# ducha-aiki/affnet

Measured on AMD Instinct MI355X. Metric: keypoints/sec (detect+AffNet+OriNet+HardNet) per image, 2000 kp @1024x768, higher is better.
Workload: dtype f32

## Files before the change

affnet_amd/SparseImgRepresenter.py:

```python
import ctypes as C

import torch
import torch.nn as nn

from . import _lib, engine
from ._lib import lib, check, ptr
from .architectures import _HipPatchNet
from .HandCraftedModules import AffineShapeEstimator, OrientationDetector, _HipHandCrafted
from .HardNet import HardTFeatNet
from .pytorch_sift import SIFTNet

_FOLLOW = (SIFTNet, HardTFeatNet)


class ScaleSpaceAffinePatchExtractor(nn.Module):
    def __init__(self, border=16, num_features=500, patch_size=32, mrSize=3.0, nlevels=3, num_Baum_iters=0,
                 init_sigma=1.6, th=None, RespNet=None, OriNet=None, AffNet=None, arith="fp32"):
        super(ScaleSpaceAffinePatchExtractor, self).__init__()
        self.arith = arith
        _lib.arith_code(arith)
        self.mrSize, self.PS, self.b = mrSize, patch_size, border
        self.num, self.nlevels = num_features, nlevels
        self.num_Baum_iters, self.init_sigma = num_Baum_iters, init_sigma
        self.th = th
        if th is not None:
            self.num = -1
        else:
            self.th = 0
        self.RespNet = RespNet
        if not 1 <= nlevels <= 6:
            raise NotImplementedError("nlevels must be 1..6 (levels per octave = nlevels + 2 <= 8)")
        self.OriNet = OriNet if OriNet is not None else OrientationDetector(patch_size=19)
        self.AffNet = AffNet if AffNet is not None else AffineShapeEstimator(patch_size=19)
        self.scale_pyr = self.sigmas = self.pix_dists = None
        self._ctx = None
        self._ctx_key = None
        self._fctx = self._fctx_key = self._pyr_ctx = None
        self.last_ids = None
        self.max_keep = 16384
        self.raw_div = 4
        self.lazy_shape_rows = -1
        self.shape_form = 1

        self.desc_form = 1

    def _context(self, x, allow_batch=False):
        engine.require_cuda(x, "image")
        if x.dim() != 4 or x.size(1) != 1 or x.size(0) < 1 or (x.size(0) != 1 and not allow_batch):
            raise ValueError("expected a (1,1,H,W) image; forward() is batch-size-1 like the reference "
                             "(HandCraftedModules.py:283-284) - use enqueue()/run_batch() for (B,1,H,W) batches")
        pre = int(1.5 * self.num) if self.num_Baum_iters > 0 else self.num
        key = (x.size(0), x.size(2), x.size(3), x.device, pre, self.num, float(self.th), self.mrSize, self.b, self.init_sigma,
               self.nlevels, self.max_keep, self.num_Baum_iters, self.raw_div, self.lazy_shape_rows)
        if self._ctx is not None and self._ctx_key == key and self._ctx.arith != _lib.arith_code(self.arith):
            self._ctx.set_arith(self.arith)
        if self._ctx is None or self._ctx_key != key:
            self._ctx = engine.Context(x.size(2), x.size(3), x.device, self.nlevels, self.init_sigma, self.b, self.mrSize,
                                       float(self.th), self.num, pre, self.max_keep, batch=x.size(0), baum_iters=self.num_Baum_iters, raw_div=self.raw_div,
                                       lazy_shape_rows=self.lazy_shape_rows, arith=self.arith)
            self._ctx_key = key
        if self._ctx.shape_form != int(self.shape_form):
            self._ctx.set_shape_form(self.shape_form)
        if self._ctx.desc_form != int(self.desc_form):
            self._ctx.set_desc_form(self.desc_form)
        return self._ctx

    def _publish_pyramid(self, ctx):
        self._pyr_ctx = ctx
        self.scale_pyr = ctx.pyramid_views()
        self.sigmas = [list(s) for s in ctx.plan.sigmas]
        self.pix_dists = [list(p) for p in ctx.plan.pix_dists]

    def _response_pyramid(self, ctx, img):
        dev = img.device
        st = engine.stream_of(dev)
        check(lib.affnet_pyramid_build(ctx.handle, ptr(img), st), ctx.handle, "affnet_pyramid_build")
        stride = lib.affnet_pyramid_image_stride(ctx.handle)
        base = lib.affnet_pyramid_level_offset(ctx.handle, 0, 0)
        resp = torch.zeros(ctx.batch * stride, dtype=torch.float32, device=dev)
        with torch.no_grad():
            for b in range(ctx.batch):
                pyr = ctx.pyramid_views(b)
                for o, (h, w) in enumerate(ctx.plan.sizes):
                    for l in range(ctx.plan.levels_per_octave):
                        off = b * stride + lib.affnet_pyramid_level_offset(ctx.handle, o, l) - base
                        r = self.RespNet(pyr[o][l], ctx.plan.sigmas[o][l])
                        resp[off:off + h * w].copy_(r.reshape(-1).to(dev, torch.float32))
        return resp

    @staticmethod
    def _native(slot):
        return slot is None or isinstance(slot, (_HipPatchNet, _HipHandCrafted))

    def enqueue(self, x, do_ori=False, desc=None, det_stream=None, input_ready=None):
        ctx = self._context(x, allow_batch=True)
        dev = x.device
        if not (self._native(self.AffNet) and self._native(self.OriNet)):
            raise NotImplementedError("the fused path needs the native AffNetFast / OriNetFast slots (foreign slots: forward())")
        img = x.contiguous().float()
        B, F = x.size(0), ctx.cap_final
        lafs = torch.empty(B, F, 2, 3, dtype=torch.float32, device=dev)
        resp = torch.empty(B, F, dtype=torch.float32, device=dev)
        ids = torch.empty(B, F, 3, dtype=torch.int32, device=dev)
        count = torch.zeros(B, dtype=torch.int32, device=dev)
        dsc = torch.empty(B, F, 128, dtype=torch.float32, device=dev) if desc is not None else None
        nets = self._nets(dev, do_ori, desc)
        follow = isinstance(desc, _FOLLOW)
        if isinstance(desc, HardTFeatNet):
            desc.check_usable()
        fused_dsc = None if follow else dsc
        if self.RespNet is not None:
            rmaps = self._response_pyramid(ctx, img)
            check(lib.affnet_detect_image_responses(ctx.handle, ptr(rmaps), engine.stream_of(dev)), ctx.handle, "affnet_detect_image_responses")
            rc = lib.affnet_describe_detected(ctx.handle, C.byref(nets), int(bool(do_ori)), ptr(lafs), ptr(resp), ptr(ids), ptr(fused_dsc),
                                              ptr(count), engine.stream_of(dev))
            check(rc, ctx.handle, "affnet_describe_detected")
        elif det_stream is None:
            rc = lib.affnet_extract_features(ctx.handle, C.byref(nets), ptr(img), int(bool(do_ori)), ptr(lafs), ptr(resp), ptr(ids),
                                             ptr(fused_dsc), ptr(count), engine.stream_of(dev))
            check(rc, ctx.handle, "affnet_extract_features")
        else:
            cur = torch.cuda.current_stream(dev)
            if input_ready is None:
                det_stream.wait_stream(cur)
            elif input_ready is not False:
                det_stream.wait_event(input_ready)
            if getattr(self, "_busy", None) is not None:
                det_stream.wait_event(self._busy)
            rc = lib.affnet_detect_image(ctx.handle, ptr(img), C.c_void_p(det_stream.cuda_stream))
            check(rc, ctx.handle, "affnet_detect_image")
            ev = torch.cuda.Event()
            ev.record(det_stream)
            cur.wait_event(ev)
            rc = lib.affnet_describe_detected(ctx.handle, C.byref(nets), int(bool(do_ori)), ptr(lafs), ptr(resp), ptr(ids), ptr(fused_dsc),
                                              ptr(count), engine.stream_of(dev))
            check(rc, ctx.handle, "affnet_describe_detected")
            self._busy = torch.cuda.Event()
            self._busy.record(cur)
        if follow:
            self._desc_follow(ctx, desc, lafs, count, dsc)
            if det_stream is not None:
                self._busy = torch.cuda.Event()
                self._busy.record(torch.cuda.current_stream(dev))
        if B == 1:
            lafs, resp, ids, dsc = lafs[0], resp[0], ids[0], (None if dsc is None else dsc[0])
        return {"LAFs": lafs, "responses": resp, "ids": ids, "descriptors": dsc, "count": count, "overflow": ctx.counter_view(0), "_img": img}

    def _desc_follow(self, ctx, desc, lafs, count, dsc):
        dev, (B, F) = lafs.device, lafs.shape[:2]
        st = engine.stream_of(dev)
        lvl = torch.empty(B, F, 3, dtype=torch.int32, device=dev)
        norm = torch.empty(B, F, 2, 3, dtype=torch.float32, device=dev)
        check(lib.affnet_level_select(ctx.handle, ptr(lafs), ptr(count), F, desc.PS, ptr(lvl), ptr(norm), st), ctx.handle, "affnet_level_select")
        if isinstance(desc, HardTFeatNet):
            floats = lib.affnet_tfeat_scratch_floats(B * F)
            cached = getattr(self, "_tfeat_scratch", None)
            if cached is None or cached.device != dev or cached.numel() < floats:
                cached = self._tfeat_scratch = torch.empty(floats, dtype=torch.float32, device=dev)
            check(lib.affnet_tfeat_forward_pyr(ctx.handle, ptr(desc.packed_weights(dev)), ptr(norm), ptr(lvl), ptr(count), F, ptr(dsc), ptr(cached), st),
                  ctx.handle, "affnet_tfeat_forward_pyr")
            return
        check(lib.affnet_sift_forward_pyr(ctx.handle, ptr(norm), ptr(lvl), ptr(count), F, ptr(desc.window(dev)), float(desc.clipval), ptr(dsc), st),
              ctx.handle, "affnet_sift_forward_pyr")

    def _nets(self, dev, do_ori, desc):
        nets = _lib.Nets()
        if self.num_Baum_iters > 0:
            if isinstance(self.AffNet, _HipHandCrafted):
                nets.h_baumberg_window = C.cast(self.AffNet.window(), C.c_void_p)
            else:
                nets.d_affnet = self.AffNet.packed_weights(dev).data_ptr()
        if do_ori:
            if isinstance(self.OriNet, _HipHandCrafted):
                nets.h_orientation_window = C.cast(self.OriNet.window(), C.c_void_p)
            else:
                nets.d_orinet = self.OriNet.packed_weights(dev).data_ptr()
        nets.d_hardnet = desc.packed_weights(dev).data_ptr() if desc is not None and not isinstance(desc, _FOLLOW) else None
        return nets

    def capture(self, x, do_ori=False, desc=None):
        if isinstance(desc, _FOLLOW):
            raise NotImplementedError("graph capture covers the fused C call (HardNet descriptors or none); the SIFT and HardTFeat descriptors "
                                      "follow it as further launches - use enqueue() / run()")
        return CapturedPath(self, x, do_ori, desc)

    def run_batch(self, x, do_ori=False, desc=None):
        r = self.enqueue(x, do_ori=do_ori, desc=desc)
        ctx = self._ctx
        ctx.read_counts(allow_empty=True)
        cnt = r["count"].cpu().tolist()
        if x.size(0) == 1:
            r = {k: (v.unsqueeze(0) if isinstance(v, torch.Tensor) and k not in ("count", "overflow", "_img") else v) for k, v in r.items()}
        out = []
        for b, n in enumerate(cnt):
            dsc = r["descriptors"]
            out.append({"LAFs": r["LAFs"][b, :n], "responses": r["responses"][b, :n], "ids": r["ids"][b, :n],
                        "descriptors": None if dsc is None else dsc[b, :n]})
        return out

    def run(self, x, do_ori=False, desc=None):
        if x.dim() == 4 and x.size(0) != 1:
            raise ValueError("run() is for a single (1,1,H,W) image; use run_batch() for (B,1,H,W) batches")
        r = self.enqueue(x, do_ori=do_ori, desc=desc)
        ctx = self._ctx
        self._publish_pyramid(ctx)
        n = int(ctx.read_counts()[1])
        self.last_ids = r["ids"][:n]
        dsc = r["descriptors"]
        return {"LAFs": r["LAFs"][:n], "responses": r["responses"][:n], "ids": r["ids"][:n],
                "descriptors": None if dsc is None else dsc[:n]}

    def _frames_context(self, x, n_max):
        engine.require_cuda(x, "image")
        if x.dim() != 4 or x.size(1) != 1 or x.size(0) < 1:
            raise ValueError("expected a (B,1,H,W) image batch")
        budget = self.num if (0 < self.num < n_max and self.num_Baum_iters > 0) else n_max
        key = (x.size(0), x.size(2), x.size(3), x.device, n_max, budget, self.mrSize, self.b, self.init_sigma, self.nlevels, self.num_Baum_iters,
               self.raw_div, self.lazy_shape_rows)
        if self._fctx is not None and self._fctx_key == key and self._fctx.arith != _lib.arith_code(self.arith):
            self._fctx.set_arith(self.arith)
        if self._fctx is None or self._fctx_key != key:
            self._fctx = engine.Context(x.size(2), x.size(3), x.device, self.nlevels, self.init_sigma, self.b, self.mrSize, float(self.th), budget, n_max,
                                        self.max_keep, batch=x.size(0), baum_iters=self.num_Baum_iters, raw_div=self.raw_div,
                                        lazy_shape_rows=self.lazy_shape_rows, arith=self.arith)
            self._fctx_key = key
        if self._fctx.shape_form != int(self.shape_form):
            self._fctx.set_shape_form(self.shape_form)
        if self._fctx.desc_form != int(self.desc_form):
            self._fctx.set_desc_form(self.desc_form)
        return self._fctx

    def enqueue_frames(self, x, LAFs, responses=None, counts=None, do_ori=True, desc=None):
        if not (self._native(self.AffNet) and self._native(self.OriNet)):
            raise NotImplementedError("the fused path needs the native AffNetFast / OriNetFast slots (foreign slots: getAffineShape / getOrientation)")
        engine.require_cuda(x, "image")
        engine.require_cuda(LAFs, "LAFs")
        dev, B = x.device, x.size(0)
        fr = LAFs.contiguous().float()
        if fr.dim() == 3:
            fr = fr.unsqueeze(0)
        if fr.dim() != 4 or fr.size(0) != B or tuple(fr.shape[2:]) != (2, 3):
            raise ValueError("LAFs must be (n,2,3) for one image or (B,n_max,2,3) for a (B,1,H,W) batch, got %s" % (tuple(LAFs.shape),))
        n_max = fr.size(1)
        if n_max == 0:
            fr, responses, counts, n_max = torch.zeros(B, 1, 2, 3, dtype=torch.float32, device=dev), None, [0] * B, 1
        rin = None
        if responses is not None:
            engine.require_cuda(responses, "responses")
            rin = responses.contiguous().float().view(B, n_max)
        cin = None
        if counts is not None:
            cin = counts if isinstance(counts, torch.Tensor) else torch.tensor(list(counts), dtype=torch.int32)
            cin = cin.to(dev, torch.int32).contiguous().view(B)
        ctx = self._frames_context(x, n_max)
        img = x.contiguous().float()
        F = ctx.cap_final
        lafs = torch.empty(B, F, 2, 3, dtype=torch.float32, device=dev)
        resp = torch.empty(B, F, dtype=torch.float32, device=dev)
        ids = torch.empty(B, F, 3, dtype=torch.int32, device=dev)
        count = torch.zeros(B, dtype=torch.int32, device=dev)
        dsc = torch.empty(B, F, 128, dtype=torch.float32, device=dev) if desc is not None else None
        nets = self._nets(dev, do_ori, desc)
        follow = isinstance(desc, _FOLLOW)
        if isinstance(desc, HardTFeatNet):
            desc.check_usable()
        rc = lib.affnet_describe_frames(ctx.handle, C.byref(nets), ptr(img), ptr(fr), ptr(rin), ptr(cin), n_max, int(bool(do_ori)), ptr(lafs), ptr(resp),
                                        ptr(ids), None if follow else ptr(dsc), ptr(count), engine.stream_of(dev))
        check(rc, ctx.handle, "affnet_describe_frames")
        if follow:
            self._desc_follow(ctx, desc, lafs, count, dsc)
        self._publish_pyramid(ctx)
        if B == 1:
            lafs, resp, ids, dsc = lafs[0], resp[0], ids[0], (None if dsc is None else dsc[0])
        return {"LAFs": lafs, "responses": resp, "ids": ids, "descriptors": dsc, "count": count, "overflow": ctx.counter_view(0), "_img": img,
                "_frames": (fr, rin, cin)}

    def describe_frames(self, x, LAFs, responses=None, counts=None, do_ori=True, desc=None):
        r = self.enqueue_frames(x, LAFs, responses=responses, counts=counts, do_ori=do_ori, desc=desc)
        ctx = self._fctx
        dsc = r["descriptors"]
        if x.size(0) == 1:
            n = int(ctx.read_counts()[1])
            self.last_ids = r["ids"][:n]
            return {"LAFs": r["LAFs"][:n], "responses": r["responses"][:n], "ids": r["ids"][:n], "descriptors": None if dsc is None else dsc[:n]}
        ctx.read_counts(allow_empty=True)
        return [{"LAFs": r["LAFs"][b, :n], "responses": r["responses"][b, :n], "ids": r["ids"][b, :n],
                 "descriptors": None if dsc is None else dsc[b, :n]} for b, n in enumerate(r["count"].cpu().tolist())]

    def _pyramid_ctx(self):
        ctx = self._pyr_ctx
        if ctx is None or self.scale_pyr is None:
            raise RuntimeError("call forward() / run() first: the pyramid of the last image is reused (stateful like the reference)")
        if ctx.batch != 1:
            raise RuntimeError("getAffineShape / getOrientation work on the pyramid of a single image")
        return ctx

    def _shape_stage(self, ctx, resp, lafs, ids, cnt, n):
        dev, st = lafs.device, engine.stream_of(lafs.device)
        P, F = ctx.cap_pre, ctx.cap_final
        PS = self.AffNet.PS
        patches = torch.empty(n, 1, PS, PS, dtype=torch.float32, device=dev)

        def shape_pass(frames):
            check(lib.affnet_pyr_grid_sample(ctx.handle, ptr(frames), ptr(ids), ptr(cnt), n, PS, ptr(patches), st), ctx.handle,
                  "affnet_pyr_grid_sample")
            with torch.no_grad():
                a = torch.cat([self.AffNet(patches[s:s + 256], {}) for s in range(0, n, 256)], 0)
            full = torch.zeros(P, 2, 2, dtype=torch.float32, device=dev)
            full[:n] = a.to(dev, torch.float32)
            return full
        A = shape_pass(lafs)
        if self.num_Baum_iters > 1:
            frames = torch.empty(P, 2, 3, dtype=torch.float32, device=dev)
            for _ in range(1, self.num_Baum_iters):
                check(lib.affnet_shape_iterate(ctx.handle, None, ptr(A), ptr(lafs), ptr(cnt), 0, ptr(frames), st), ctx.handle, "affnet_shape_iterate")
                Ai = shape_pass(frames)
                check(lib.affnet_shape_iterate(ctx.handle, ptr(Ai), ptr(A), ptr(lafs), ptr(cnt), 1, ptr(frames), st), ctx.handle, "affnet_shape_iterate")
        r2 = torch.empty(F, dtype=torch.float32, device=dev)
        l2 = torch.empty(F, 2, 3, dtype=torch.float32, device=dev)
        i2 = torch.empty(F, 3, dtype=torch.int32, device=dev)
        c2 = torch.zeros(1, dtype=torch.int32, device=dev)
        check(lib.affnet_shape_filter_select(ctx.handle, ptr(resp), ptr(lafs), ptr(ids), ptr(A), ptr(cnt), ptr(r2), ptr(l2),
                                             ptr(i2), ptr(c2), st), ctx.handle, "affnet_shape_filter_select")
        return r2, l2, i2, c2, int(c2.item())

    def _orientation_stage(self, ctx, lafs, ids, cnt, n):
        dev, st = lafs.device, engine.stream_of(lafs.device)
        PS = self.OriNet.PS
        patches = torch.empty(n, 1, PS, PS, dtype=torch.float32, device=dev)
        if n:
            check(lib.affnet_pyr_grid_sample(ctx.handle, ptr(lafs), ptr(ids), ptr(cnt), n, PS, ptr(patches), st), ctx.handle,
                  "affnet_pyr_grid_sample")
        with torch.no_grad():
            ang = self.OriNet(patches)
        if ang.dim() <= 2:
            c, s = torch.cos(ang).view(-1, 1, 1), torch.sin(ang).view(-1, 1, 1)
            ang = torch.cat([torch.cat([c, s], 2), torch.cat([-s, c], 2)], 1)
        R = ang.to(dev, torch.float32).contiguous()
        if n:
            check(lib.affnet_apply_rotation(ctx.handle, ptr(lafs), ptr(R), ptr(cnt), n, st), ctx.handle, "affnet_apply_rotation")

    @staticmethod
    def _frame_rows(ctx, LAFs, pyr_idxs, level_idxs, cap):
        engine.require_cuda(LAFs, "LAFs")
        dev, n = LAFs.device, LAFs.size(0)
        if n > cap:
            raise ValueError("%d frames, the context of the last forward() holds %d rows" % (n, cap))
        lafs = torch.zeros(cap, 2, 3, dtype=torch.float32, device=dev)
        lafs[:n] = LAFs.float()
        ids = torch.zeros(cap, 3, dtype=torch.int32, device=dev)
        ids[:n, 0] = torch.as_tensor(pyr_idxs).to(dev).view(-1).to(torch.int32)
        ids[:n, 1] = torch.as_tensor(level_idxs).to(dev).view(-1).to(torch.int32)
        ids[:n, 2] = torch.arange(n, dtype=torch.int32, device=dev)
        return lafs, ids, torch.full((1,), n, dtype=torch.int32, device=dev), n

    def getAffineShape(self, final_resp, LAFs, final_pyr_idxs, final_level_idxs, num_features=0):
        ctx = self._pyramid_ctx()
        if self.num_Baum_iters <= 0:
            raise ValueError("getAffineShape needs num_Baum_iters > 0 (the reference's loop body never runs otherwise, SparseImgRepresenter.py:127)")
        if num_features != self.num and not (num_features <= 0 and self.num <= 0):
            raise ValueError("num_features = %d: the context of the last forward() is sized for the extractor's own budget (%d)" % (num_features, self.num))
        lafs, ids, cnt, n = self._frame_rows(ctx, LAFs, final_pyr_idxs, final_level_idxs, ctx.cap_pre)
        resp = torch.zeros(ctx.cap_pre, dtype=torch.float32, device=lafs.device)
        resp[:n] = final_resp.to(lafs.device, torch.float32).view(-1)
        resp, lafs, ids, cnt, n = self._shape_stage(ctx, resp, lafs, ids, cnt, n)
        self.last_ids = ids[:n]
        return resp[:n], lafs[:n], ids[:n, 0].long(), ids[:n, 1].long()

    def getOrientation(self, LAFs, final_pyr_idxs, final_level_idxs):
        ctx = self._pyramid_ctx()
        lafs, ids, cnt, n = self._frame_rows(ctx, LAFs, final_pyr_idxs, final_level_idxs, LAFs.size(0))
        self._orientation_stage(ctx, lafs, ids, cnt, n)
        return lafs

    def _staged(self, x, do_ori):
        ctx = self._context(x)
        dev, st = x.device, engine.stream_of(x.device)
        img = x.contiguous().float()
        P = ctx.cap_pre
        rmaps = None
        if self.RespNet is not None:
            rmaps = self._response_pyramid(ctx, img)
        else:
            check(lib.affnet_pyramid_build(ctx.handle, ptr(img), st), ctx.handle, "affnet_pyramid_build")
        self._publish_pyramid(ctx)
        resp = torch.empty(P, dtype=torch.float32, device=dev)
        lafs = torch.empty(P, 2, 3, dtype=torch.float32, device=dev)
        ids = torch.empty(P, 3, dtype=torch.int32, device=dev)
        cnt = torch.zeros(1, dtype=torch.int32, device=dev)
        if rmaps is not None:
            check(lib.affnet_detect_responses(ctx.handle, ptr(rmaps), ptr(resp), ptr(lafs), ptr(ids), ptr(cnt), st), ctx.handle,
                  "affnet_detect_responses")
        else:
            check(lib.affnet_detect(ctx.handle, ptr(resp), ptr(lafs), ptr(ids), ptr(cnt), st), ctx.handle, "affnet_detect")
        n = int(cnt.item())
        ctx.read_counts()
        if self.num_Baum_iters > 0:
            resp, lafs, ids, cnt, n = self._shape_stage(ctx, resp, lafs, ids, cnt, n)
        if do_ori:
            self._orientation_stage(ctx, lafs, ids, cnt, n)
        out = torch.empty_like(lafs)
        check(lib.affnet_scale_lafs(ctx.handle, ptr(lafs), ptr(out), ptr(cnt), lafs.size(0), x.size(3), x.size(2), 0, st), ctx.handle,
              "affnet_scale_lafs")
        self.last_ids = ids[:n]
        return out[:n], resp[:n]

    def forward(self, x, do_ori=False):
        aff_native = self.num_Baum_iters == 0 or self._native(self.AffNet)
        ori_native = (not do_ori) or self._native(self.OriNet)
        if aff_native and ori_native:
            form, self.shape_form = self.shape_form, 0
            try:
                r = self.run(x, do_ori=do_ori)
            finally:
                self.shape_form = form
            return r["LAFs"], r["responses"]
        return self._staged(x, do_ori)

    def extract_patches_from_pyr(self, dLAFs, PS=41):
        if self._ctx is None or self.scale_pyr is None:
            raise RuntimeError("call forward() first: the pyramid of the last image is reused (stateful like the reference)")
        ctx = self._ctx
        if ctx.batch != 1:
            raise RuntimeError("extract_patches_from_pyr works on the pyramid of a single-image forward()")
        engine.require_cuda(dLAFs, "dLAFs")
        dev, st = dLAFs.device, engine.stream_of(dLAFs.device)
        lafs = dLAFs.contiguous().float()
        n = lafs.size(0)
        out = torch.empty(n, 1, PS, PS, dtype=torch.float32, device=dev)
        if n == 0:
            return out
        ids = torch.empty(n, 3, dtype=torch.int32, device=dev)
        norm = torch.empty(n, 2, 3, dtype=torch.float32, device=dev)
        check(lib.affnet_level_select(ctx.handle, ptr(lafs), None, n, PS, ptr(ids), ptr(norm), st), ctx.handle, "affnet_level_select")
        check(lib.affnet_pyr_grid_sample(ctx.handle, ptr(norm), ptr(ids), None, n, PS, ptr(out), st), ctx.handle, "affnet_pyr_grid_sample")
        self.last_level_ids = ids
        return out


class CapturedPath(object):
    def __init__(self, det, x, do_ori, desc):
        if not (det._native(det.AffNet) and det._native(det.OriNet)) or det.RespNet is not None:
            raise NotImplementedError("graph capture needs the native slots (foreign slots run Python between the stages)")
        ctx = det._context(x, allow_batch=True)
        dev = x.device
        self.det, self.ctx, self.do_ori, self.desc = det, ctx, bool(do_ori), desc
        B, F = x.size(0), ctx.cap_final
        self.image = x.contiguous().float().clone()
        self.out = {"LAFs": torch.empty(B, F, 2, 3, dtype=torch.float32, device=dev), "responses": torch.empty(B, F, dtype=torch.float32, device=dev),
                    "ids": torch.empty(B, F, 3, dtype=torch.int32, device=dev), "count": torch.zeros(B, dtype=torch.int32, device=dev),
                    "descriptors": torch.empty(B, F, 128, dtype=torch.float32, device=dev) if desc is not None else None}
        self._nets = det._nets(dev, do_ori, desc)
        self._mods = [m for m in (det.AffNet, det.OriNet if do_ori else None, desc) if m is not None and hasattr(m, "packed_weights")]
        self._blobs = [m.packed_weights(dev) for m in self._mods]
        self._stamps = [m._weights_stamp() for m in self._mods]
        self._arith = ctx.arith
        self._stream = torch.cuda.Stream(device=dev)
        torch.cuda.synchronize(dev)
        o = self.out
        check(lib.affnet_graph_capture_extract(ctx.handle, C.byref(self._nets), ptr(self.image), int(self.do_ori), ptr(o["LAFs"]), ptr(o["responses"]),
                                               ptr(o["ids"]), ptr(o["descriptors"]), ptr(o["count"]), C.c_void_p(self._stream.cuda_stream)),
              ctx.handle, "affnet_graph_capture_extract")

    def launch(self, x=None, check_weights=True):
        if check_weights:
            for m, stamp in zip(self._mods, self._stamps):
                if m._weights_stamp() != stamp:
                    raise RuntimeError("the weights of %s changed after capture(): the graph holds the old packed weights - capture again" % type(m).__name__)
        if self.ctx.arith != self._arith:
            raise RuntimeError("the arithmetic mode of the extractor changed after capture(): the graph runs the mode it was captured with - capture again")
        if x is not None:
            self.image.copy_(x, non_blocking=True)
        busy = getattr(self.det, "_busy", None)
        if busy is not None:
            torch.cuda.current_stream(self.image.device).wait_event(busy)
        check(lib.affnet_graph_launch(self.ctx.handle, engine.stream_of(self.image.device)), self.ctx.handle, "affnet_graph_launch")
        out = dict(self.out, overflow=self.ctx.counter_view(0), _img=self.image)
        if self.image.size(0) == 1:
            return {k: (v[0] if (v is not None and k not in ("count", "overflow", "_img")) else v) for k, v in out.items()}
        return out

    def run(self, x=None, check_weights=True):
        if self.image.size(0) != 1:
            raise ValueError("run() is for single images; use launch() for batches")
        r = self.launch(x, check_weights=check_weights)
        self.det._publish_pyramid(self.ctx)
        n = int(self.ctx.read_counts()[1])
        dsc = r["descriptors"]
        return {"LAFs": r["LAFs"][:n], "responses": r["responses"][:n], "ids": r["ids"][:n], "descriptors": None if dsc is None else dsc[:n]}


def get_geometry_and_descriptors(img, det, desc, do_ori=True):
    from .HardNet import HardNet
    if isinstance(desc, (HardNet,) + _FOLLOW) and det._native(det.AffNet) and det._native(det.OriNet):
        r = det.run(img, do_ori=do_ori, desc=desc)
        return r["LAFs"], r["descriptors"]
    with torch.no_grad():
        LAFs, resp = det(img, do_ori=do_ori)
        patches = det.extract_patches_from_pyr(LAFs, PS=32)
        return LAFs, desc(patches)
```

affnet_amd/_lib.py:

```python
import ctypes as C
import os

_HERE = os.path.dirname(os.path.abspath(__file__))
LIB_PATH = os.environ.get("AFFNET_HIP_LIB") or os.path.join(_HERE, "libaffnet_hip.so")
PROBES_LIB_PATH = os.path.join(_HERE, "libaffnet_hip_probes.so")

MAX_OCTAVES, MAX_LEVELS, MAX_TAPS = 16, 8, 37
NET_AFFNET, NET_ORINET, NET_HARDNET, NET_AFFNET_FULLCONV = 0, 1, 2, 3
ARITH_FP32_MFMA, ARITH_FP32_SPLIT3, ARITH_FP32_SPLIT2H = 0, 1, 2
ARITH_NAMES = {"fp32": ARITH_FP32_MFMA, "fp32_mfma": ARITH_FP32_MFMA, "fp32_split3": ARITH_FP32_SPLIT3, "split3": ARITH_FP32_SPLIT3,
               "fp32_split2h": ARITH_FP32_SPLIT2H, "split2h": ARITH_FP32_SPLIT2H}


def arith_code(arith):
    if arith is None:
        return ARITH_FP32_MFMA
    if isinstance(arith, str):
        if arith.lower() not in ARITH_NAMES:
            raise ValueError("arith must be one of %s" % sorted(ARITH_NAMES))
        return ARITH_NAMES[arith.lower()]
    if int(arith) not in (ARITH_FP32_MFMA, ARITH_FP32_SPLIT3, ARITH_FP32_SPLIT2H):
        raise ValueError("arith must be AFFNET_ARITH_FP32_MFMA (0), AFFNET_ARITH_FP32_SPLIT3 (1) or AFFNET_ARITH_FP32_SPLIT2H (2)")
    return int(arith)
SHAPE_FORM_DIRECT, SHAPE_FORM_WINOGRAD = 0, 1
DESC_FORM_DIRECT, DESC_FORM_POLYPHASE = 0, 1
OK, ERR_INVALID, ERR_HIP, ERR_CAPACITY, ERR_EMPTY = 0, -1, -2, -3, -4


class Config(C.Structure):
    _fields_ = [
        ("height", C.c_int32), ("width", C.c_int32), ("n_octaves", C.c_int32), ("levels_per_octave", C.c_int32),
        ("oct_h", C.c_int32 * MAX_OCTAVES), ("oct_w", C.c_int32 * MAX_OCTAVES),
        ("level_sigma", (C.c_float * MAX_LEVELS) * MAX_OCTAVES),
        ("level_sigma4", (C.c_float * MAX_LEVELS) * MAX_OCTAVES),
        ("level_sigma_px", (C.c_double * MAX_LEVELS) * MAX_OCTAVES),
        ("first_blur_taps", C.c_int32), ("first_blur", C.c_float * (MAX_TAPS * MAX_TAPS)),
        ("level_blur_taps", C.c_int32 * MAX_LEVELS),
        ("level_blur", (C.c_float * (MAX_TAPS * MAX_TAPS)) * MAX_LEVELS),
        ("level_blur0_taps", C.c_int32 * MAX_LEVELS),
        ("level_blur0", (C.c_float * (MAX_TAPS * MAX_TAPS)) * MAX_LEVELS),
        ("lazy_shape_rows", C.c_int32),
        ("onepass", C.c_int32),
        ("mr_size", C.c_float), ("threshold", C.c_float),
        ("num_features", C.c_int32), ("num_prefilter", C.c_int32),
        ("max_raw_per_octave_div", C.c_int32), ("max_keep", C.c_int32), ("batch", C.c_int32), ("baum_iters", C.c_int32),
        ("arith", C.c_int32),
    ]


class Nets(C.Structure):
    _fields_ = [("d_affnet", C.c_void_p), ("d_orinet", C.c_void_p), ("d_hardnet", C.c_void_p),
                ("h_orientation_window", C.c_void_p), ("h_baumberg_window", C.c_void_p)]


_P, _I, _SZ = C.c_void_p, C.c_int, C.c_size_t
SYMBOLS = {
    "affnet_config_fill": (_I, [C.POINTER(Config), _I, _I, _I, C.c_double, _I, C.c_double, C.c_double, _I, _I, _I, _I]),
    "affnet_ctx_create": (_I, [C.POINTER(_P), _I, C.POINTER(Config)]),
    "affnet_ctx_destroy": (None, [_P]),
    "affnet_last_error": (C.c_char_p, [_P]),
    "affnet_version": (C.c_char_p, []),
    "affnet_set_arith": (_I, [_P, _I]),
    "affnet_get_arith": (_I, [_P]),
    "affnet_set_shape_form": (_I, [_P, _I]),
    "affnet_get_shape_form": (_I, [_P]),
    "affnet_set_desc_form": (_I, [_P, _I]),
    "affnet_get_desc_form": (_I, [_P]),
    "affnet_workspace_bytes": (_SZ, [_P]),
    "affnet_bind_workspace": (_I, [_P, _P, _SZ]),
    "affnet_pyramid_level_offset": (C.c_int64, [_P, _I, _I]),
    "affnet_pyramid_image_stride": (C.c_int64, [_P]),
    "affnet_batch": (_I, [_P]),
    "affnet_capacity_prefilter": (_I, [_P]),
    "affnet_capacity_final": (_I, [_P]),
    "affnet_gauss_blur": (_I, [_P, _P, _P, _I, _I, C.POINTER(C.c_float), _I, _P]),
    "affnet_pyramid_build": (_I, [_P, _P, _P]),
    "affnet_hessian_response": (_I, [_P, _P, _P, _I, _I, C.c_float, _P]),
    "affnet_detect": (_I, [_P, _P, _P, _P, _P, _P]),
    "affnet_detect_responses": (_I, [_P, _P, _P, _P, _P, _P, _P]),
    "affnet_laf_grid_sample": (_I, [_P, _P, _I, _I, _P, _I, _I, _P, _P]),
    "affnet_pyr_grid_sample": (_I, [_P, _P, _P, _P, _I, _I, _P, _P]),
    "affnet_cnn32_packed_floats": (_SZ, [_I]),
    "affnet_cnn32_winograd_offset": (C.c_int64, [_I, _I]),
    "affnet_cnn32_pack_weights": (_I, [_I, C.POINTER(_P), C.POINTER(_P), C.POINTER(_P), _P, _P, _P, _P, _P]),
    "affnet_cnn32_forward": (_I, [_P, _I, _P, _P, _P, _I, _P, _P, _P]),
    "affnet_cnn32_forward_pyr": (_I, [_P, _I, _P, _P, _P, _P, _I, _P, _P, _P]),
    "affnet_local_norm": (_I, [_P, _P, _P, _I, _I, _P]),
    "affnet_fullconv_scratch_bytes": (_SZ, [_I, _I]),
    "affnet_fullconv_forward": (_I, [_P, _P, _P, _I, _I, _P, _P, _P]),
    "affnet_nms2d": (_I, [_P, _P, _P, _I, _I, C.c_float, _P]),
    "affnet_shape_filter_select": (_I, [_P, _P, _P, _P, _P, _P, _P, _P, _P, _P, _P]),
    "affnet_apply_rotation": (_I, [_P, _P, _P, _P, _I, _P]),
    "affnet_scale_lafs": (_I, [_P, _P, _P, _P, _I, _I, _I, _I, _P]),
    "affnet_lafs_to_ellipses": (_I, [_P, _P, _P, _I, _P, _P]),
    "affnet_ellipses_to_lafs": (_I, [_P, _P, _P, _I, _P, _P]),
    "affnet_level_select": (_I, [_P, _P, _P, _I, _I, _P, _P, _P]),
    "affnet_handcrafted_forward": (_I, [_P, _I, _P, _I, _P, _P, _P, _P]),
    "affnet_handcrafted_forward_pyr": (_I, [_P, _I, _P, _P, _P, _I, _P, _P, _P]),
    "affnet_sift_host_window": (_I, [_I, C.POINTER(C.c_float)]),
    "affnet_sift_forward": (_I, [_P, _P, _I, _P, C.c_float, _P, _P]),
    "affnet_sift_forward_pyr": (_I, [_P, _P, _P, _P, _I, _P, C.c_float, _P, _P]),
    "affnet_tfeat_packed_floats": (_SZ, []),
    "affnet_tfeat_pack_weights": (_I, [_P, _P, _P, _P, _P, _P, _P]),
    "affnet_tfeat_scratch_floats": (_SZ, [_I]),
    "affnet_tfeat_forward": (_I, [_P, _P, _P, _P, _I, _P, _P, _P]),
    "affnet_tfeat_forward_pyr": (_I, [_P, _P, _P, _P, _P, _I, _P, _P, _P]),
    "affnet_match_scratch_bytes": (_SZ, [_I, _I]),
    "affnet_distance_matrix": (_I, [_P, _P, _I, _P, _I, _I, _P, _P, _P]),
    "affnet_match_snn": (_I, [_P, _P, _I, _P, _I, _I, C.c_float, _P, _P, _P, _P, _P, _P, _P]),
    "affnet_reproject_lafs": (_I, [_P, _P, _I, C.POINTER(C.c_float), _P, _P]),
    "affnet_centre_nn": (_I, [_P, _P, _I, _P, _I, _P, _P, _P]),
    "affnet_extract_features": (_I, [_P, C.POINTER(Nets), _P, _I, _P, _P, _P, _P, _P, _P]),
    "affnet_detect_image": (_I, [_P, _P, _P]),
    "affnet_detect_image_responses": (_I, [_P, _P, _P]),
    "affnet_detect_image_onepass": (_I, [_P, _P, _P, _P]),
    "affnet_detect_image_onepass_responses": (_I, [_P, _P, _P, _P]),
    "affnet_detected_list": (_I, [_P, _P, _P, _P, _P, _P]),
    "affnet_load_frames": (_I, [_P, _P, _I, _P, _P, _P, _I, _I, _P]),
    "affnet_describe_frames": (_I, [_P, C.POINTER(Nets), _P, _P, _P, _P, _I, _I, _P, _P, _P, _P, _P, _P]),
    "affnet_shape_iterate": (_I, [_P, _P, _P, _P, _P, _I, _P, _P]),
    "affnet_affmap_offset": (C.c_int64, [_P, _I]),
    "affnet_affmap_image_stride": (C.c_int64, [_P]),
    "affnet_describe_detected": (_I, [_P, C.POINTER(Nets), _I, _P, _P, _P, _P, _P, _P]),
    "affnet_graph_capture_extract": (_I, [_P, C.POINTER(Nets), _P, _I, _P, _P, _P, _P, _P, _P]),
    "affnet_graph_launch": (_I, [_P, _P]),
    "affnet_profile_enable": (_I, [_P, _I]),
    "affnet_profile_read": (_I, [_P, C.POINTER(C.c_double * 8), C.POINTER(C.c_int32)]),
    "affnet_read_counts": (_I, [_P, C.POINTER(C.c_int32 * 4), _P]),
    "affnet_counter_offset": (C.c_int64, [_P, _I]),
    "affnet_counter_stride": (C.c_int64, [_P]),
    "affnet_host_base_grid": (_I, [_I, C.POINTER(C.c_float)]),
}

DEBUG_SYMBOLS = {
    "affnet_cnn32_debug_timing": (_I, [_P, _P]),
    "affnet_cnn32_debug_layer": (_I, [_P, _I, _P, _P, _I, _P, _P]),
    "affnet_cnn32_debug_winograd_u": (_I, [_P, _I, _P, _I, _P, _P]),
    "affnet_selftest_mfma": (_I, [_P, _P, _P, _P]),
    "affnet_debug_split3_variant": (_I, [_P, _I]),
}

PROBE_SYMBOLS = {
    "affnet_cnn32_probe": (_I, [_P, _I, _I, _I, _I, _P, _P]),
    "affnet_split3_gemm": (_I, [_P, _P, _I, _I, _I, _I, _P, _P]),
    "affnet_split3_rate": (_I, [_I, _I, _I, _P, _P]),
    "affnet_debug_stream": (_I, [_P, _P, _SZ, _I, _I, _I, _P]),
    "affnet_probe_shape_offsets": (_I, [_P, C.POINTER(C.c_int64 * 3)]),
    "affnet_probe_affnet_wino_layer": (_I, [_P, _I, _P, _P, _I, _P, _P]),
    "affnet_probe_affnet_wino_partials": (_I, [_P, _P, _P, _I, _P, _P]),
    "affnet_probe_hardnet_poly_layer": (_I, [_P, _P, _P, _I, _P, _P]),
    "affnet_probe_hardnet_poly_forward": (_I, [_P, _P, _P, _I, _P, _P, _P]),
    "affnet_probe_hardnet_poly_u": (_I, [_P, _P, _I, _P, _P]),
}


class AffnetHipError(RuntimeError):
    pass


class AffnetEmptyError(AffnetHipError):
    """AFFNET_ERR_EMPTY: no image of the call produced a detection (the reference raises in torch.cat([]),
    SparseImgRepresenter.py:100)."""


def _load():
    if not os.path.isfile(LIB_PATH):
        if os.path.basename(LIB_PATH) == os.path.basename(PROBES_LIB_PATH):
            raise ImportError("affnet_amd: %s is missing - the tools under tools/ need the probe build of the library: "
                              "AFFNET_PROBES=1 bash affnet_amd/csrc/build.sh" % LIB_PATH)
        raise ImportError(
            "affnet_amd: %s is missing - the HIP extension is the only implementation of this path "
            "(no CPU fallback). Build it: bash affnet_amd/csrc/build.sh" % LIB_PATH)
    lib = C.CDLL(LIB_PATH)
    for table in (SYMBOLS, DEBUG_SYMBOLS):
        for name, (res, args) in table.items():
            fn = getattr(lib, name)
            fn.restype, fn.argtypes = res, args
    for name, (res, args) in PROBE_SYMBOLS.items():
        if hasattr(lib, name):
            fn = getattr(lib, name)
            fn.restype, fn.argtypes = res, args
    return lib


lib = _load()


def check(rc, ctx=None, what=""):
    if rc != OK:
        msg = lib.affnet_last_error(ctx).decode() if ctx else ""
        if rc == ERR_EMPTY:
            raise AffnetEmptyError("%s: %s" % (what or "libaffnet_hip call", msg))
        raise AffnetHipError("%s failed (code %d): %s" % (what or "libaffnet_hip call", rc, msg))


def ptr(t):
    return None if t is None else C.c_void_p(t.data_ptr())


def current_stream(device):
    import torch
    return C.c_void_p(torch.cuda.current_stream(device).cuda_stream)
```

affnet_amd/csrc/cnn32.hip:

```cpp
#include "common.h"

static void aff_fill_pyr_src(const affnet_ctx* ctx, PyrSrc* s) {
    memset(s, 0, sizeof(*s));
    if (ctx->ws) aff_fill_pyr_table(ctx, &s->t);
    aff_base_grid(32, s->base);
}

static int cnn_check(affnet_ctx* ctx, const CnnCall& c, int* rows) {
    *rows = 0;
    if (c.kind < 0 || c.kind > 2) return aff_fail(ctx, AFFNET_ERR_INVALID, "cnn32: unknown net kind %d", c.kind);
    if (!c.packed || !c.out || c.n_max < 0 || (!c.patches && (!c.lafs || !c.ids))) return aff_fail(ctx, AFFNET_ERR_INVALID, "cnn32: null argument");
    if (!c.patches && !ctx->ws) return aff_fail(ctx, AFFNET_ERR_INVALID, "cnn32: sampling from the pyramid needs a bound workspace");
    if (c.dbg_layer < 0 && !c.scratch)
        return aff_fail(ctx, AFFNET_ERR_INVALID, "cnn32: d_scratch is required (HardNet n*(8192+512) floats, AffNet / OriNet n*144 floats)");
    if (c.dbg_layer >= 0 && ctx->arith != AFFNET_ARITH_FP32_MFMA)
        return aff_fail(ctx, AFFNET_ERR_INVALID, "cnn32: layer dumps exist for AFFNET_ARITH_FP32_MFMA only (context is in arithmetic mode %d)", ctx->arith);
    if (c.n_max == 0) return AFFNET_OK;
    if (c.kind == AFFNET_NET_HARDNET && c.n_max > 65535)
        return aff_fail(ctx, AFFNET_ERR_INVALID, "cnn32: n_max=%d (HardNet head: max 65535 rows per image)", c.n_max);
    const int row_count = c.row_count < 0 ? c.n_max - c.row_begin : c.row_count;
    if (c.row_begin < 0 || row_count < 0 || c.row_begin + row_count > c.n_max) return aff_fail(ctx, AFFNET_ERR_INVALID, "cnn32: bad row window");
    *rows = row_count;
    return AFFNET_OK;
}

int aff_arith_index(const affnet_ctx* ctx) {
    return ctx->arith == AFFNET_ARITH_FP32_SPLIT2H ? 2 : (ctx->arith == AFFNET_ARITH_FP32_SPLIT3 ? 1 : 0);
}

static int trunk_launch(affnet_ctx* ctx, const CnnCall& c, const NetLayout& L, dim3 grid, bool wino, const int32_t* reeval, int shape_op) {
    CnnArgs a;
    a.packed = c.packed; a.off = to_offsets(L, ctx->arith);
    a.wino_u = nullptr; a.reeval = reeval;
    if ((c.kind == AFFNET_NET_ORINET || wino) && ctx->arith == AFFNET_ARITH_FP32_MFMA) {
        const int rc = aff_wino_derive_u(ctx, c.kind, c.packed, L, c.st, &a.wino_u);
        if (rc) return rc;
    }
    const bool poly = c.poly && c.kind == AFFNET_NET_HARDNET && ctx->arith == AFFNET_ARITH_FP32_MFMA;
    if (poly) {
        const int rc = aff_poly_derive_u(ctx, c.packed, L, c.st, &a.wino_u);
        if (rc) return rc;
    }
    a.patches = c.patches; a.lafs = c.lafs; a.ids = c.ids; a.count = c.count; a.n_max = c.n_max;
    a.out = (c.dbg_layer < 0) ? c.scratch : c.out;
    a.dbg_layer = c.dbg_layer; a.dbg_out = c.dbg_out; a.dbg_time = ctx->dbg_time;
    a.row_begin = c.row_begin; a.skip_cnt = c.skip_cnt; a.skip_n = c.skip_n;
    a.shape_cnt = (c.fuse && shape_op) ? c.fuse->cnt : nullptr; a.shape_op = shape_op;
    a.s3_alt = ctx->split3_variant;
    PyrSrc ps;
    aff_fill_pyr_src(ctx, &ps);
    static_assert(AFFNET_NET_AFFNET == 0 && AFFNET_NET_ORINET == 1 && AFFNET_NET_HARDNET == 2, "trunk getter order");
    static TrunkKernel (*const trunk_of[3])(int, bool) = {aff_trunk_affnet, aff_trunk_orinet, aff_trunk_hardnet};
    const bool stamps = a.dbg_time || c.dbg_layer >= 0;
    hipLaunchKernelGGL(wino ? aff_trunk_affnet_wino(stamps) : (poly ? aff_trunk_hardnet_poly(stamps) : trunk_of[c.kind](aff_arith_index(ctx), stamps)), grid, dim3(512), 0, c.st, a, ps);
    AFF_LAUNCH_CHECK(ctx);
    return AFFNET_OK;
}

static int cnn_launch(affnet_ctx* ctx, const CnnCall& c) {
    int rows;
    int rc = cnn_check(ctx, c, &rows);
    if (rc || rows == 0) return rc;
    const NetLayout L = net_layout(c.kind);
    const int B = c.patches ? 1 : ctx->B;
    const bool form1 = c.wino_reeval && c.kind == AFFNET_NET_AFFNET && c.fuse && c.dbg_layer < 0 && ctx->arith == AFFNET_ARITH_FP32_MFMA;
    rc = trunk_launch(ctx, c, L, dim3(rows, B), form1, nullptr, c.shape_op);
    if (rc) return rc;
    if (form1) {
        int32_t* flags = reinterpret_cast<int32_t*>(c.scratch + (size_t)B * c.n_max * HEAD_PART_AFF);
        rc = aff_margin_affnet(ctx, c, L, rows, B, flags);
        if (rc) return rc;
        rc = trunk_launch(ctx, c, L, dim3(rows, B), false, flags, 0);
        if (rc) return rc;
    }
    if (c.dbg_layer < 0 && c.kind != AFFNET_NET_HARDNET) {
        rc = c.kind == AFFNET_NET_AFFNET ? aff_finish_affnet(ctx, c, L, rows, B) : aff_finish_orinet(ctx, c, L, rows, B);
        if (rc) return rc;
    }
    if (c.mark_head) aff_prof_mark(ctx, 7, c.st);
    if (c.dbg_layer < 0 && c.kind == AFFNET_NET_HARDNET) return aff_hardnet_head(ctx, c, L, B);
    return AFFNET_OK;
}

extern "C" int affnet_cnn32_forward(affnet_ctx* ctx, int net_kind, const float* d_packed, const float* d_patches, const int32_t* d_count,
                                    int n_max, float* d_out, float* d_scratch, void* stream) {
    AFF_DEVICE(ctx);
    if (!ctx || !d_patches) return aff_fail(ctx, AFFNET_ERR_INVALID, "cnn32_forward: null argument");
    CnnCall c;
    c.kind = net_kind; c.packed = d_packed; c.patches = d_patches; c.count = d_count; c.n_max = n_max; c.out = d_out; c.scratch = d_scratch; c.st = (hipStream_t)stream;
    return cnn_launch(ctx, c);
}

extern "C" int affnet_cnn32_forward_pyr(affnet_ctx* ctx, int net_kind, const float* d_packed, const float* d_lafs, const int32_t* d_ids,
                                        const int32_t* d_count, int n_max, float* d_out, float* d_scratch, void* stream) {
    AFF_DEVICE(ctx);
    if (!ctx) return AFFNET_ERR_INVALID;
    CnnCall c;
    c.kind = net_kind; c.packed = d_packed; c.lafs = d_lafs; c.ids = d_ids; c.count = d_count; c.n_max = n_max; c.out = d_out; c.scratch = d_scratch; c.st = (hipStream_t)stream;
    return cnn_launch(ctx, c);
}

int aff_affnet_filter_rows(affnet_ctx* ctx, const float* packed, const float* resp, const float* lafs, const int32_t* ids, const int32_t* count,
                           float* out, float* scratch, int row_begin, int row_count, bool lazy, int shape_op, hipStream_t st) {
    ShapeFuse sf;
    sf.resp = resp; sf.lafs = lafs; sf.key = ctx->st_key; sf.good = ctx->st_good; sf.cnt = ctx->cnt;
    CnnCall c;
    c.kind = AFFNET_NET_AFFNET; c.packed = packed; c.lafs = lafs; c.ids = ids; c.count = count; c.n_max = ctx->cap_pre; c.out = out; c.scratch = scratch; c.st = st;
    c.row_begin = row_begin; c.row_count = row_count;
    c.skip_cnt = lazy ? ctx->cnt : nullptr; c.skip_n = ctx->cfg.num_features;
    c.fuse = &sf; c.shape_op = shape_op;
    c.wino_reeval = ctx->shape_form == AFFNET_SHAPE_FORM_WINOGRAD;
    return cnn_launch(ctx, c);
}

int aff_orinet_rotate(affnet_ctx* ctx, const float* packed, float* lafs, const int32_t* ids, const int32_t* count, int n_max, float* out, float* scratch,
                      hipStream_t st, const DenormSel* denorm) {
    CnnCall c;
    c.kind = AFFNET_NET_ORINET; c.packed = packed; c.lafs = lafs; c.ids = ids; c.count = count; c.n_max = n_max; c.out = out; c.scratch = scratch; c.st = st;
    c.rot_lafs = lafs; c.denorm = denorm;
    return cnn_launch(ctx, c);
}

int aff_hardnet_forward_pyr_marked(affnet_ctx* ctx, const float* packed, const float* lafs, const int32_t* ids, const int32_t* count,
                                   int n_max, float* out, float* scratch, hipStream_t st) {
    CnnCall c;
    c.kind = AFFNET_NET_HARDNET; c.packed = packed; c.lafs = lafs; c.ids = ids; c.count = count; c.n_max = n_max; c.out = out; c.scratch = scratch; c.st = st;
    c.mark_head = true;
    c.poly = ctx->desc_form == AFFNET_DESC_FORM_POLYPHASE && !ctx->cfg.onepass;
    return cnn_launch(ctx, c);
}

int aff_hardnet_poly_patches(affnet_ctx* ctx, const float* packed, const float* patches, int n, float* out, float* scratch, int dbg_layer, hipStream_t st) {
    if (ctx->arith != AFFNET_ARITH_FP32_MFMA) return aff_fail(ctx, AFFNET_ERR_INVALID, "hardnet_poly: AFFNET_ARITH_FP32_MFMA only");
    CnnCall c;
    c.kind = AFFNET_NET_HARDNET; c.packed = packed; c.patches = patches; c.n_max = n; c.out = out; c.scratch = scratch; c.st = st;
    c.dbg_layer = dbg_layer; c.dbg_out = dbg_layer >= 0 ? out : nullptr;
    c.poly = true;
    return cnn_launch(ctx, c);
}

extern "C" int affnet_debug_split3_variant(affnet_ctx* ctx, int bits) {
    if (!ctx) return AFFNET_ERR_INVALID;
    ctx->split3_variant = bits;
    return AFFNET_OK;
}

extern "C" int affnet_cnn32_debug_timing(affnet_ctx* ctx, unsigned long long* d_stamps) {
    if (!ctx) return AFFNET_ERR_INVALID;
    ctx->dbg_time = d_stamps;
    return AFFNET_OK;
}

extern "C" int affnet_cnn32_debug_layer(affnet_ctx* ctx, int net_kind, const float* d_packed, const float* d_patch, int layer, float* d_out,
                                        void* stream) {
    AFF_DEVICE(ctx);
    if (!ctx || !d_patch || !d_out || layer < 0 || layer > 5) return aff_fail(ctx, AFFNET_ERR_INVALID, "cnn32_debug_layer: bad argument");
    CnnCall c;
    c.kind = net_kind; c.packed = d_packed; c.patches = d_patch; c.n_max = 1; c.out = d_out; c.st = (hipStream_t)stream;
    c.dbg_layer = layer; c.dbg_out = d_out;
    return cnn_launch(ctx, c);
}

extern "C" int affnet_cnn32_debug_winograd_u(affnet_ctx* ctx, int net_kind, const float* d_packed, int layer, float* d_out, void* stream) {
    AFF_DEVICE(ctx);
    if (!ctx || !d_packed || !d_out || (net_kind != AFFNET_NET_AFFNET && net_kind != AFFNET_NET_ORINET) || (layer != 1 && layer != 3 && layer != 5))
        return aff_fail(ctx, AFFNET_ERR_INVALID, "cnn32_debug_winograd_u: AffNet / OriNet, layer 1, 3 or 5");
    const float* u;
    const int rc = aff_wino_derive_u(ctx, net_kind, d_packed, net_layout(net_kind), (hipStream_t)stream, &u);
    if (rc) return rc;
    return aff_copy_async(ctx, d_out, u + Wino16::offset(layer), (size_t)Wino16::floats(layer) * sizeof(float), (hipStream_t)stream);
}
```

affnet_amd/csrc/cnn_trunk.h:

```cpp
#pragma once
#include <math.h>

#include <type_traits>

#include "common.h"

#include "cnn_mfma.h"

template <int TM>
__device__ __forceinline__ void head_partials(const float* __restrict__ hw, const f32x4 (&bias)[1], const f32x4 (&acc)[TM][1],
                                              float* __restrict__ part, int wave, int lane) {
    constexpr int MT = 4, MG = MT / TM;
    const int mg = wave % MG, ng = wave / MG;
    const int n = lane & 15, g = lane >> 4;
    const int c4 = ng * 16 + 4 * g;
    f32x4 v[TM];
#pragma unroll
    for (int i = 0; i < TM; ++i) {
        v[i] = acc[i][0] + bias[0];
        v[i].x = fmaxf(v[i].x, 0.0f); v[i].y = fmaxf(v[i].y, 0.0f); v[i].z = fmaxf(v[i].z, 0.0f); v[i].w = fmaxf(v[i].w, 0.0f);
    }
    const __amdgpu_buffer_rsrc_t r = weight_rsrc(hw, 3 * 4096);
    f32x4 w[3][TM];
#pragma unroll
    for (int o = 0; o < 3; ++o)
#pragma unroll
        for (int i = 0; i < TM; ++i) w[o][i] = buf_read4(r, (n * 64 + c4) * 4, (o * 4096 + (mg * TM + i) * 16 * 64) * 4);
#pragma unroll
    for (int o = 0; o < 3; ++o) {
        float sacc = 0.f;
#pragma unroll
        for (int i = 0; i < TM; ++i)
#pragma unroll
            for (int j = 0; j < 4; ++j) sacc = fmaf(v[i][j], w[o][i][j], sacc);
        sacc = wave_sum(sacc);
        if (lane == 0) part[wave * 4 + o] = sacc;
    }
}

__device__ __forceinline__ void aff_head_weights_wino(const float* __restrict__ hw, f32x4 (&w)[3][2], int wave, int lane) {
    const __amdgpu_buffer_rsrc_t r = weight_rsrc(hw, 3 * 4096);
    const int m = lane & 15, c4 = (wave >> 1) * 16 + 4 * (lane >> 4);
    const int pix = (2 * (m >> 2) + (wave & 1)) * 8 + 2 * (m & 3);
#pragma unroll
    for (int o = 0; o < 3; ++o)
#pragma unroll
        for (int k = 0; k < 2; ++k) w[o][k] = buf_read4(r, (pix * 64 + c4) * 4, (o * 4096 + k * 64) * 4);
}
__device__ __forceinline__ void head_partials_wino(const f32x4 (&w)[3][2], f32x4 bias, const f32x4 (&y)[2], float* __restrict__ part, int wave, int lane) {
    f32x4 v[2];
#pragma unroll
    for (int k = 0; k < 2; ++k) v[k] = bias_relu(y[k], bias);
#pragma unroll
    for (int o = 0; o < 3; ++o) {
        float sacc = 0.f;
#pragma unroll
        for (int k = 0; k < 2; ++k)
#pragma unroll
            for (int j = 0; j < 4; ++j) sacc = fmaf(v[k][j], w[o][k][j], sacc);
        sacc = wave_sum(sacc);
        if (lane == 0) part[wave * 4 + o] = sacc;
    }
}

#define ORI_HP 68
struct OriHeadLane {
    int mg, n, c4;
    template <int TM>
    __device__ __forceinline__ static OriHeadLane of(int wave, int lane) {
        constexpr int MT = 4, MG = MT / TM;
        const int mg = wave % MG, ng = wave / MG;
        const int n = lane & 15, g = lane >> 4;
        return {mg, n, ng * 16 + 4 * g};
    }
};
template <int TM>
__device__ __forceinline__ void ori_head_weights(const float* __restrict__ hw, const OriHeadLane& L, f32x4 (&w)[2][TM]) {
    const __amdgpu_buffer_rsrc_t r = weight_rsrc(hw, 2 * 4096);
#pragma unroll
    for (int o = 0; o < 2; ++o)
#pragma unroll
        for (int i = 0; i < TM; ++i) w[o][i] = buf_read4(r, (L.n * 64 + L.c4) * 4, (o * 4096 + (L.mg * TM + i) * 16 * 64) * 4);
}
template <int NTHR>
__device__ __forceinline__ void ori_head_zero_halo(float* act, int tid) {
    for (int e = tid; e < 36 * 16; e += NTHR) {
        const int hp = e >> 4, q4 = e & 15;
        const int y = hp < 10 ? 0 : (hp < 20 ? 9 : 1 + ((hp - 20) >> 1)), x = hp < 10 ? hp : (hp < 20 ? hp - 10 : ((hp - 20) & 1) * 9);
        *reinterpret_cast<f32x4*>(&act[(y * 10 + x) * ORI_HP + 4 * q4]) = (f32x4){0.f, 0.f, 0.f, 0.f};
    }
}
template <int TM>
__device__ __forceinline__ void ori_head_pbase(const OriHeadLane& L, int (&pbase)[TM]) {
#pragma unroll
    for (int i = 0; i < TM; ++i) {
        const int p = (L.mg * TM + i) * 16 + L.n;
        pbase[i] = ((p >> 3) * 10 + (p & 7)) * ORI_HP + L.c4;
    }
}
template <int TM>
__device__ __forceinline__ void ori_head_reduce(const f32x4 (&w)[2][TM], const int (&pbase)[TM], float* __restrict__ part, const float* act, int wave, int lane) {
    __syncthreads();
#pragma unroll
    for (int q = 0; q < 9; ++q) {
        float s0 = 0.f, s1 = 0.f;
#pragma unroll
        for (int i = 0; i < TM; ++i) {
            const f32x4 av = *reinterpret_cast<const f32x4*>(&act[pbase[i] + ((q / 3) * 10 + q % 3) * ORI_HP]);
#pragma unroll
            for (int j = 0; j < 4; ++j) { s0 = fmaf(av[j], w[0][i][j], s0); s1 = fmaf(av[j], w[1][i][j], s1); }
        }
        s0 = wave_sum(s0);
        s1 = wave_sum(s1);
        if (lane == 0) { part[wave * 18 + q] = s0; part[wave * 18 + 9 + q] = s1; }
    }
}
template <int TM, int NTHR>
__device__ __forceinline__ void head_partials_ori_lds(const float* __restrict__ hw, const f32x4 (&bias)[1], const f32x4 (&acc)[TM][1],
                                                      float* __restrict__ part, float* act, int wave, int lane, int tid) {
    constexpr int MT = 4, MG = MT / TM;
    const int mg = wave % MG, ng = wave / MG;
    const int n = lane & 15, g = lane >> 4;
    const int c4 = ng * 16 + 4 * g;
    f32x4 v[TM];
#pragma unroll
    for (int i = 0; i < TM; ++i) {
        v[i] = acc[i][0] + bias[0];
        v[i].x = fmaxf(v[i].x, 0.0f); v[i].y = fmaxf(v[i].y, 0.0f); v[i].z = fmaxf(v[i].z, 0.0f); v[i].w = fmaxf(v[i].w, 0.0f);
    }
    const __amdgpu_buffer_rsrc_t r = weight_rsrc(hw, 2 * 4096);
    f32x4 w[2][TM];
#pragma unroll
    for (int o = 0; o < 2; ++o)
#pragma unroll
        for (int i = 0; i < TM; ++i) w[o][i] = buf_read4(r, (n * 64 + c4) * 4, (o * 4096 + (mg * TM + i) * 16 * 64) * 4);
    __syncthreads();
    for (int e = tid; e < 36 * 16; e += NTHR) {
        const int hp = e >> 4, q4 = e & 15;
        const int y = hp < 10 ? 0 : (hp < 20 ? 9 : 1 + ((hp - 20) >> 1)), x = hp < 10 ? hp : (hp < 20 ? hp - 10 : ((hp - 20) & 1) * 9);
        *reinterpret_cast<f32x4*>(&act[(y * 10 + x) * ORI_HP + 4 * q4]) = (f32x4){0.f, 0.f, 0.f, 0.f};
    }
    int pbase[TM];
#pragma unroll
    for (int i = 0; i < TM; ++i) {
        const int p = (mg * TM + i) * 16 + n;
        pbase[i] = ((p >> 3) * 10 + (p & 7)) * ORI_HP + c4;
        *reinterpret_cast<f32x4*>(&act[pbase[i] + 11 * ORI_HP]) = v[i];
    }
    __syncthreads();
#pragma unroll
    for (int q = 0; q < 9; ++q) {
        float s0 = 0.f, s1 = 0.f;
#pragma unroll
        for (int i = 0; i < TM; ++i) {
            const f32x4 av = *reinterpret_cast<const f32x4*>(&act[pbase[i] + ((q / 3) * 10 + q % 3) * ORI_HP]);
#pragma unroll
            for (int j = 0; j < 4; ++j) { s0 = fmaf(av[j], w[0][i][j], s0); s1 = fmaf(av[j], w[1][i][j], s1); }
        }
        s0 = wave_sum(s0);
        s1 = wave_sum(s1);
        if (lane == 0) { part[wave * 18 + q] = s0; part[wave * 18 + 9 + q] = s1; }
    }
}

#define CNN_STAMP(k)                                                                                     \
    do {                                                                                                 \
        if (STAMPS && a.dbg_time && lane == 0) a.dbg_time[((size_t)pidx * NW + wave) * 32 + (k)] = __builtin_readcyclecounter(); \
    } while (0)

template <int CB>
struct TrunkLds {
    static constexpr int ACT = (CB / 4) * LayC0::PSG;
    static constexpr int PATCH = WP32 * WP32;
    static constexpr int RED = 256;
    static constexpr int TOTAL = ACT + PATCH + RED;
};

template <int KIND, int NW>
struct TrunkShape {
    static constexpr int CB = (KIND == AFFNET_NET_HARDNET) ? 32 : 16;
    static constexpr int NTHR = NW * 64;
    static constexpr int T1M = (CB == 16) ? 8 : 64 / NW, T1N = CB / 16;
    static constexpr int T2M = (CB == 16) ? 4 : 64 / NW, T2N = 1;
    static constexpr int T4M = (CB == 16) ? 2 : 32 / NW, T4N = 1;
    static constexpr int AREG = (NW == 8 && CB == 32) ? 128 : 48;
    static constexpr int G2 = pick_groups(CB, T2M, T2N, 32, AREG), G3 = pick_groups(2 * CB, T2M, T2N, 32, AREG);
    static constexpr int G4 = pick_groups(2 * CB, T4M, T4N, 32, AREG), G5 = pick_groups(4 * CB, T4M, T4N, 32, AREG);
};

template <int C, typename L, int NTHR>
__device__ __forceinline__ void dump_planes(const float* act, float* dst) {
    constexpr int H = L::H;
    for (int i = threadIdx.x; i < C * H * H; i += NTHR) {
        const int c = i / (H * H), r = i - c * H * H, y = r / H, x = r - y * H;
        dst[i] = act[L::at(c, y, x)];
    }
}

template <int CB>
struct SplitLays {
    typedef LayQ<16, 32, 34, CB, 0, 3> LQH;
    typedef LayQ<16, 32, 34, CB, 16, 3> LQH2;
    using LR0 = LayR<32, 32, 34, CB, 0>;
    using LR0H = LayR<16, 32, 34, CB, 0, 34>;
    using LR1 = LayR<32, 32, 34, CB, 16>;
    using LR1H = LayR<16, 32, 34, CB, 16, 34>;
    static_assert(LR0::BYTES <= TrunkLds<CB>::ACT * 4 && LR1::BYTES <= TrunkLds<CB>::ACT * 4 && LR0H::GS == LR0::GS && LR1H::GS == LR1::GS, "whole-patch split layouts");
    static_assert(LQH::BYTES <= TrunkLds<CB>::ACT * 4 && LQH2::BYTES <= TrunkLds<CB>::ACT * 4, "pre-split layouts must fit the activation buffer");
};

template <int KIND, int NW, bool STAMPS, int S3 = 0>
__global__ __launch_bounds__(NW * 64, (KIND == AFFNET_NET_HARDNET) ? NW / 4 : 4) void cnn32_trunk_kernel(CnnArgs a, PyrSrc ps) {
    static_assert(S3 == 0 || S3 == 2 || S3 == 3 || (S3 == 1 && KIND != AFFNET_NET_ORINET),
                  "S3 = number of terms of the split arithmetic; 1 = exact AffNet with Winograd conv1 / conv3 / conv5, exact HardNet with polyphase conv2 / conv4");
    constexpr bool EXACT = S3 <= 1;
    constexpr bool WINO13 = (S3 == 0 && KIND == AFFNET_NET_ORINET) || (S3 == 1 && KIND == AFFNET_NET_AFFNET);
    constexpr bool WINO5 = WINO13;
    constexpr bool POLY = S3 == 1 && KIND == AFFNET_NET_HARDNET;
    using S = TrunkShape<KIND, NW>;
    constexpr int CB = S::CB, NTHR = S::NTHR;
    static_assert((CB / 4) * LayC1::PSG <= TrunkLds<CB>::ACT && (CB / 2) * LayC3::PSG <= TrunkLds<CB>::ACT, "LDS layout");
    __shared__ __attribute__((aligned(16))) float lds[TrunkLds<CB>::TOTAL];
    float* act = lds;
    float* patch = lds + TrunkLds<CB>::ACT;
    float* red = patch + TrunkLds<CB>::PATCH;
    const int n = a.count ? min(a.count[blockIdx.y], a.n_max) : a.n_max;
    const int prow = blockIdx.x + a.row_begin;
    if (KIND == AFFNET_NET_AFFNET && a.shape_cnt && blockIdx.x == 0 && threadIdx.x == 0) {
        int32_t* c = a.shape_cnt + (size_t)blockIdx.y * CNT_TOTAL;
        if (a.shape_op == 1) { c[CNT_SURVIVED] = 0; c[CNT_SURVIVED1] = 0; c[CNT_AFF_EVAL] = 0; c[CNT_AFF_REEVAL] = 0; }
        else if (a.shape_op == 2) c[CNT_SURVIVED1] = c[CNT_SURVIVED];
    }
    if (prow >= n || lazy_skip(a.skip_cnt, a.skip_n, blockIdx.y, CNT_SURVIVED)) return;
    const size_t pidx = (size_t)blockIdx.y * a.n_max + prow;
    if (KIND == AFFNET_NET_AFFNET && a.reeval && a.reeval[pidx] == 0) return;
    const int tid = threadIdx.x, wave = tid >> 6, lane = tid & 63;
    if (KIND == AFFNET_NET_HARDNET) __builtin_amdgcn_s_setprio(3);
    CNN_STAMP(0);
    if (STAMPS && a.dbg_time && lane == 0) {
        a.dbg_time[((size_t)pidx * NW + wave) * 32 + 14] = __builtin_amdgcn_s_getreg((31 << 11) | 4);
        a.dbg_time[((size_t)pidx * NW + wave) * 32 + 15] = __builtin_amdgcn_s_getreg((31 << 11) | 20);
    }
    float w0[3][S::T1N];
    f32x4 bias0[S::T1N];
    conv0_load_w<NW, CB, S::T1M, S::T1N>(a.packed + a.off.w[0], a.packed + a.off.b[0], w0, bias0, wave, lane);
    f32x4 b1[1][S::T1N];
    f32x4 Ur[4];
    if constexpr (S3 == 0 && KIND == AFFNET_NET_AFFNET) prefetch_b0<NW, CB, 32, S::T1M, S::T1N, 1>(a.packed + a.off.w[1], b1, wave, lane);
    if constexpr (WINO13) wino_prefetch_u_row<NW, CB, CB, 32, Wino16::NB1>(a.wino_u, Ur, wave, lane);

    constexpr int PPT = 1024 / NTHR;
    constexpr int RPT = 32 / PPT;
    float v[PPT];
    if (a.patches) {
        const float* src = a.patches + pidx * 1024;
#pragma unroll
        for (int q = 0; q < PPT; ++q) v[q] = src[tid + q * NTHR];
    } else {
        int o = a.ids[3 * pidx], l = a.ids[3 * pidx + 1];
        o = o < 0 ? 0 : (o >= ps.t.n_octaves ? ps.t.n_octaves - 1 : o);
        l = l < 0 ? 0 : (l >= ps.t.n_levels ? ps.t.n_levels - 1 : l);
        const float* img = ps.t.lvl[o][l] + blockIdx.y * ps.t.img_stride;
        const int h = ps.t.h[o], w = ps.t.w[o];
        const float* L = a.lafs + 6 * pidx;
        const float m = (float)(h < w ? h : w);
        const float t00 = L[0] * m, t01 = L[1] * m, t02 = L[2] * (float)w;
        const float t10 = L[3] * m, t11 = L[4] * m, t12 = L[5] * (float)h;
#pragma unroll
        for (int q = 0; q < PPT; ++q)
            v[q] = aff_sample_bilinear(img, h, w, t00, t01, t02, t10, t11, t12, ps.base[tid & 31], ps.base[(tid >> 5) + q * RPT]);
    }
    CNN_STAMP(16);
    if (tid < 4 * 33) {
        const int e = tid;
        const int y = e < 34 ? 0 : (e < 68 ? 33 : 1 + ((e - 68) >> 1)), x = e < 34 ? e : (e < 68 ? e - 34 : ((e - 68) & 1) * 33);
        patch[y * WP32 + x] = 0.0f;
    }
    if constexpr (EXACT) zero_halo<LayC0, NTHR>(act, CB);
    else if constexpr (S3 == 2) zero_halo_q<typename SplitLays<CB>::LR0, NTHR>(act);
    else zero_halo_q<typename SplitLays<CB>::LQH, NTHR>(act);
    float sum = 0.f;
#pragma unroll
    for (int q = 0; q < PPT; ++q) sum += v[q];
    const float mean = block_sum<NW>(sum, red) * (1.0f / 1024.0f);
    CNN_STAMP(17);
    float sq = 0.f;
#pragma unroll
    for (int q = 0; q < PPT; ++q) { v[q] -= mean; sq += v[q] * v[q]; }
    const float var = block_sum<NW>(sq, red + NW) * (1.0f / 1023.0f);
    const float sd = sqrtf(var) + 1e-7f;
    CNN_STAMP(18);
#pragma unroll
    for (int q = 0; q < PPT; ++q) patch[((tid >> 5) + q * RPT + 1) * WP32 + (tid & 31) + 1] = v[q] / sd;
    __syncthreads();
    CNN_STAMP(1);

    if constexpr (S3 == 0 && KIND == AFFNET_NET_HARDNET) {
        constexpr int T1M = S::T1M, T1N = S::T1N, T2M = S::T2M, T2N = S::T2N, T4M = S::T4M, T4N = S::T4N;
        constexpr int NB1 = (16 * 16 / 16) * (CB / 16) / NW, NB3 = (8 * 8 / 16) * (2 * CB / 16) / NW, NB5 = (4 * 4 / 16) * (4 * CB / 16) / NW;

        f32x4 Up[2][4];
        f32x4 Uw[16];
        {
            f32x4 acc[T1M][T1N];
            conv0_mfma<NW, CB, T1M, T1N>(patch, w0, bias0, acc, wave, lane);
            CNN_STAMP(19);
            store_tiles_lds<CB, LayC0, T1M, T1N, false>(act, bias0, acc, wave, lane);
            CNN_STAMP(20);
            wino_prefetch_u_pair<NW, CB, CB, 32, NB1>(a.packed + a.off.w_wino[0], Up, wave, lane);
            __syncthreads();
        }
        if (STAMPS && a.dbg_layer == 0) { dump_planes<CB, LayC0, NTHR>(act, a.dbg_out); return; }
        CNN_STAMP(2);

        f32x4 b2[S::G2][T2N];
        f32x4 bias2[T2N];
        {
            f32x4 y[NB1][4], bw[NB1];
            __builtin_amdgcn_s_setprio(0);
            conv3x3_wino_mfma_pair_rows<NW, CB, CB, LayC0, NB1>(act, a.packed + a.off.w_wino[0], Up, y, wave, lane);
            __builtin_amdgcn_s_setprio(3);
            CNN_STAMP(3);
            prefetch_b0<NW, 2 * CB, 16, T2M, T2N, S::G2>(a.packed + a.off.w[2], b2, wave, lane);
            prefetch_bias<NW, 16, T2M, T2N>(a.packed + a.off.b[2], bias2, wave, lane);
            wino_bias<NW, 32, CB, NB1>(a.packed + a.off.b[1], bw, wave, lane);
            __syncthreads();
            CNN_STAMP(21);
            zero_halo<LayC1, NTHR>(act, CB);
            wino_store_lds<CB, LayC1, NB1>(act, bw, y, wave, lane);
            CNN_STAMP(22);
            __syncthreads();
            CNN_STAMP(4);
        }
        if (STAMPS && a.dbg_layer == 1) { dump_planes<CB, LayC1, NTHR>(act, a.dbg_out); return; }

        {
            f32x4 acc[T2M][T2N];
            __builtin_amdgcn_s_setprio(0);
            conv3x3_mfma<NW, CB, 2 * CB, LayC1, 2, T2M, T2N, S::G2>(act, a.packed + a.off.w[2], b2, acc, wave, lane);
            __builtin_amdgcn_s_setprio(3);
            CNN_STAMP(5);
            wino_prefetch_u_pair<NW, 2 * CB, 2 * CB, 16, NB3>(a.packed + a.off.w_wino[1], Up, wave, lane);
            __syncthreads();
            zero_halo<LayC2, NTHR>(act, 2 * CB);
            store_tiles_lds<2 * CB, LayC2, T2M, T2N>(act, bias2, acc, wave, lane);
            __syncthreads();
            CNN_STAMP(6);
        }
        if (STAMPS && a.dbg_layer == 2) { dump_planes<2 * CB, LayC2, NTHR>(act, a.dbg_out); return; }

        f32x4 b4[S::G4][T4N];
        f32x4 bias4[T4N];
        {
            f32x4 y[NB3][4], bw[NB3];
            __builtin_amdgcn_s_setprio(0);
            conv3x3_wino_mfma_pair_rows<NW, 2 * CB, 2 * CB, LayC2, NB3>(act, a.packed + a.off.w_wino[1], Up, y, wave, lane);
            __builtin_amdgcn_s_setprio(3);
            CNN_STAMP(7);
            prefetch_b0<NW, 4 * CB, 8, T4M, T4N, S::G4>(a.packed + a.off.w[4], b4, wave, lane);
            prefetch_bias<NW, 8, T4M, T4N>(a.packed + a.off.b[4], bias4, wave, lane);
            wino_bias<NW, 16, 2 * CB, NB3>(a.packed + a.off.b[3], bw, wave, lane);
            __syncthreads();
            zero_halo<LayC3, NTHR>(act, 2 * CB);
            wino_store_lds<2 * CB, LayC3, NB3>(act, bw, y, wave, lane);
            __syncthreads();
            CNN_STAMP(8);
        }
        if (STAMPS && a.dbg_layer == 3) { dump_planes<2 * CB, LayC3, NTHR>(act, a.dbg_out); return; }

        {
            f32x4 acc[T4M][T4N];
            __builtin_amdgcn_s_setprio(0);
            conv3x3_mfma<NW, 2 * CB, 4 * CB, LayC3, 2, T4M, T4N, S::G4>(act, a.packed + a.off.w[4], b4, acc, wave, lane);
            __builtin_amdgcn_s_setprio(3);
            CNN_STAMP(9);
            wino_prefetch_u<NW, 4 * CB, 4 * CB, 8, NB5>(a.packed + a.off.w_wino[2], Uw, wave, lane);
            __syncthreads();
            zero_halo<LayC4, NTHR>(act, 4 * CB);
            store_tiles_lds<4 * CB, LayC4, T4M, T4N>(act, bias4, acc, wave, lane);
            __syncthreads();
            CNN_STAMP(10);
        }
        if (STAMPS && a.dbg_layer == 4) { dump_planes<4 * CB, LayC4, NTHR>(act, a.dbg_out); return; }

        f32x4 y[NB5][4], bw[NB5];
        __builtin_amdgcn_s_setprio(0);
        static_assert(NB5 == 1 && (4 * CB / 16) * 4096 <= TrunkLds<CB>::ACT, "conv5: one pass per wave, V of the layer fits the activation buffer");
        conv3x3_wino_mfma_shared_v<NW, 4 * CB, 4 * CB, LayC4>(act, a.packed + a.off.w_wino[2], Uw, y, wave, lane);
        __builtin_amdgcn_s_setprio(3);
        CNN_STAMP(11);
        wino_bias<NW, 8, 4 * CB, NB5>(a.packed + a.off.b[5], bw, wave, lane);
        if (!STAMPS || a.dbg_layer < 0) {
            wino_store_global<4 * CB, 8, NB5>(a.out + pidx * (64 * 4 * CB), bw, y, wave, lane);
            CNN_STAMP(13);
            return;
        }
        __syncthreads();
        wino_store_lds<4 * CB, LayC5, NB5>(act, bw, y, wave, lane);
        __syncthreads();
        CNN_STAMP(12);
        if (STAMPS && a.dbg_layer == 5) { dump_planes<4 * CB, LayC5, NTHR>(act, a.dbg_out); return; }
    } else if constexpr (POLY) {
        constexpr int T1M = S::T1M, T1N = S::T1N;
        constexpr int NB1 = (16 * 16 / 16) * (CB / 16) / NW, NB3 = (8 * 8 / 16) * (2 * CB / 16) / NW, NB5 = (4 * 4 / 16) * (4 * CB / 16) / NW;
        constexpr int NBP2 = (8 * 8 / 16) * (2 * CB / 16) / NW, NBP4 = (4 * 4 / 16) * (4 * CB / 16) / NW;

        f32x4 Up[2][4];
        f32x4 Uw[16];
        {
            f32x4 acc[T1M][T1N];
            conv0_mfma<NW, CB, T1M, T1N>(patch, w0, bias0, acc, wave, lane);
            CNN_STAMP(19);
            store_tiles_lds<CB, LayC0, T1M, T1N, false>(act, bias0, acc, wave, lane);
            CNN_STAMP(20);
            wino_prefetch_u_pair<NW, CB, CB, 32, NB1>(a.packed + a.off.w_wino[0], Up, wave, lane);
            __syncthreads();
        }
        if (STAMPS && a.dbg_layer == 0) { dump_planes<CB, LayC0, NTHR>(act, a.dbg_out); return; }
        CNN_STAMP(2);

        f32x4 P2a[2][3], P2b[2][3];
        {
            f32x4 y[NB1][4], bw[NB1];
            __builtin_amdgcn_s_setprio(0);
            conv3x3_wino_mfma_pair_rows<NW, CB, CB, LayC0, NB1>(act, a.packed + a.off.w_wino[0], Up, y, wave, lane);
            __builtin_amdgcn_s_setprio(3);
            CNN_STAMP(3);
            poly_prefetch_u<NW, CB, 2 * CB, 16, NBP2, 2>(a.wino_u + Poly32::offset(2), P2a, P2b, wave, lane);
            wino_bias<NW, 32, CB, NB1>(a.packed + a.off.b[1], bw, wave, lane);
            __syncthreads();
            CNN_STAMP(21);
            zero_halo<LayC1, NTHR>(act, CB);
            wino_store_lds<CB, LayC1, NB1>(act, bw, y, wave, lane);
            CNN_STAMP(22);
            __syncthreads();
            CNN_STAMP(4);
        }
        if (STAMPS && a.dbg_layer == 1) { dump_planes<CB, LayC1, NTHR>(act, a.dbg_out); return; }

        {
            f32x4 y[NBP2][4], bw[NBP2];
            __builtin_amdgcn_s_setprio(0);
            conv3x3_poly_mfma_rows<NW, CB, 2 * CB, LayC1, NBP2, 2>(act, a.wino_u + Poly32::offset(2), P2a, P2b, y, wave, lane);
            __builtin_amdgcn_s_setprio(3);
            CNN_STAMP(5);
            wino_prefetch_u_pair<NW, 2 * CB, 2 * CB, 16, NB3>(a.packed + a.off.w_wino[1], Up, wave, lane);
            wino_bias<NW, 16, 2 * CB, NBP2>(a.packed + a.off.b[2], bw, wave, lane);
            __syncthreads();
            zero_halo<LayC2, NTHR>(act, 2 * CB);
            wino_store_lds<2 * CB, LayC2, NBP2>(act, bw, y, wave, lane);
            __syncthreads();
            CNN_STAMP(6);
        }
        if (STAMPS && a.dbg_layer == 2) { dump_planes<2 * CB, LayC2, NTHR>(act, a.dbg_out); return; }

        f32x4 P4a[1][3], P4b[1][3];
        {
            f32x4 y[NB3][4], bw[NB3];
            __builtin_amdgcn_s_setprio(0);
            conv3x3_wino_mfma_pair_rows<NW, 2 * CB, 2 * CB, LayC2, NB3>(act, a.packed + a.off.w_wino[1], Up, y, wave, lane);
            __builtin_amdgcn_s_setprio(3);
            CNN_STAMP(7);
            poly_prefetch_u<NW, 2 * CB, 4 * CB, 8, NBP4, 1>(a.wino_u + Poly32::offset(4), P4a, P4b, wave, lane);
            wino_bias<NW, 16, 2 * CB, NB3>(a.packed + a.off.b[3], bw, wave, lane);
            __syncthreads();
            zero_halo<LayC3, NTHR>(act, 2 * CB);
            wino_store_lds<2 * CB, LayC3, NB3>(act, bw, y, wave, lane);
            __syncthreads();
            CNN_STAMP(8);
        }
        if (STAMPS && a.dbg_layer == 3) { dump_planes<2 * CB, LayC3, NTHR>(act, a.dbg_out); return; }

        {
            f32x4 y[NBP4][4], bw[NBP4];
            __builtin_amdgcn_s_setprio(0);
            conv3x3_poly_mfma_rows<NW, 2 * CB, 4 * CB, LayC3, NBP4, 1>(act, a.wino_u + Poly32::offset(4), P4a, P4b, y, wave, lane);
            __builtin_amdgcn_s_setprio(3);
            CNN_STAMP(9);
            wino_prefetch_u<NW, 4 * CB, 4 * CB, 8, NB5>(a.packed + a.off.w_wino[2], Uw, wave, lane);
            wino_bias<NW, 8, 4 * CB, NBP4>(a.packed + a.off.b[4], bw, wave, lane);
            __syncthreads();
            zero_halo<LayC4, NTHR>(act, 4 * CB);
            wino_store_lds<4 * CB, LayC4, NBP4>(act, bw, y, wave, lane);
            __syncthreads();
            CNN_STAMP(10);
        }
        if (STAMPS && a.dbg_layer == 4) { dump_planes<4 * CB, LayC4, NTHR>(act, a.dbg_out); return; }

        f32x4 y[NB5][4], bw[NB5];
        __builtin_amdgcn_s_setprio(0);
        static_assert(NB5 == 1 && (4 * CB / 16) * 4096 <= TrunkLds<CB>::ACT, "conv5: one pass per wave, V of the layer fits the activation buffer");
        conv3x3_wino_mfma_shared_v<NW, 4 * CB, 4 * CB, LayC4>(act, a.packed + a.off.w_wino[2], Uw, y, wave, lane);
        __builtin_amdgcn_s_setprio(3);
        CNN_STAMP(11);
        wino_bias<NW, 8, 4 * CB, NB5>(a.packed + a.off.b[5], bw, wave, lane);
        if (!STAMPS || a.dbg_layer < 0) {
            wino_store_global<4 * CB, 8, NB5>(a.out + pidx * (64 * 4 * CB), bw, y, wave, lane);
            CNN_STAMP(13);
            return;
        }
        __syncthreads();
        wino_store_lds<4 * CB, LayC5, NB5>(act, bw, y, wave, lane);
        __syncthreads();
        CNN_STAMP(12);
        if (STAMPS && a.dbg_layer == 5) { dump_planes<4 * CB, LayC5, NTHR>(act, a.dbg_out); return; }
    } else if constexpr (EXACT) {
        constexpr int T1M = S::T1M, T1N = S::T1N, T2M = S::T2M, T2N = S::T2N, T4M = S::T4M, T4N = S::T4N;
        static_assert(NW == 8 && CB == 16, "Wino16 describes the 16-channel trunks on 8 waves");
        f32x4 b4[S::G4][T4N];
        f32x4 bias4[T4N];
        if constexpr (WINO13) {
            constexpr int NB1 = Wino16::NB1, NB3 = Wino16::NB3;
            {
                f32x4 acc[T1M][T1N];
                conv0_mfma<NW, CB, T1M, T1N>(patch, w0, bias0, acc, wave, lane);
                CNN_STAMP(19);
                store_tiles_lds<CB, LayC0, T1M, T1N, false>(act, bias0, acc, wave, lane);
                CNN_STAMP(20);
                __syncthreads();
            }
            if (STAMPS && a.dbg_layer == 0) { dump_planes<CB, LayC0, NTHR>(act, a.dbg_out); return; }
            CNN_STAMP(2);

            f32x4 b2[S::G2][T2N];
            f32x4 bias2[T2N];
            {
                f32x4 y[NB1][4], bw[NB1];
                conv3x3_wino_mfma_rows<NW, CB, CB, LayC0, NB1>(act, a.wino_u, Ur, y, wave, lane);
                CNN_STAMP(3);
                prefetch_b0<NW, 2 * CB, 16, T2M, T2N, S::G2>(a.packed + a.off.w[2], b2, wave, lane);
                prefetch_bias<NW, 16, T2M, T2N>(a.packed + a.off.b[2], bias2, wave, lane);
                wino_bias<NW, 32, CB, NB1>(a.packed + a.off.b[1], bw, wave, lane);
                __syncthreads();
                CNN_STAMP(21);
                zero_halo<LayC1, NTHR>(act, CB);
                wino_store_lds<CB, LayC1, NB1>(act, bw, y, wave, lane);
                CNN_STAMP(22);
                __syncthreads();
                CNN_STAMP(4);
            }
            if (STAMPS && a.dbg_layer == 1) { dump_planes<CB, LayC1, NTHR>(act, a.dbg_out); return; }

            {
                f32x4 acc[T2M][T2N];
                conv3x3_mfma<NW, CB, 2 * CB, LayC1, 2, T2M, T2N, S::G2>(act, a.packed + a.off.w[2], b2, acc, wave, lane);
                CNN_STAMP(5);
                wino_prefetch_u_row<NW, 2 * CB, 2 * CB, 16, NB3>(a.wino_u + Wino16::offset(3), Ur, wave, lane);
                __syncthreads();
                zero_halo<LayC2, NTHR>(act, 2 * CB);
                store_tiles_lds<2 * CB, LayC2, T2M, T2N>(act, bias2, acc, wave, lane);
                __syncthreads();
                CNN_STAMP(6);
            }
            if (STAMPS && a.dbg_layer == 2) { dump_planes<2 * CB, LayC2, NTHR>(act, a.dbg_out); return; }

            {
                f32x4 y[NB3][4], bw[NB3];
                conv3x3_wino_mfma_rows<NW, 2 * CB, 2 * CB, LayC2, NB3>(act, a.wino_u + Wino16::offset(3), Ur, y, wave, lane);
                CNN_STAMP(7);
                prefetch_b0<NW, 4 * CB, 8, T4M, T4N, S::G4>(a.packed + a.off.w[4], b4, wave, lane);
                prefetch_bias<NW, 8, T4M, T4N>(a.packed + a.off.b[4], bias4, wave, lane);
                wino_bias<NW, 16, 2 * CB, NB3>(a.packed + a.off.b[3], bw, wave, lane);
                __syncthreads();
                zero_halo<LayC3, NTHR>(act, 2 * CB);
                wino_store_lds<2 * CB, LayC3, NB3>(act, bw, y, wave, lane);
                __syncthreads();
                CNN_STAMP(8);
            }
            if (STAMPS && a.dbg_layer == 3) { dump_planes<2 * CB, LayC3, NTHR>(act, a.dbg_out); return; }

        } else {
            static_assert(T1M * 8 > S::AREG, "conv1: two A sets of T1M float4 do not fit -> rolling single set (conv3x3_mfma_roll)");
            f32x4 bias1[T1N];
            {
                f32x4 acc[T1M][T1N];
                conv0_mfma<NW, CB, T1M, T1N>(patch, w0, bias0, acc, wave, lane);
                CNN_STAMP(19);
                prefetch_bias<NW, 32, T1M, T1N>(a.packed + a.off.b[1], bias1, wave, lane);
                store_tiles_lds<CB, LayC0, T1M, T1N, false>(act, bias0, acc, wave, lane);
                CNN_STAMP(20);
                __syncthreads();
            }
            if (STAMPS && a.dbg_layer == 0) { dump_planes<CB, LayC0, NTHR>(act, a.dbg_out); return; }
            CNN_STAMP(2);

            f32x4 b2[S::G2][T2N];
            f32x4 bias2[T2N];
            {
                f32x4 acc[T1M][T1N];
                conv3x3_mfma_roll<NW, CB, CB, LayC0, 1, T1M, T1N>(act, a.packed + a.off.w[1], b1, acc, wave, lane);
                CNN_STAMP(3);
                prefetch_b0<NW, 2 * CB, 16, T2M, T2N, S::G2>(a.packed + a.off.w[2], b2, wave, lane);
                prefetch_bias<NW, 16, T2M, T2N>(a.packed + a.off.b[2], bias2, wave, lane);
                __syncthreads();
                CNN_STAMP(21);
                zero_halo<LayC1, NTHR>(act, CB);
                store_tiles_lds<CB, LayC1, T1M, T1N>(act, bias1, acc, wave, lane);
                CNN_STAMP(22);
                __syncthreads();
                CNN_STAMP(4);
            }
            if (STAMPS && a.dbg_layer == 1) { dump_planes<CB, LayC1, NTHR>(act, a.dbg_out); return; }

            f32x4 b3[S::G3][T2N];
            f32x4 bias3[T2N];
            {
                f32x4 acc[T2M][T2N];
                conv3x3_mfma<NW, CB, 2 * CB, LayC1, 2, T2M, T2N, S::G2>(act, a.packed + a.off.w[2], b2, acc, wave, lane);
                CNN_STAMP(5);
                prefetch_b0<NW, 2 * CB, 16, T2M, T2N, S::G3>(a.packed + a.off.w[3], b3, wave, lane);
                prefetch_bias<NW, 16, T2M, T2N>(a.packed + a.off.b[3], bias3, wave, lane);
                __syncthreads();
                zero_halo<LayC2, NTHR>(act, 2 * CB);
                store_tiles_lds<2 * CB, LayC2, T2M, T2N>(act, bias2, acc, wave, lane);
                __syncthreads();
                CNN_STAMP(6);
            }
            if (STAMPS && a.dbg_layer == 2) { dump_planes<2 * CB, LayC2, NTHR>(act, a.dbg_out); return; }

            {
                f32x4 acc[T2M][T2N];
                conv3x3_mfma<NW, 2 * CB, 2 * CB, LayC2, 1, T2M, T2N, S::G3>(act, a.packed + a.off.w[3], b3, acc, wave, lane);
                CNN_STAMP(7);
                prefetch_b0<NW, 4 * CB, 8, T4M, T4N, S::G4>(a.packed + a.off.w[4], b4, wave, lane);
                prefetch_bias<NW, 8, T4M, T4N>(a.packed + a.off.b[4], bias4, wave, lane);
                __syncthreads();
                zero_halo<LayC3, NTHR>(act, 2 * CB);
                store_tiles_lds<2 * CB, LayC3, T2M, T2N>(act, bias3, acc, wave, lane);
                __syncthreads();
                CNN_STAMP(8);
            }
            if (STAMPS && a.dbg_layer == 3) { dump_planes<2 * CB, LayC3, NTHR>(act, a.dbg_out); return; }

        }

        f32x4 b5[S::G5][T4N];
        f32x4 bias5[T4N];
        {
            f32x4 acc[T4M][T4N];
            conv3x3_mfma<NW, 2 * CB, 4 * CB, LayC3, 2, T4M, T4N, S::G4>(act, a.packed + a.off.w[4], b4, acc, wave, lane);
            CNN_STAMP(9);
            if constexpr (WINO5) {
                wino5_prefetch_u(a.wino_u + Wino16::offset(5), Ur, wave, lane);
            } else {
                prefetch_b0<NW, 4 * CB, 8, T4M, T4N, S::G5>(a.packed + a.off.w[5], b5, wave, lane);
                prefetch_bias<NW, 8, T4M, T4N>(a.packed + a.off.b[5], bias5, wave, lane);
            }
            __syncthreads();
            zero_halo<LayC4, NTHR>(act, 4 * CB);
            store_tiles_lds<4 * CB, LayC4, T4M, T4N>(act, bias4, acc, wave, lane);
            __syncthreads();
            CNN_STAMP(10);
        }
        if (STAMPS && a.dbg_layer == 4) { dump_planes<4 * CB, LayC4, NTHR>(act, a.dbg_out); return; }

        static_assert(!WINO5 || (Wino5::X >= 16 * LayC4::PSG && Wino5::X + Wino5::X_FLOATS <= TrunkLds<CB>::TOTAL),
                      "Winograd conv5: the exchange lies behind conv4's output inside the LDS array");
        if constexpr (KIND == AFFNET_NET_ORINET) {
            static_assert(Wino5::HEAD + 100 * ORI_HP <= Wino5::X, "conv5: the head copy in front of the exchange");
            f32x4 acc[2][4], y[2], hw[2][T4M];
            conv3x3_wino_mfma_half_rows<NW, LayC4>(act, a.wino_u + Wino16::offset(5), Ur, acc, wave, lane);
            CNN_STAMP(11);
            const f32x4 bw = *reinterpret_cast<const f32x4*>(&a.packed[a.off.b[5] + (wave >> 1) * 16 + 4 * (lane >> 4)]);
            const OriHeadLane HL = OriHeadLane::of<T4M>(wave, lane);
            if (!STAMPS || a.dbg_layer < 0) ori_head_weights<T4M>(a.packed + a.off.head_w, HL, hw);
            wino5_combine(lds, acc, y, wave, lane);
            if (!STAMPS || a.dbg_layer < 0) {
                float* copy = lds + Wino5::HEAD;
                ori_head_zero_halo<NTHR>(copy, tid);
                wino5_store_lds<10, ORI_HP, 4>(copy + 11 * ORI_HP, bw, y, wave, lane);
                int pbase[T4M];
                ori_head_pbase<T4M>(HL, pbase);
                ori_head_reduce<T4M>(hw, pbase, a.out + pidx * HEAD_PART_ORI, copy, wave, lane);
                CNN_STAMP(13);
                return;
            }
            __syncthreads();
            wino5_store_lds<LayC5::WP, 4, LayC5::PSG>(act + (LayC5::WP + 1) * 4, bw, y, wave, lane);
            __syncthreads();
            CNN_STAMP(12);
            if (STAMPS && a.dbg_layer == 5) { dump_planes<4 * CB, LayC5, NTHR>(act, a.dbg_out); return; }
            return;
        } else if constexpr (WINO5) {
            f32x4 acc[2][4], y[2], hw[3][2];
            conv3x3_wino_mfma_half_rows<NW, LayC4>(act, a.wino_u + Wino16::offset(5), Ur, acc, wave, lane);
            CNN_STAMP(11);
            const f32x4 bw = *reinterpret_cast<const f32x4*>(&a.packed[a.off.b[5] + (wave >> 1) * 16 + 4 * (lane >> 4)]);
            if (!STAMPS || a.dbg_layer < 0) aff_head_weights_wino(a.packed + a.off.head_w, hw, wave, lane);
            wino5_combine(lds, acc, y, wave, lane);
            if (!STAMPS || a.dbg_layer < 0) {
                head_partials_wino(hw, bw, y, a.out + pidx * HEAD_PART_AFF, wave, lane);
                CNN_STAMP(13);
                return;
            }
            __syncthreads();
            wino5_store_lds<LayC5::WP, 4, LayC5::PSG>(act + (LayC5::WP + 1) * 4, bw, y, wave, lane);
            __syncthreads();
            CNN_STAMP(12);
            if (STAMPS && a.dbg_layer == 5) { dump_planes<4 * CB, LayC5, NTHR>(act, a.dbg_out); return; }
            return;
        }
        f32x4 acc[T4M][T4N];
        conv3x3_mfma<NW, 4 * CB, 4 * CB, LayC4, 1, T4M, T4N, S::G5>(act, a.packed + a.off.w[5], b5, acc, wave, lane);
        CNN_STAMP(11);
        if (!STAMPS || a.dbg_layer < 0) {
            head_partials<T4M>(a.packed + a.off.head_w, bias5, acc, a.out + pidx * HEAD_PART_AFF, wave, lane);
            CNN_STAMP(13);
            return;
        }
        __syncthreads();
        store_tiles_lds<4 * CB, LayC5, T4M, T4N>(act, bias5, acc, wave, lane);
        __syncthreads();
        CNN_STAMP(12);
        if (STAMPS && a.dbg_layer == 5) { dump_planes<4 * CB, LayC5, NTHR>(act, a.dbg_out); return; }
    } else if constexpr (KIND == AFFNET_NET_HARDNET) {
        using SL = SplitLays<CB>;
        using LQH = typename SL::LQH;
        using LQH2 = typename SL::LQH2;
        using LR0 = typename SL::LR0;
        using LR1 = typename SL::LR1;
        constexpr int TERMS = S3;
        constexpr bool WHOLE = TERMS == 2;
        f32x4 bias1[2];
        const int s3_alt = a.s3_alt;
        using LQ2 = std::conditional_t<TERMS == 2, LayR<16, 16, 20, 2 * CB, 16>, LayQ<16, 16, 18, 2 * CB, 0, 3>>;
        using LQ4 = std::conditional_t<TERMS == 2, LayR<8, 8, 12, 4 * CB, 0>, LayQ<8, 8, 16, 4 * CB, 128, 3>>;
        static_assert(LQ2::BYTES <= TrunkLds<CB>::ACT * 4 && LQ4::BYTES <= TrunkLds<CB>::ACT * 4, "pre-split layouts must fit the activation buffer");
        char* base = reinterpret_cast<char*>(act);
        f32x4 acc_a[4][2], acc_b[4][2];
        S3W<2> wf1;
        S3W<1> wf2;
        f32x4 acc2_a[4][1], acc2_b[4][1], bias2[1];
        f32x4 acc2w[4][2], bias2w[2];
        if constexpr (WHOLE) {
            f32x4 acc1[8][2];
            S3W<2> wf2w;
            s3_prefetch_w0<NW, CB, CB, 64, 8, 2, TERMS>(a.packed + a.off.w_s3[1], wf1, wave, lane);
            prefetch_bias<NW, 32, 8, 2>(a.packed + a.off.b[1], bias1, wave, lane);
            conv0_whole_split_q<NW, LR0, 2>(patch, w0, bias0, act, wave, lane);
            __syncthreads();
            CNN_STAMP(2);
            __builtin_amdgcn_s_setprio(0);
            conv3x3_mfma_s3q<NW, CB, CB, LR0, 1, 8, 2>(act, a.packed + a.off.w_s3[1], wf1, acc1, wave, lane, s3_alt);
            __builtin_amdgcn_s_setprio(3);
            CNN_STAMP(3);
            s3_prefetch_w0<NW, CB, 2 * CB, 16, 4, 2, TERMS>(a.packed + a.off.w_s3[2], wf2w, wave, lane);
            prefetch_bias<NW, 16, 4, 2>(a.packed + a.off.b[2], bias2w, wave, lane);
            __syncthreads();
            zero_halo_q<LR1, NTHR>(act);
            store_tiles_split_q<CB, LR1, 8, 2>(act, bias1, acc1, wave, lane);
            __syncthreads();
            CNN_STAMP(4);
            __builtin_amdgcn_s_setprio(0);
            conv3x3_mfma_s3q<NW, CB, 2 * CB, LR1, 2, 4, 2>(act, a.packed + a.off.w_s3[2], wf2w, acc2w, wave, lane, s3_alt);
            __builtin_amdgcn_s_setprio(3);
        } else {
            s3_prefetch_w0<NW, CB, CB, 32, 4, 2, TERMS>(a.packed + a.off.w_s3[1], wf1, wave, lane);
            prefetch_bias<NW, 32, 8, 2>(a.packed + a.off.b[1], bias1, wave, lane);
            conv0_half_split_q<NW, LQH, 2>(patch, w0, bias0, act, 0, wave, lane);
            __syncthreads();
            CNN_STAMP(2);
            __builtin_amdgcn_s_setprio(0);
            conv3x3_mfma_s3q<NW, CB, CB, LQH, 1, 4, 2>(act, a.packed + a.off.w_s3[1], wf1, acc_a, wave, lane, s3_alt);
            __builtin_amdgcn_s_setprio(3);
            __syncthreads();
            if (tid < LQH::SLOTS * 4 * 32) {
                const int t = tid / 128, g = (tid >> 5) & 3, x = tid & 31;
                *reinterpret_cast<f32x4*>(base + g * LQH::GS + LQH::at(17, x + 1) + t * LQH::TSTEP) = (f32x4){0.f, 0.f, 0.f, 0.f};
            }
            conv0_half_split_q<NW, LQH, 2>(patch, w0, bias0, act, 1, wave, lane);
            __syncthreads();
            __builtin_amdgcn_s_setprio(0);
            conv3x3_mfma_s3q<NW, CB, CB, LQH, 1, 4, 2>(act, a.packed + a.off.w_s3[1], wf1, acc_b, wave, lane, s3_alt);
            __builtin_amdgcn_s_setprio(3);
            CNN_STAMP(3);
            s3_prefetch_w0<NW, CB, 2 * CB, 8, 4, 1, TERMS>(a.packed + a.off.w_s3[2], wf2, wave, lane);
            bias2[0] = *reinterpret_cast<const f32x4*>(&a.packed[a.off.b[2] + (wave >> 1) * 16 + 4 * (lane >> 4)]);
            __syncthreads();
            zero_halo_q<LQH2, NTHR>(act);
            store_tiles_split_q<CB, LQH2, 4, 2>(act, bias1, acc_a, wave, lane);
            __syncthreads();
            CNN_STAMP(4);
            __builtin_amdgcn_s_setprio(0);
            conv3x3_mfma_s3q<NW, CB, 2 * CB, LQH2, 2, 4, 1>(act, a.packed + a.off.w_s3[2], wf2, acc2_a, wave, lane, s3_alt);
            __builtin_amdgcn_s_setprio(3);
            __syncthreads();
            store_tiles_split_q<CB, LQH2, 4, 2>(act, bias1, acc_b, wave, lane);
            if (wave == 7) {
                const int n = lane & 15;
#pragma unroll
                for (int i = 2; i < 4; ++i) split_store_tile_q<LQH2, 2>(base, LQH2::at(0, (i - 2) * 16 + n + 1), 0, bias1, acc_a[i], lane >> 4);
            }
            __syncthreads();
            __builtin_amdgcn_s_setprio(0);
            conv3x3_mfma_s3q<NW, CB, 2 * CB, LQH2, 2, 4, 1>(act, a.packed + a.off.w_s3[2], wf2, acc2_b, wave, lane, s3_alt);
            __builtin_amdgcn_s_setprio(3);
        }
        CNN_STAMP(5);
        S3W<2> wf3;
        S3W<1> wf4, wf5;
        f32x4 bias3[2], bias4[1], bias5s[1];
        s3_prefetch_w0<NW, 2 * CB, 2 * CB, 16, 4, 2, TERMS>(a.packed + a.off.w_s3[3], wf3, wave, lane);
        prefetch_bias<NW, 16, 4, 2>(a.packed + a.off.b[3], bias3, wave, lane);
        __syncthreads();
        zero_halo_q<LQ2, NTHR>(act);
        if constexpr (WHOLE) store_tiles_split_q<2 * CB, LQ2, 4, 2>(act, bias2w, acc2w, wave, lane);
        else {
            store_tiles_split_q<2 * CB, LQ2, 4, 1, 8>(act, bias2, acc2_a, wave, lane, 0);
            store_tiles_split_q<2 * CB, LQ2, 4, 1, 8>(act, bias2, acc2_b, wave, lane, 8);
        }
        __syncthreads();
        CNN_STAMP(6);
        {
            f32x4 acc_[4][2];
            __builtin_amdgcn_s_setprio(0);
            conv3x3_mfma_s3q<NW, 2 * CB, 2 * CB, LQ2, 1, 4, 2>(act, a.packed + a.off.w_s3[3], wf3, acc_, wave, lane, s3_alt);
            __builtin_amdgcn_s_setprio(3);
            CNN_STAMP(7);
            s3_prefetch_w0<NW, 2 * CB, 4 * CB, 4, 4, 1, TERMS>(a.packed + a.off.w_s3[4], wf4, wave, lane);
            prefetch_bias<NW, 8, 4, 1>(a.packed + a.off.b[4], bias4, wave, lane);
            __syncthreads();
            store_tiles_split_q<2 * CB, LQ2, 4, 2>(act, bias3, acc_, wave, lane);
            __syncthreads();
            CNN_STAMP(8);
        }
        {
            f32x4 acc_[4][1];
            __builtin_amdgcn_s_setprio(0);
            conv3x3_mfma_s3q<NW, 2 * CB, 4 * CB, LQ2, 2, 4, 1>(act, a.packed + a.off.w_s3[4], wf4, acc_, wave, lane, s3_alt);
            __builtin_amdgcn_s_setprio(3);
            CNN_STAMP(9);
            s3_prefetch_w0<NW, 4 * CB, 4 * CB, 4, 4, 1, TERMS>(a.packed + a.off.w_s3[5], wf5, wave, lane);
            prefetch_bias<NW, 8, 4, 1>(a.packed + a.off.b[5], bias5s, wave, lane);
            __syncthreads();
            zero_halo_q<LQ4, NTHR>(act);
            store_tiles_split_q<4 * CB, LQ4, 4, 1>(act, bias4, acc_, wave, lane);
            __syncthreads();
            CNN_STAMP(10);
        }
        f32x4 acc5[4][1];
        __builtin_amdgcn_s_setprio(0);
        conv3x3_mfma_s3q<NW, 4 * CB, 4 * CB, LQ4, 1, 4, 1>(act, a.packed + a.off.w_s3[5], wf5, acc5, wave, lane, s3_alt);
        __builtin_amdgcn_s_setprio(3);
        CNN_STAMP(11);
        store_tiles_global<4 * CB, 4, 1>(a.out + pidx * (64 * 4 * CB), bias5s, acc5, wave, lane);
    } else {
        constexpr int T4M = S::T4M, T4N = S::T4N;
        using SL = SplitLays<CB>;
        using LQH = typename SL::LQH;
        using LQH2 = typename SL::LQH2;
        using LR0 = typename SL::LR0;
        using LR0H = typename SL::LR0H;
        using LR1 = typename SL::LR1;
        using LR1H = typename SL::LR1H;
        constexpr int TERMS = S3;
        constexpr bool WHOLE = TERMS == 2;
        f32x4 bias1[1];
        using LQ2 = std::conditional_t<TERMS == 2, LayR<16, 16, 20, 2 * CB, 0>, LayQ<16, 16, 18, 2 * CB, 0, 3>>;
        using LQ4 = std::conditional_t<TERMS == 2, LayR<8, 8, 12, 4 * CB, 0>, LayQ<8, 8, 16, 4 * CB, 128, 3>>;
        static_assert(LQ2::BYTES <= TrunkLds<CB>::ACT * 4 && LQ4::BYTES <= TrunkLds<CB>::ACT * 4, "pre-split layouts must fit the activation buffer");
        char* base = reinterpret_cast<char*>(act);
        f32x4 acc_a[4][1], acc_b[4][1];
        S3W<1> wf1, wf2;
        f32x4 acc2_a[2][1], acc2_b[2][1], bias2[1];
        if constexpr (WHOLE) {
            prefetch_bias_fresh<NW, 32, 8, 1>(a.packed + a.off.b[1], bias1, wave, lane);
            conv0_whole_split_q<NW, LR0, 1>(patch, w0, bias0, act, wave, lane);
            s3_prefetch_w0<NW, CB, CB, 32, 4, 1, TERMS>(a.packed + a.off.w_s3[1], wf1, wave, lane);
            __syncthreads();
            CNN_STAMP(2);
            conv3x3_mfma_s3q<NW, CB, CB, LR0H, 1, 4, 1>(act, a.packed + a.off.w_s3[1], wf1, acc_a, wave, lane, false);
            conv3x3_mfma_s3q<NW, CB, CB, LR0H, 1, 4, 1>(act + LR0::at(16, 0) / 4, a.packed + a.off.w_s3[1], wf1, acc_b, wave, lane, false);
            CNN_STAMP(3);
            {
                int l2 = lane;
                asm volatile("" : "+v"(l2));
                bias2[0] = *reinterpret_cast<const f32x4*>(&a.packed[a.off.b[2] + (wave >> 2) * 16 + 4 * (l2 >> 4)]);
            }
            __syncthreads();
            zero_halo_q<LR1, NTHR>(act);
            store_tiles_split_q<CB, LR1, 4, 1, 16>(act, bias1, acc_a, wave, lane, 0);
            store_tiles_split_q<CB, LR1, 4, 1, 16>(act, bias1, acc_b, wave, lane, 16);
            s3_prefetch_w0<NW, CB, 2 * CB, 8, 2, 1, TERMS>(a.packed + a.off.w_s3[2], wf2, wave, lane);
            __syncthreads();
            CNN_STAMP(4);
            conv3x3_mfma_s3q<NW, CB, 2 * CB, LR1H, 2, 2, 1>(act, a.packed + a.off.w_s3[2], wf2, acc2_a, wave, lane, false);
            conv3x3_mfma_s3q<NW, CB, 2 * CB, LR1H, 2, 2, 1>(act + LR1::at(16, 0) / 4, a.packed + a.off.w_s3[2], wf2, acc2_b, wave, lane, false);
        } else {
            prefetch_bias_fresh<NW, 32, 8, 1>(a.packed + a.off.b[1], bias1, wave, lane);
            conv0_half_split_q<NW, LQH, 1>(patch, w0, bias0, act, 0, wave, lane);
            s3_prefetch_w0<NW, CB, CB, 32, 4, 1, TERMS>(a.packed + a.off.w_s3[1], wf1, wave, lane);
            __syncthreads();
            CNN_STAMP(2);
            conv3x3_mfma_s3q<NW, CB, CB, LQH, 1, 4, 1>(act, a.packed + a.off.w_s3[1], wf1, acc_a, wave, lane, false);
            __syncthreads();
            if (tid < LQH::SLOTS * 2 * 32) {
                const int t = tid >> 6, g = (tid >> 5) & 1, x = tid & 31;
                *reinterpret_cast<f32x4*>(base + g * LQH::GS + LQH::at(17, x + 1) + t * LQH::TSTEP) = (f32x4){0.f, 0.f, 0.f, 0.f};
            }
            conv0_half_split_q<NW, LQH, 1>(patch, w0, bias0, act, 1, wave, lane);
            s3_prefetch_w0<NW, CB, CB, 32, 4, 1, TERMS>(a.packed + a.off.w_s3[1], wf1, wave, lane);
            __syncthreads();
            conv3x3_mfma_s3q<NW, CB, CB, LQH, 1, 4, 1>(act, a.packed + a.off.w_s3[1], wf1, acc_b, wave, lane, false);
            CNN_STAMP(3);
            {
                int l2 = lane;
                asm volatile("" : "+v"(l2));
                bias2[0] = *reinterpret_cast<const f32x4*>(&a.packed[a.off.b[2] + (wave >> 2) * 16 + 4 * (l2 >> 4)]);
            }
            __syncthreads();
            zero_halo_q<LQH2, NTHR>(act);
            store_tiles_split_q<CB, LQH2, 4, 1>(act, bias1, acc_a, wave, lane);
            s3_prefetch_w0<NW, CB, 2 * CB, 8, 2, 1, TERMS>(a.packed + a.off.w_s3[2], wf2, wave, lane);
            __syncthreads();
            CNN_STAMP(4);
            conv3x3_mfma_s3q<NW, CB, 2 * CB, LQH2, 2, 2, 1>(act, a.packed + a.off.w_s3[2], wf2, acc2_a, wave, lane, false);
            __syncthreads();
            store_tiles_split_q<CB, LQH2, 4, 1>(act, bias1, acc_b, wave, lane);
            if (wave == 7) {
                const int n = lane & 15;
#pragma unroll
                for (int i = 2; i < 4; ++i) split_store_tile_q<LQH2, 1>(base, LQH2::at(0, (i - 2) * 16 + n + 1), 0, bias1, acc_a[i], lane >> 4);
            }
            s3_prefetch_w0<NW, CB, 2 * CB, 8, 2, 1, TERMS>(a.packed + a.off.w_s3[2], wf2, wave, lane);
            __syncthreads();
            conv3x3_mfma_s3q<NW, CB, 2 * CB, LQH2, 2, 2, 1>(act, a.packed + a.off.w_s3[2], wf2, acc2_b, wave, lane, false);
        }
        CNN_STAMP(5);
        S3W<1> wf3, wf4;
        f32x4 bias3[1], bias4[1];
        __syncthreads();
        zero_halo_q<LQ2, NTHR>(act);
        store_tiles_split_q<2 * CB, LQ2, 2, 1, 8>(act, bias2, acc2_a, wave, lane, 0);
        store_tiles_split_q<2 * CB, LQ2, 2, 1, 8>(act, bias2, acc2_b, wave, lane, 8);
        s3_prefetch_w0<NW, 2 * CB, 2 * CB, 16, 4, 1, TERMS>(a.packed + a.off.w_s3[3], wf3, wave, lane);
        prefetch_bias_fresh<NW, 16, 4, 1>(a.packed + a.off.b[3], bias3, wave, lane);
        __syncthreads();
        CNN_STAMP(6);
        {
            f32x4 acc_[4][1];
            conv3x3_mfma_s3q<NW, 2 * CB, 2 * CB, LQ2, 1, 4, 1>(act, a.packed + a.off.w_s3[3], wf3, acc_, wave, lane, false);
            CNN_STAMP(7);
            __syncthreads();
            store_tiles_split_q<2 * CB, LQ2, 4, 1>(act, bias3, acc_, wave, lane);
            s3_prefetch_w0<NW, 2 * CB, 4 * CB, 4, 2, 1, TERMS>(a.packed + a.off.w_s3[4], wf4, wave, lane);
            prefetch_bias_fresh<NW, 8, 2, 1>(a.packed + a.off.b[4], bias4, wave, lane);
            __syncthreads();
            CNN_STAMP(8);
        }
        S3W<T4N> wf5;
        f32x4 bias5s[T4N];
        {
            f32x4 acc_[2][1];
            conv3x3_mfma_s3q<NW, 2 * CB, 4 * CB, LQ2, 2, 2, 1>(act, a.packed + a.off.w_s3[4], wf4, acc_, wave, lane, false);
            CNN_STAMP(9);
            __syncthreads();
            zero_halo_q<LQ4, NTHR>(act);
            store_tiles_split_q<4 * CB, LQ4, 2, 1>(act, bias4, acc_, wave, lane);
            s3_prefetch_w0<NW, 4 * CB, 4 * CB, 4, T4M, T4N, TERMS>(a.packed + a.off.w_s3[5], wf5, wave, lane);
            prefetch_bias_fresh<NW, 8, T4M, T4N>(a.packed + a.off.b[5], bias5s, wave, lane);
            __syncthreads();
            CNN_STAMP(10);
        }
        f32x4 acc5[T4M][T4N];
        conv3x3_mfma_s3q<NW, 4 * CB, 4 * CB, LQ4, 1, T4M, T4N>(act, a.packed + a.off.w_s3[5], wf5, acc5, wave, lane, false);
        CNN_STAMP(11);
        int lane_h = lane;
        asm volatile("" : "+v"(lane_h));
        if constexpr (KIND == AFFNET_NET_ORINET)
            head_partials_ori_lds<T4M, NTHR>(a.packed + a.off.head_w, bias5s, acc5, a.out + pidx * HEAD_PART_ORI, act, wave, lane_h, tid);
        else
            head_partials<T4M>(a.packed + a.off.head_w, bias5s, acc5, a.out + pidx * HEAD_PART_AFF, wave, lane_h);
        CNN_STAMP(13);
    }
}
```

affnet_amd/csrc/cnn_trunk_hardnet_poly.hip:

```cpp
#include "cnn_trunk.h"

__global__ __launch_bounds__(256) void poly_derive_u_kernel(const float* __restrict__ packed, int w2, int w4, float* __restrict__ U) {
    int e = blockIdx.x * 256 + threadIdx.x;
    if (e >= Poly32::PAIRS) return;
    const int l = e >= 32 * 64 ? 4 : 2;
    const int cin = 16 * l, cout = 32 * l;
    const float* src = packed + (l == 4 ? w4 : w2);
    float* dst = U + Poly32::offset(l);
    e -= l == 4 ? 32 * 64 : 0;
    const int n = (e >> 2) % cout, c = (e >> 2) / cout * 4 + (e & 3);
    float g[9], u[POLY_XI];
#pragma unroll
    for (int t = 0; t < 9; ++t) g[t] = src[w_tap_index(t, c, n, cin, cout)];
    poly_weight_transform(g, u);
#pragma unroll
    for (int xi = 0; xi < POLY_XI; ++xi) dst[w_tap_index(xi, c, n, cin, cout)] = u[xi];
}

int aff_poly_u_ensure(affnet_ctx* ctx) {
    if (ctx->poly_u) return AFFNET_OK;
    AFF_HIP(ctx, hipMalloc((void**)&ctx->poly_u, (size_t)Poly32::FLOATS * sizeof(float)));
    return AFFNET_OK;
}

int aff_poly_derive_u(affnet_ctx* ctx, const float* packed, const NetLayout& L, hipStream_t st, const float** u) {
    const int rc = aff_poly_u_ensure(ctx);
    if (rc) return rc;
    hipLaunchKernelGGL(poly_derive_u_kernel, dim3((Poly32::PAIRS + 255) / 256), dim3(256), 0, st, packed, (int)L.w_off[2], (int)L.w_off[4], ctx->poly_u);
    AFF_LAUNCH_CHECK(ctx);
    *u = ctx->poly_u;
    return AFFNET_OK;
}

TrunkKernel aff_trunk_hardnet_poly(bool stamps) {
    static const TrunkKernel k[2] = {cnn32_trunk_kernel<AFFNET_NET_HARDNET, 8, false, 1>, cnn32_trunk_kernel<AFFNET_NET_HARDNET, 8, true, 1>};
    return k[stamps];
}
```

affnet_amd/csrc/common.h:

```cpp
#pragma once
#include <hip/hip_runtime.h>
#include <stdint.h>
#include <stdio.h>
#include <string.h>

#include <string>
#include <vector>

#include "../../include/affnet_hip.h"
#include "../../include/affnet_hip_debug.h"
#include "weights_layout.h"

#define AFF_WAVE 64

enum {
    CNT_RAW0 = 0,
    CNT_CAND = AFFNET_MAX_OCTAVES,
    CNT_OVERFLOW,
    CNT_SEL,
    CNT_EQ_TAKEN,
    CNT_SEL_MODE,
    CNT_SEL_THRESH,
    CNT_SEL_NEED_EQ,
    CNT_DET,
    CNT_SHAPED,
    CNT_SURVIVED,
    CNT_CAND2,
    CNT_AFF_EVAL,
    CNT_SURVIVED1,
    CNT_SEL_EQ_TOTAL,
    CNT_SEL_TIE_LO, CNT_SEL_TIE_HI,
    CNT_AFF_REEVAL,
    CNT_POS0 = AFFNET_MAX_OCTAVES + 24,
    CNT_HYP0 = AFFNET_MAX_OCTAVES + 24 + (AFFNET_MAX_LEVELS - 2) * AFFNET_MAX_OCTAVES,
    CNT_TOTAL = AFFNET_MAX_OCTAVES + 24 + (AFFNET_MAX_LEVELS - 2) * AFFNET_MAX_OCTAVES + 8 * AFFNET_MAX_OCTAVES
};

#define OVF_FRAMES_COUNT 16
#define OVF_FRAMES_NONFINITE 32

#define SEL_HIST_BINS 2048

struct RawMax {
    int32_t pix;
    int32_t lvl;
    float val;
    float s, y, x;
    float prev[2];
};

struct OctaveGeom {
    int32_t h, w;
    int64_t pyr_off;
    int64_t map_off;
    int64_t raw_off;
    int32_t raw_cap;
};

struct affnet_ctx {
    int device = 0;
    affnet_config cfg;
    int B = 1;
    size_t pyr_stride = 0;
    size_t map_stride = 0;
    size_t raw_stride = 0;
    std::string err;
    OctaveGeom oct[AFFNET_MAX_OCTAVES];
    size_t off_pyr = 0, off_map = 0, off_raw = 0, off_cnt = 0, off_hist = 0, off_cand = 0, off_sel = 0, off_stage = 0;
    size_t off_affmap = 0, off_dense = 0, off_cand2 = 0, off_lvltab = 0;
    size_t aff_stride = 0;
    size_t aff_off[AFFNET_MAX_OCTAVES] = {0};
    size_t dense_stride = 0;
    float* affmap = nullptr; float* dense = nullptr;
    float* cand2_resp = nullptr; float* cand2_syx = nullptr; int32_t* cand2_ids = nullptr;
    int32_t* lvltab = nullptr;
    size_t ws_bytes = 0;
    size_t pyr_floats = 0, map_bytes = 0, raw_total = 0, cand_cap = 0;
    int cap_pre = 0, cap_final = 0;
    char* ws = nullptr;
    float* pyr = nullptr;
    uint8_t* omap = nullptr;
    RawMax* raw = nullptr;
    int32_t* cnt = nullptr;
    uint32_t* sel_hist = nullptr;
    float* cand_resp = nullptr; float* cand_syx = nullptr; int32_t* cand_ids = nullptr;
    float* sel_resp = nullptr; float* sel_syx = nullptr; int32_t* sel_ids = nullptr;
    float* st_det_resp = nullptr; float* st_det_lafs = nullptr; int32_t* st_det_ids = nullptr;
    int32_t* st_det_count = nullptr;
    float* st_A = nullptr; float* st_key = nullptr; int32_t* st_good = nullptr;
    float* st_A2 = nullptr; float* st_lafs_iter = nullptr;
    float* st_R = nullptr; float* st_lafs_norm = nullptr; int32_t* st_lvl_ids = nullptr;
    float* st_hard_scratch = nullptr;
    float* st_lafs_shaped = nullptr;
    int32_t* st_rank = nullptr;
    bool prof_on = false;
    std::vector<hipEvent_t> prof_ev;
    int prof_calls = 0;
    unsigned long long* dbg_time = nullptr;
    int shape_form = AFFNET_SHAPE_FORM_WINOGRAD;
    int arith = AFFNET_ARITH_FP32_MFMA;
    int split3_variant = 0;
    hipGraph_t graph = nullptr;
    hipGraphExec_t graph_exec = nullptr;
    float* wino_u = nullptr;
    float* poly_u = nullptr;
    int desc_form = AFFNET_DESC_FORM_POLYPHASE;
    ~affnet_ctx() {
        if (wino_u) (void)hipFree(wino_u);
        if (poly_u) (void)hipFree(poly_u);
        if (graph_exec) (void)hipGraphExecDestroy(graph_exec);
        if (graph) (void)hipGraphDestroy(graph);
        for (auto& e : prof_ev) (void)hipEventDestroy(e);
    }
};

struct AffDeviceGuard {
    int prev = -1;
    bool switched = false;
    explicit AffDeviceGuard(const affnet_ctx* ctx) {
        if (!ctx) return;
        if (hipGetDevice(&prev) != hipSuccess) { (void)hipGetLastError(); prev = -1; return; }
        if (prev != ctx->device) switched = hipSetDevice(ctx->device) == hipSuccess;
    }
    ~AffDeviceGuard() {
        if (switched) (void)hipSetDevice(prev);
    }
    AffDeviceGuard(const AffDeviceGuard&) = delete;
    AffDeviceGuard& operator=(const AffDeviceGuard&) = delete;
};
#define AFF_DEVICE(ctx) AffDeviceGuard aff_device_guard_(ctx)

#define PROF_RING 256
#define PROF_EVENTS (AFFNET_PROFILE_STAGES + 2)

#define AFF_HIP(ctx, expr)                                                                         \
    do {                                                                                           \
        hipError_t e_ = (expr);                                                                    \
        if (e_ != hipSuccess)                                                                      \
            return aff_fail(ctx, AFFNET_ERR_HIP, "%s failed: %s (%s:%d)", #expr, hipGetErrorString(e_), \
                            __FILE__, __LINE__);                                                   \
    } while (0)

#define AFF_LAUNCH_CHECK(ctx)                                                                      \
    do {                                                                                           \
        hipError_t e_ = hipGetLastError();                                                         \
        if (e_ != hipSuccess)                                                                      \
            return aff_fail(ctx, AFFNET_ERR_HIP, "kernel launch failed: %s (%s:%d)",                \
                            hipGetErrorString(e_), __FILE__, __LINE__);                            \
    } while (0)

struct AffZeroSegs {
    unsigned char* p[8];
    size_t bytes[8];
    int n = 0;
    bool overflow = false;
    void add(void* ptr, size_t nbytes) {
        if (!ptr || !nbytes) return;
        if (n >= 8) { overflow = true; return; }
        p[n] = (unsigned char*)ptr; bytes[n] = nbytes; ++n;
    }
};

static inline size_t aff_align(size_t x, size_t a = 256) { return (x + a - 1) / a * a; }
static inline int aff_cdiv(int a, int b) { return (a + b - 1) / b; }

struct PyrTable {
    const float* lvl[AFFNET_MAX_OCTAVES][AFFNET_MAX_LEVELS];
    int h[AFFNET_MAX_OCTAVES], w[AFFNET_MAX_OCTAVES];
    int n_octaves, n_levels;
    size_t img_stride;
};

struct LevelTable { double sig[AFFNET_MAX_OCTAVES * AFFNET_MAX_LEVELS]; int n_oct, n_lvl; };
struct DenormSel {
    float* out_px; int32_t* ids; float* lafs_norm;
    float c_a, c_x, c_y, ps, ca, cx, cy;
    LevelTable lt;
};


#define HEAD_PART_AFF 32
#define HEAD_PART_ORI 144
#define HEAD_KSPLIT 4
#define HEAD_KC 128
#define HEAD_AS (HEAD_KC + 4)

struct PyrSrc {
    PyrTable t;
    float base[32];
};

struct CnnArgs {
    const float* packed;
    NetOffsets off;
    const float* wino_u;
    const int32_t* reeval;
    const float* patches;
    const float* lafs;
    const int32_t* ids;
    const int32_t* count;
    int n_max;
    float* out;
    int dbg_layer;
    int s3_alt;
    float* dbg_out;
    unsigned long long* dbg_time;
    int row_begin;
    const int32_t* skip_cnt;
    int skip_n;
    int32_t* shape_cnt;
    int shape_op;
};

__device__ __forceinline__ bool lazy_skip(const int32_t* skip_cnt, int skip_n, int image, int which = CNT_SURVIVED1) {
    if (!skip_cnt) return false;
    const int32_t* c = skip_cnt + (size_t)image * CNT_TOTAL;
    return c[CNT_SEL_MODE] == 1 && c[which] >= skip_n;
}

struct Wino16 {
    static constexpr int U1 = 16 * 16 * 16, U3 = 16 * 32 * 32, U5 = 16 * 64 * 64, FLOATS = U1 + U3 + U5;
    static constexpr int PAIRS = 16 * 16 + 32 * 32 + 64 * 64;
    static constexpr int NB1 = 2, NB3 = 1;
    static constexpr int offset(int layer) { return layer == 1 ? 0 : (layer == 3 ? U1 : U1 + U3); }
    static constexpr int floats(int layer) { return layer == 1 ? U1 : (layer == 3 ? U3 : U5); }
};

struct ShapeFuse {
    const float* resp; const float* lafs; float* key; int32_t* good; int32_t* cnt;
};

struct CnnCall {
    int kind = -1;
    const float* packed = nullptr;
    const float* patches = nullptr;
    const float* lafs = nullptr; const int32_t* ids = nullptr;
    const int32_t* count = nullptr; int n_max = 0;
    float* out = nullptr; float* scratch = nullptr;
    hipStream_t st = nullptr;
    int dbg_layer = -1; float* dbg_out = nullptr;
    bool mark_head = false;
    int row_begin = 0, row_count = -1;
    const int32_t* skip_cnt = nullptr; int skip_n = 0;
    const ShapeFuse* fuse = nullptr; int shape_op = 0;
    bool poly = false;
    bool wino_reeval = false;
    float* rot_lafs = nullptr; const DenormSel* denorm = nullptr;
};

typedef void (*TrunkKernel)(CnnArgs, PyrSrc);

int aff_fail(affnet_ctx* ctx, int code, const char* fmt, ...);
int aff_zero_async(affnet_ctx* ctx, void* dst, size_t bytes, hipStream_t st);
int aff_zero_multi_async(affnet_ctx* ctx, const AffZeroSegs& z, hipStream_t st);
int aff_copy_async(affnet_ctx* ctx, void* dst, const void* src, size_t bytes, hipStream_t st);
int aff_copy2d_async(affnet_ctx* ctx, void* dst, size_t dpitch, const void* src, size_t spitch, size_t width_bytes, size_t rows, hipStream_t st);
void aff_base_grid(int ps, float* base);

void aff_prof_mark(affnet_ctx* ctx, int idx, hipStream_t st);

int aff_detect_impl(affnet_ctx* ctx, const float* d_responses, float* d_resp, float* d_lafs, int32_t* d_ids, int32_t* d_count, void* stream);
int aff_detect_onepass_impl(affnet_ctx* ctx, const float* d_packed_fullconv, const float* d_responses, hipStream_t st);

int aff_fullconv_launch(affnet_ctx* ctx, const float* packed, const float* img, size_t img_stride, int h, int w, float* out, size_t out_stride,
                        float* scratch, size_t scratch_stride, int B, hipStream_t st);

int aff_handcrafted_launch(affnet_ctx* ctx, int kind, const float* patches, const float* lafs, const int32_t* ids, const int32_t* count,
                           int n_max, const float* h_weights, float* out, float* out_angle, hipStream_t st);

void aff_fill_pyr_table(const affnet_ctx* ctx, PyrTable* t);
int aff_shape_select(affnet_ctx* ctx, const float* d_resp_in, const float* d_lafs_in, const int32_t* d_ids_in, const float* d_A,
                     const int32_t* d_count_in, float* d_resp_out, float* d_lafs_out, int32_t* d_ids_out, int32_t* d_count_out, hipStream_t st);
int aff_shape_iterate(affnet_ctx* ctx, const float* A, float* base, const float* lafs, const int32_t* count, int mode, float* lafs_out,
                      hipStream_t st);
void aff_denorm_sel_fill(affnet_ctx* ctx, int ps, float* d_lafs_px, int32_t* d_ids, float* d_lafs_norm, DenormSel* ds);
int aff_denorm_level_select(affnet_ctx* ctx, const float* d_lafs_norm_in, float* d_lafs_px, const int32_t* d_count, int n_max, int ps, int32_t* d_ids,
                            float* d_lafs_norm, hipStream_t st);

int aff_arith_index(const affnet_ctx* ctx);
int aff_affnet_filter_rows(affnet_ctx* ctx, const float* packed, const float* resp, const float* lafs, const int32_t* ids, const int32_t* count,
                           float* out, float* scratch, int row_begin, int row_count, bool lazy, int shape_op, hipStream_t st);
int aff_orinet_rotate(affnet_ctx* ctx, const float* packed, float* lafs, const int32_t* ids, const int32_t* count, int n_max, float* out, float* scratch,
                      hipStream_t st, const DenormSel* denorm);
int aff_hardnet_forward_pyr_marked(affnet_ctx* ctx, const float* packed, const float* lafs, const int32_t* ids, const int32_t* count,
                                   int n_max, float* out, float* scratch, hipStream_t st);

int aff_hardnet_poly_patches(affnet_ctx* ctx, const float* packed, const float* patches, int n, float* out, float* scratch, int dbg_layer, hipStream_t st);

TrunkKernel aff_trunk_affnet(int arith_index, bool stamps);
TrunkKernel aff_trunk_affnet_wino(bool stamps);
TrunkKernel aff_trunk_orinet(int arith_index, bool stamps);
TrunkKernel aff_trunk_hardnet(int arith_index, bool stamps);
TrunkKernel aff_trunk_hardnet_poly(bool stamps);
int aff_poly_u_ensure(affnet_ctx* ctx);
int aff_poly_derive_u(affnet_ctx* ctx, const float* packed, const NetLayout& L, hipStream_t st, const float** u);
int aff_wino_u_ensure(affnet_ctx* ctx);
int aff_wino_derive_u(affnet_ctx* ctx, int kind, const float* packed, const NetLayout& L, hipStream_t st, const float** u);

int aff_finish_affnet(affnet_ctx* ctx, const CnnCall& c, const NetLayout& L, int rows, int B);
int aff_margin_affnet(affnet_ctx* ctx, const CnnCall& c, const NetLayout& L, int rows, int B, int32_t* flags);
int aff_finish_orinet(affnet_ctx* ctx, const CnnCall& c, const NetLayout& L, int rows, int B);
int aff_hardnet_head(affnet_ctx* ctx, const CnnCall& c, const NetLayout& L, int B);

struct AffTile {
    int x0, y0, tw, th;
};

__device__ __forceinline__ AffTile aff_tile_box(float t00, float t01, float t02, float t10, float t11, float t12, int ps, int cap) {
    const float um = (float)(ps - 1) / (float)ps;
    const float hx = (fabsf(t00) + fabsf(t01)) * um, hy = (fabsf(t10) + fabsf(t11)) * um;
    const float cx = t02 - 0.5f, cy = t12 - 0.5f;
    AffTile t;
    t.tw = 0; t.th = 0; t.x0 = 0; t.y0 = 0;
    if (!(hx < 4096.0f && hy < 4096.0f && fabsf(cx) < 1.0e6f && fabsf(cy) < 1.0e6f)) return t;
    const int x0 = (int)floorf(cx - hx) - 1, x1 = (int)floorf(cx + hx) + 2;
    const int y0 = (int)floorf(cy - hy) - 1, y1 = (int)floorf(cy + hy) + 2;
    const int tw = x1 - x0 + 1, th = y1 - y0 + 1;
    if (tw * th > cap || tw * th > 2 * ps * ps) return t;
    t.x0 = x0; t.y0 = y0; t.tw = tw; t.th = th;
    return t;
}

template <int NTHR>
__device__ __forceinline__ void aff_tile_load(float* tile, const AffTile t, const float* __restrict__ img, int h, int w, int tid) {
    const int n = t.tw * t.th;
    for (int i = tid; i < n; i += NTHR) {
        const int ty = i / t.tw, tx = i - ty * t.tw;
        const int gy = t.y0 + ty, gx = t.x0 + tx;
        tile[i] = (gy >= 0 && gy < h && gx >= 0 && gx < w) ? img[(size_t)gy * w + gx] : 0.0f;
    }
}

__device__ __forceinline__ float aff_sample_bilinear(const float* __restrict__ img, int h, int w,
                                                     float t00, float t01, float t02, float t10,
                                                     float t11, float t12, float u, float v) {
    float gx = fmaf(1.0f, t02, fmaf(v, t01, u * t00));
    float gy = fmaf(1.0f, t12, fmaf(v, t11, u * t10));
    const float fw = (float)w, fh = (float)h;
    gx = 2.0f * gx / fw - 1.0f;
    gy = 2.0f * gy / fh - 1.0f;
    const float ix = fmaf(gx + 1.0f, fw * 0.5f, -0.5f);
    const float iy = fmaf(gy + 1.0f, fh * 0.5f, -0.5f);
    const float x0f = floorf(ix), y0f = floorf(iy);
    const float x1f = x0f + 1.0f, y1f = y0f + 1.0f;
    const float wx1 = ix - x0f, wx0 = x1f - ix, wy1 = iy - y0f, wy0 = y1f - iy;
    const float nw = wx0 * wy0, ne = wx1 * wy0, sw = wx0 * wy1, se = wx1 * wy1;
    const float cx0 = fminf(fmaxf(x0f, -2.0f), fw + 1.0f), cy0 = fminf(fmaxf(y0f, -2.0f), fh + 1.0f);
    const int x0 = (int)cx0, y0 = (int)cy0, x1 = x0 + 1, y1 = y0 + 1;
    const bool xin0 = (x0 >= 0) & (x0 < w), xin1 = (x1 >= 0) & (x1 < w);
    const bool yin0 = (y0 >= 0) & (y0 < h), yin1 = (y1 >= 0) & (y1 < h);
    const float vnw = (xin0 & yin0) ? img[(size_t)y0 * w + x0] : 0.0f;
    const float vne = (xin1 & yin0) ? img[(size_t)y0 * w + x1] : 0.0f;
    const float vsw = (xin0 & yin1) ? img[(size_t)y1 * w + x0] : 0.0f;
    const float vse = (xin1 & yin1) ? img[(size_t)y1 * w + x1] : 0.0f;
    return fmaf(vse, se, fmaf(vsw, sw, fmaf(vne, ne, vnw * nw)));
}

__device__ __forceinline__ float aff_sample_bilinear_tile(const float* tile, const AffTile tl, const float* __restrict__ img, int h, int w,
                                                          float t00, float t01, float t02, float t10, float t11, float t12, float u, float v) {
    float gx = fmaf(1.0f, t02, fmaf(v, t01, u * t00));
    float gy = fmaf(1.0f, t12, fmaf(v, t11, u * t10));
    const float fw = (float)w, fh = (float)h;
    gx = 2.0f * gx / fw - 1.0f;
    gy = 2.0f * gy / fh - 1.0f;
    const float ix = fmaf(gx + 1.0f, fw * 0.5f, -0.5f);
    const float iy = fmaf(gy + 1.0f, fh * 0.5f, -0.5f);
    const float x0f = floorf(ix), y0f = floorf(iy);
    const float x1f = x0f + 1.0f, y1f = y0f + 1.0f;
    const float wx1 = ix - x0f, wx0 = x1f - ix, wy1 = iy - y0f, wy0 = y1f - iy;
    const float nw = wx0 * wy0, ne = wx1 * wy0, sw = wx0 * wy1, se = wx1 * wy1;
    const float cx0 = fminf(fmaxf(x0f, -2.0f), fw + 1.0f), cy0 = fminf(fmaxf(y0f, -2.0f), fh + 1.0f);
    const int x0 = (int)cx0, y0 = (int)cy0;
    const int lx = x0 - tl.x0, ly = y0 - tl.y0;
    float vnw, vne, vsw, vse;
    if (lx >= 0 && ly >= 0 && lx + 1 < tl.tw && ly + 1 < tl.th) {
        const float* p = tile + ly * tl.tw + lx;
        vnw = p[0]; vne = p[1]; vsw = p[tl.tw]; vse = p[tl.tw + 1];
    } else {
        const int x1 = x0 + 1, y1 = y0 + 1;
        const bool xin0 = (x0 >= 0) & (x0 < w), xin1 = (x1 >= 0) & (x1 < w);
        const bool yin0 = (y0 >= 0) & (y0 < h), yin1 = (y1 >= 0) & (y1 < h);
        vnw = (xin0 & yin0) ? img[(size_t)y0 * w + x0] : 0.0f;
        vne = (xin1 & yin0) ? img[(size_t)y0 * w + x1] : 0.0f;
        vsw = (xin0 & yin1) ? img[(size_t)y1 * w + x0] : 0.0f;
        vse = (xin1 & yin1) ? img[(size_t)y1 * w + x1] : 0.0f;
    }
    return fmaf(vse, se, fmaf(vsw, sw, fmaf(vne, ne, vnw * nw)));
}
```

affnet_amd/csrc/context.hip:

```cpp
#include <stdarg.h>

#include "common.h"

int aff_fail(affnet_ctx* ctx, int code, const char* fmt, ...) {
    char buf[1024];
    va_list ap;
    va_start(ap, fmt);
    vsnprintf(buf, sizeof(buf), fmt, ap);
    va_end(ap);
    if (ctx) ctx->err = buf;
    return code;
}

__global__ __launch_bounds__(256) void aff_zero_kernel(unsigned char* __restrict__ p, size_t bytes) {
    const size_t head = ((16 - ((size_t)p & 15)) & 15) < bytes ? ((16 - ((size_t)p & 15)) & 15) : bytes;
    const size_t n16 = (bytes - head) / 16, tail0 = head + n16 * 16;
    uint4* q = reinterpret_cast<uint4*>(p + head);
    for (size_t i = (size_t)blockIdx.x * 256 + threadIdx.x; i < n16; i += (size_t)gridDim.x * 256) q[i] = make_uint4(0u, 0u, 0u, 0u);
    if (blockIdx.x == 0) {
        for (size_t i = threadIdx.x; i < head; i += 256) p[i] = 0;
        for (size_t i = tail0 + threadIdx.x; i < bytes; i += 256) p[i] = 0;
    }
}

__global__ __launch_bounds__(256) void aff_zero_multi_kernel(AffZeroSegs z) {
    unsigned char* p = z.p[blockIdx.y];
    const size_t bytes = z.bytes[blockIdx.y];
    const size_t head = ((16 - ((size_t)p & 15)) & 15) < bytes ? ((16 - ((size_t)p & 15)) & 15) : bytes;
    const size_t n16 = (bytes - head) / 16, tail0 = head + n16 * 16;
    uint4* q = reinterpret_cast<uint4*>(p + head);
    for (size_t i = (size_t)blockIdx.x * 256 + threadIdx.x; i < n16; i += (size_t)gridDim.x * 256) q[i] = make_uint4(0u, 0u, 0u, 0u);
    if (blockIdx.x == 0) {
        for (size_t i = threadIdx.x; i < head; i += 256) p[i] = 0;
        for (size_t i = tail0 + threadIdx.x; i < bytes; i += 256) p[i] = 0;
    }
}

int aff_zero_multi_async(affnet_ctx* ctx, const AffZeroSegs& z, hipStream_t st) {
    if (z.overflow) return aff_fail(ctx, AFFNET_ERR_INVALID, "internal: more than 8 areas in one fused clear (AffZeroSegs)");
    if (z.n <= 0) return AFFNET_OK;
    size_t blocks = 1;
    for (int i = 0; i < z.n; ++i) {
        const size_t b = (z.bytes[i] / 16 + 255) / 256;
        blocks = b > blocks ? b : blocks;
    }
    blocks = blocks > 2048 ? 2048 : blocks;
    hipLaunchKernelGGL(aff_zero_multi_kernel, dim3((unsigned)blocks, (unsigned)z.n), dim3(256), 0, st, z);
    AFF_LAUNCH_CHECK(ctx);
    return AFFNET_OK;
}

__global__ __launch_bounds__(256) void aff_copy2d_kernel(uint32_t* __restrict__ dst, size_t dpitch_w, const uint32_t* __restrict__ src, size_t spitch_w,
                                                         size_t width_w) {
    const uint32_t* s = src + (size_t)blockIdx.y * spitch_w;
    uint32_t* d = dst + (size_t)blockIdx.y * dpitch_w;
    for (size_t i = (size_t)blockIdx.x * 256 + threadIdx.x; i < width_w; i += (size_t)gridDim.x * 256) d[i] = s[i];
}

int aff_zero_async(affnet_ctx* ctx, void* dst, size_t bytes, hipStream_t st) {
    if (!dst || bytes == 0) return AFFNET_OK;
    size_t blocks = (bytes / 16 + 255) / 256;
    blocks = blocks < 1 ? 1 : (blocks > 4096 ? 4096 : blocks);
    hipLaunchKernelGGL(aff_zero_kernel, dim3((unsigned)blocks), dim3(256), 0, st, (unsigned char*)dst, bytes);
    AFF_LAUNCH_CHECK(ctx);
    return AFFNET_OK;
}

int aff_copy2d_async(affnet_ctx* ctx, void* dst, size_t dpitch, const void* src, size_t spitch, size_t width_bytes, size_t rows, hipStream_t st) {
    if (rows == 0 || width_bytes == 0) return AFFNET_OK;
    if (!dst || !src || ((size_t)dst & 3) || ((size_t)src & 3) || (dpitch & 3) || (spitch & 3) || (width_bytes & 3) || rows > 65535)
        return aff_fail(ctx, AFFNET_ERR_INVALID, "copy2d: pointers, pitches and width must be multiples of 4 bytes, rows <= 65535");
    size_t bx = (width_bytes / 4 + 255) / 256;
    bx = bx < 1 ? 1 : (bx > 2048 ? 2048 : bx);
    hipLaunchKernelGGL(aff_copy2d_kernel, dim3((unsigned)bx, (unsigned)rows), dim3(256), 0, st, (uint32_t*)dst, dpitch / 4, (const uint32_t*)src, spitch / 4,
                       width_bytes / 4);
    AFF_LAUNCH_CHECK(ctx);
    return AFFNET_OK;
}

int aff_copy_async(affnet_ctx* ctx, void* dst, const void* src, size_t bytes, hipStream_t st) {
    return aff_copy2d_async(ctx, dst, bytes, src, bytes, bytes, 1, st);
}

extern "C" const char* affnet_version(void) { return "affnet_hip 0.2 (gfx950, hipcc, fp32 MFMA 16x16x4)"; }

extern "C" const char* affnet_last_error(const affnet_ctx* ctx) { return ctx ? ctx->err.c_str() : "null context"; }

void aff_base_grid(int ps, float* base) {
    if (ps == 1) { base[0] = 0.0f; return; }
    const float step = 2.0f / (float)(ps - 1);
    const int half = ps / 2;
    for (int i = 0; i < ps; ++i) {
        float v = (i < half) ? fmaf(step, (float)i, -1.0f) : fmaf(-step, (float)(ps - 1 - i), 1.0f);
        base[i] = (v * (float)(ps - 1)) / (float)ps;
    }
}

extern "C" int affnet_host_base_grid(int ps, float* out) {
    if (ps < 1 || !out) return AFFNET_ERR_INVALID;
    aff_base_grid(ps, out);
    return AFFNET_OK;
}

static int validate(affnet_ctx* ctx, const affnet_config* c) {
    if (c->height < 8 || c->width < 8) return aff_fail(ctx, AFFNET_ERR_INVALID, "image %dx%d too small", c->height, c->width);
    if (c->batch > 4096) return aff_fail(ctx, AFFNET_ERR_INVALID, "batch=%d (max 4096)", c->batch);
    if (c->arith < AFFNET_ARITH_FP32_MFMA || c->arith > AFFNET_ARITH_FP32_SPLIT2H) return aff_fail(ctx, AFFNET_ERR_INVALID, "arith=%d (AFFNET_ARITH_*)", c->arith);
    if (c->n_octaves < 1 || c->n_octaves > AFFNET_MAX_OCTAVES) return aff_fail(ctx, AFFNET_ERR_INVALID, "n_octaves=%d", c->n_octaves);
    if (c->levels_per_octave < 3 || c->levels_per_octave > AFFNET_MAX_LEVELS)
        return aff_fail(ctx, AFFNET_ERR_INVALID, "levels_per_octave=%d", c->levels_per_octave);
    if (c->oct_h[0] != c->height || c->oct_w[0] != c->width) return aff_fail(ctx, AFFNET_ERR_INVALID, "octave 0 size mismatch");
    for (int o = 1; o < c->n_octaves; ++o)
        if (c->oct_h[o] != (c->oct_h[o - 1] - 1) / 2 + 1 || c->oct_w[o] != (c->oct_w[o - 1] - 1) / 2 + 1)
            return aff_fail(ctx, AFFNET_ERR_INVALID, "octave %d size is not ceil(prev/2)", o);
    if (c->first_blur_taps != 0 && (c->first_blur_taps % 2 == 0 || c->first_blur_taps > AFFNET_MAX_TAPS))
        return aff_fail(ctx, AFFNET_ERR_INVALID, "first_blur_taps=%d", c->first_blur_taps);
    for (int l = 1; l < c->levels_per_octave; ++l)
        if (c->level_blur_taps[l] % 2 == 0 || c->level_blur_taps[l] < 1 || c->level_blur_taps[l] > AFFNET_MAX_TAPS)
            return aff_fail(ctx, AFFNET_ERR_INVALID, "level_blur_taps[%d]=%d", l, c->level_blur_taps[l]);
    if (c->level_blur0_taps[1] != 0)
        for (int l = 1; l < c->levels_per_octave; ++l)
            if (c->level_blur0_taps[l] % 2 == 0 || c->level_blur0_taps[l] < 1 || c->level_blur0_taps[l] > AFFNET_MAX_TAPS)
                return aff_fail(ctx, AFFNET_ERR_INVALID, "level_blur0_taps[%d]=%d", l, c->level_blur0_taps[l]);
    return AFFNET_OK;
}

extern "C" int affnet_ctx_create(affnet_ctx** out, int device, const affnet_config* cfg) {
    if (!out) return AFFNET_ERR_INVALID;
    affnet_ctx* ctx = new affnet_ctx();
    ctx->device = device;
    if (!cfg) {
        memset(&ctx->cfg, 0, sizeof(ctx->cfg));
        *out = ctx;
        return AFFNET_OK;
    }
    ctx->cfg = *cfg;
    ctx->arith = cfg->arith;
    int rc = validate(ctx, cfg);
    if (rc != AFFNET_OK) { *out = ctx; return rc; }
    const affnet_config& c = ctx->cfg;
    const int div = c.max_raw_per_octave_div > 0 ? c.max_raw_per_octave_div : 4;
    size_t pyr = 0, mapb = 0, raw = 0;
    for (int o = 0; o < c.n_octaves; ++o) {
        OctaveGeom& g = ctx->oct[o];
        g.h = c.oct_h[o]; g.w = c.oct_w[o];
        g.pyr_off = (int64_t)pyr; pyr += (size_t)c.levels_per_octave * g.h * g.w;
        g.map_off = (int64_t)mapb; mapb += aff_align((size_t)g.h * g.w, 16);
        int cap = (int)((size_t)g.h * g.w / div); if (cap < 256) cap = 256;
        g.raw_off = (int64_t)raw; g.raw_cap = cap; raw += cap;
    }
    ctx->B = c.batch > 0 ? c.batch : 1;
    const size_t B = (size_t)ctx->B;
    ctx->pyr_floats = pyr; ctx->map_bytes = mapb; ctx->raw_total = raw; ctx->cand_cap = raw;
    ctx->pyr_stride = aff_align(pyr * sizeof(float)) / sizeof(float);
    ctx->map_stride = aff_align(mapb);
    ctx->raw_stride = raw;
    const int keep = c.max_keep > 0 ? c.max_keep : 65536;
    ctx->cap_pre = c.num_prefilter > 0 ? c.num_prefilter : keep;
    ctx->cap_final = c.num_features > 0 ? c.num_features : ctx->cap_pre;
    if (ctx->cap_final > ctx->cap_pre) ctx->cap_final = ctx->cap_pre;
    size_t off = 0;
    ctx->off_pyr = off; off += B * ctx->pyr_stride * sizeof(float);
    ctx->off_map = off; off += B * ctx->map_stride;
    ctx->off_raw = off; off += aff_align(B * raw * sizeof(RawMax));
    ctx->off_cnt = off; off += aff_align(B * CNT_TOTAL * sizeof(int32_t));
    ctx->off_hist = off; off += aff_align(B * SEL_HIST_BINS * sizeof(uint32_t));
    ctx->off_cand = off; off += aff_align(B * ctx->cand_cap * 7 * sizeof(float));
    ctx->off_sel = off; off += aff_align(B * (size_t)ctx->cap_pre * 7 * sizeof(float));
    ctx->off_stage = off;
    const size_t P = B * (size_t)ctx->cap_pre, F = B * (size_t)ctx->cap_final;
    off += aff_align(P * 10 * sizeof(float));
    off += aff_align(P * 4 * sizeof(float));
    off += aff_align(P * 10 * sizeof(float));
    off += aff_align(P * 2 * sizeof(float));
    off += aff_align(P * sizeof(int32_t));
    off += aff_align(B * sizeof(int32_t));
    off += aff_align(F * 6 * sizeof(float));
    off += aff_align(F * 4 * sizeof(float));
    off += aff_align(F * 9 * sizeof(float));
    {
        const size_t hard = F * (8192 + 4 * 128), aff = P * 144;
        off += aff_align((hard > aff ? hard : aff) * sizeof(float));
    }
    if (c.onepass) {
        if (c.num_prefilter != c.num_features) { *out = ctx; return aff_fail(ctx, AFFNET_ERR_INVALID, "onepass: num_prefilter must equal num_features"); }
        size_t aff = 0;
        for (int o = 0; o < c.n_octaves; ++o) {
            if (c.oct_h[o] < 34 || c.oct_w[o] < 34) {
                *out = ctx;
                return aff_fail(ctx, AFFNET_ERR_INVALID, "onepass: octave %d is %dx%d, LocalNorm2d(33) needs >= 34 px in this library (17 in the reference: use "
                                "border >= 15 like its scripts, so that the pyramid stops earlier)", o, c.oct_w[o], c.oct_h[o]);
            }
            ctx->aff_off[o] = aff; aff += aff_align((size_t)4 * c.oct_h[o] * c.oct_w[o] * sizeof(float)) / sizeof(float);
        }
        ctx->aff_stride = aff;
        ctx->dense_stride = affnet_fullconv_scratch_bytes(c.oct_h[0], c.oct_w[0]) / sizeof(float);
        ctx->off_affmap = off; off += aff_align(B * aff * sizeof(float));
        ctx->off_dense = off; off += aff_align(B * ctx->dense_stride * sizeof(float));
        ctx->off_cand2 = off; off += aff_align(B * ctx->cand_cap * 7 * sizeof(float));
        ctx->off_lvltab = off; off += aff_align(B * (size_t)AFFNET_MAX_OCTAVES * AFFNET_MAX_LEVELS * 4 * sizeof(int32_t));
    }
    ctx->ws_bytes = off;
    *out = ctx;
    return AFFNET_OK;
}

extern "C" void affnet_ctx_destroy(affnet_ctx* ctx) { delete ctx; }

extern "C" int affnet_set_arith(affnet_ctx* ctx, int arith) {
    if (!ctx) return AFFNET_ERR_INVALID;
    if (arith < AFFNET_ARITH_FP32_MFMA || arith > AFFNET_ARITH_FP32_SPLIT2H) return aff_fail(ctx, AFFNET_ERR_INVALID, "arith=%d (AFFNET_ARITH_*)", arith);
    ctx->arith = arith;
    ctx->cfg.arith = arith;
    return AFFNET_OK;
}
extern "C" int affnet_get_arith(const affnet_ctx* ctx) { return ctx ? ctx->arith : AFFNET_ERR_INVALID; }

extern "C" int affnet_set_shape_form(affnet_ctx* ctx, int form) {
    if (!ctx) return AFFNET_ERR_INVALID;
    if (form != AFFNET_SHAPE_FORM_DIRECT && form != AFFNET_SHAPE_FORM_WINOGRAD) return aff_fail(ctx, AFFNET_ERR_INVALID, "shape form=%d (AFFNET_SHAPE_FORM_*)", form);
    ctx->shape_form = form;
    return AFFNET_OK;
}
extern "C" int affnet_get_shape_form(const affnet_ctx* ctx) { return ctx ? ctx->shape_form : AFFNET_ERR_INVALID; }

extern "C" int affnet_set_desc_form(affnet_ctx* ctx, int form) {
    if (!ctx) return AFFNET_ERR_INVALID;
    if (form != AFFNET_DESC_FORM_DIRECT && form != AFFNET_DESC_FORM_POLYPHASE) return aff_fail(ctx, AFFNET_ERR_INVALID, "descriptor form=%d (AFFNET_DESC_FORM_*)", form);
    ctx->desc_form = form;
    return AFFNET_OK;
}
extern "C" int affnet_get_desc_form(const affnet_ctx* ctx) { return ctx ? ctx->desc_form : AFFNET_ERR_INVALID; }

extern "C" size_t affnet_workspace_bytes(const affnet_ctx* ctx) { return ctx ? ctx->ws_bytes : 0; }

extern "C" int affnet_capacity_prefilter(const affnet_ctx* ctx) { return ctx ? ctx->cap_pre : 0; }
extern "C" int affnet_capacity_final(const affnet_ctx* ctx) { return ctx ? ctx->cap_final : 0; }

extern "C" int64_t affnet_pyramid_level_offset(const affnet_ctx* ctx, int octave, int level) {
    if (!ctx || octave < 0 || octave >= ctx->cfg.n_octaves || level < 0 || level >= ctx->cfg.levels_per_octave) return -1;
    const OctaveGeom& g = ctx->oct[octave];
    return (int64_t)(ctx->off_pyr / sizeof(float)) + g.pyr_off + (int64_t)level * g.h * g.w;
}

extern "C" int64_t affnet_pyramid_image_stride(const affnet_ctx* ctx) { return ctx ? (int64_t)ctx->pyr_stride : 0; }

extern "C" int64_t affnet_counter_offset(const affnet_ctx* ctx, int which) {
    if (!ctx || ctx->ws_bytes == 0 || which < 0 || which > 4) return -1;
    const int idx = which == 0 ? CNT_OVERFLOW : (which == 1 ? CNT_DET : (which == 2 ? CNT_SHAPED : (which == 3 ? CNT_AFF_EVAL : CNT_AFF_REEVAL)));
    return (int64_t)(ctx->off_cnt / sizeof(int32_t)) + idx;
}
extern "C" int64_t affnet_counter_stride(const affnet_ctx* ctx) { return ctx ? (int64_t)CNT_TOTAL : 0; }

extern "C" int64_t affnet_affmap_offset(const affnet_ctx* ctx, int octave) {
    if (!ctx || !ctx->cfg.onepass || octave < 0 || octave >= ctx->cfg.n_octaves) return -1;
    return (int64_t)(ctx->off_affmap / sizeof(float)) + (int64_t)ctx->aff_off[octave];
}
extern "C" int64_t affnet_affmap_image_stride(const affnet_ctx* ctx) { return (ctx && ctx->cfg.onepass) ? (int64_t)ctx->aff_stride : 0; }
extern "C" int affnet_batch(const affnet_ctx* ctx) { return ctx ? ctx->B : 0; }

extern "C" int affnet_bind_workspace(affnet_ctx* ctx, void* d_workspace, size_t bytes) {
    if (!ctx) return AFFNET_ERR_INVALID;
    if (!d_workspace || bytes < ctx->ws_bytes)
        return aff_fail(ctx, AFFNET_ERR_INVALID, "workspace too small: %zu < %zu", bytes, ctx->ws_bytes);
    if (((uintptr_t)d_workspace & 255) != 0) return aff_fail(ctx, AFFNET_ERR_INVALID, "workspace must be 256-byte aligned");
    {
        hipPointerAttribute_t at;
        if (hipPointerGetAttributes(&at, d_workspace) == hipSuccess) {
            if (at.type == hipMemoryTypeDevice && at.device != ctx->device)
                return aff_fail(ctx, AFFNET_ERR_INVALID, "workspace belongs to device %d, the context to device %d", at.device, ctx->device);
        } else {
            (void)hipGetLastError();
        }
    }
    char* b = (char*)d_workspace;
    ctx->ws = b;
    ctx->pyr = (float*)(b + ctx->off_pyr);
    ctx->omap = (uint8_t*)(b + ctx->off_map);
    ctx->raw = (RawMax*)(b + ctx->off_raw);
    ctx->cnt = (int32_t*)(b + ctx->off_cnt);
    ctx->sel_hist = (uint32_t*)(b + ctx->off_hist);
    const size_t B = (size_t)ctx->B;
    float* cand = (float*)(b + ctx->off_cand);
    const size_t CC = B * ctx->cand_cap;
    ctx->cand_resp = cand; ctx->cand_syx = cand + CC; ctx->cand_ids = (int32_t*)(cand + 4 * CC);
    float* sel = (float*)(b + ctx->off_sel);
    const size_t P = B * (size_t)ctx->cap_pre, F = B * (size_t)ctx->cap_final;
    ctx->sel_resp = sel; ctx->sel_syx = sel + P; ctx->sel_ids = (int32_t*)(sel + 4 * P);
    char* s = b + ctx->off_stage;
    ctx->st_det_resp = (float*)s; ctx->st_det_lafs = (float*)s + P; ctx->st_det_ids = (int32_t*)((float*)s + 7 * P);
    s += aff_align(P * 10 * sizeof(float));
    ctx->st_A = (float*)s; s += aff_align(P * 4 * sizeof(float));
    ctx->st_A2 = (float*)s; ctx->st_lafs_iter = (float*)s + 4 * P; s += aff_align(P * 10 * sizeof(float));
    ctx->st_key = (float*)s; ctx->st_good = (int32_t*)((float*)s + P); s += aff_align(P * 2 * sizeof(float));
    ctx->st_rank = (int32_t*)s; s += aff_align(P * sizeof(int32_t));
    ctx->st_det_count = (int32_t*)s; s += aff_align(B * sizeof(int32_t));
    ctx->st_lafs_shaped = (float*)s; s += aff_align(F * 6 * sizeof(float));
    ctx->st_R = (float*)s; s += aff_align(F * 4 * sizeof(float));
    ctx->st_lafs_norm = (float*)s; ctx->st_lvl_ids = (int32_t*)((float*)s + 6 * F); s += aff_align(F * 9 * sizeof(float));
    ctx->st_hard_scratch = (float*)s;
    if (ctx->cfg.onepass) {
        ctx->affmap = (float*)(b + ctx->off_affmap);
        ctx->dense = (float*)(b + ctx->off_dense);
        float* c2 = (float*)(b + ctx->off_cand2);
        ctx->cand2_resp = c2; ctx->cand2_syx = c2 + CC; ctx->cand2_ids = (int32_t*)(c2 + 4 * CC);
        ctx->lvltab = (int32_t*)(b + ctx->off_lvltab);
    }
    return AFFNET_OK;
}

extern "C" int affnet_read_counts(affnet_ctx* ctx, int32_t out[4], void* stream) {
    AFF_DEVICE(ctx);
    if (!ctx || !ctx->ws) return AFFNET_ERR_INVALID;
    std::vector<int32_t> all((size_t)ctx->B * CNT_TOTAL);
    AFF_HIP(ctx, hipMemcpyAsync(all.data(), ctx->cnt, all.size() * sizeof(int32_t), hipMemcpyDeviceToHost, (hipStream_t)stream));
    AFF_HIP(ctx, hipStreamSynchronize((hipStream_t)stream));
    int32_t host[CNT_TOTAL];
    memset(host, 0, sizeof(host));
    int raw = 0;
    for (int b = 0; b < ctx->B; ++b) {
        const int32_t* h = all.data() + (size_t)b * CNT_TOTAL;
        host[CNT_DET] += h[CNT_DET]; host[CNT_SHAPED] += h[CNT_SHAPED]; host[CNT_OVERFLOW] |= h[CNT_OVERFLOW];
        for (int o = 0; o < ctx->cfg.n_octaves; ++o) raw += h[CNT_RAW0 + o];
    }
    out[0] = host[CNT_DET]; out[1] = host[CNT_SHAPED]; out[2] = host[CNT_OVERFLOW];
    out[3] = raw;
    if (host[CNT_OVERFLOW] & OVF_FRAMES_NONFINITE)
        return aff_fail(ctx, AFFNET_ERR_INVALID, "load_frames: a caller-supplied frame or response was not finite (stored as a zero row; flag %d)",
                        host[CNT_OVERFLOW]);
    if (host[CNT_OVERFLOW]) return aff_fail(ctx, AFFNET_ERR_CAPACITY, "a fixed-capacity detector list overflowed (flag %d)", host[CNT_OVERFLOW]);
    if (host[CNT_DET] == 0)
        return aff_fail(ctx, AFFNET_ERR_EMPTY, "no keypoints detected in %d image(s) (the reference raises in torch.cat, SparseImgRepresenter.py:100)", ctx->B);
    return AFFNET_OK;
}
```

affnet_amd/csrc/debug.hip:

```cpp
#include "common.h"

#include "../../include/affnet_hip_probes.h"

template <typename T>
__global__ __launch_bounds__(256) void stream_read_kernel(const T* __restrict__ src, float* __restrict__ dst, size_t n_items) {
    float acc = 0.f;
    for (size_t i = (size_t)blockIdx.x * 256 + threadIdx.x; i < n_items; i += (size_t)gridDim.x * 256) {
        const T v = src[i];
        const float* f = reinterpret_cast<const float*>(&v);
#pragma unroll
        for (int k = 0; k < (int)(sizeof(T) / 4); ++k) acc += f[k];
    }
    if (acc == 123.456f) dst[blockIdx.x] = acc;
    if (threadIdx.x == 0 && blockIdx.x == 0) dst[0] = acc;
}

template <typename T>
__global__ __launch_bounds__(256) void stream_write_kernel(T* __restrict__ dst, size_t n_items) {
    T v;
    float* f = reinterpret_cast<float*>(&v);
#pragma unroll
    for (int k = 0; k < (int)(sizeof(T) / 4); ++k) f[k] = (float)(threadIdx.x + k);
    for (size_t i = (size_t)blockIdx.x * 256 + threadIdx.x; i < n_items; i += (size_t)gridDim.x * 256) dst[i] = v;
}

__global__ __launch_bounds__(256) void tile_read_kernel(const float* __restrict__ img, float* __restrict__ dst, int h, int w, int halo) {
    const int LW = 64 + 2 * halo, n_el = LW * LW;
    const int x0 = blockIdx.x * 64, y0 = blockIdx.y * 64;
    float acc = 0.f;
    for (int i = threadIdx.x; i < n_el; i += 256) {
        const int ty = i / LW, tx = i - ty * LW;
        int gy = y0 + ty - halo, gx = x0 + tx - halo;
        gy = gy < 0 ? 0 : (gy >= h ? h - 1 : gy);
        gx = gx < 0 ? 0 : (gx >= w ? w - 1 : gx);
        acc += img[(size_t)gy * w + gx];
    }
    if (acc == 123.456f) dst[blockIdx.x] = acc;
}

struct f32x2s { float a, b; };

extern "C" int affnet_debug_stream(const void* d_src, void* d_dst, size_t n_bytes, int width, int mode, int halo, void* stream) {
    if (!d_dst || n_bytes == 0 || (n_bytes & 65535) != 0) return AFFNET_ERR_INVALID;
    hipStream_t st = (hipStream_t)stream;
    const int blocks = 256 * 16;
    if (mode == 0) {
        if (!d_src) return AFFNET_ERR_INVALID;
        if (width == 4) hipLaunchKernelGGL(stream_read_kernel<float>, dim3(blocks), dim3(256), 0, st, (const float*)d_src, (float*)d_dst, n_bytes / 4);
        else if (width == 8) hipLaunchKernelGGL(stream_read_kernel<f32x2s>, dim3(blocks), dim3(256), 0, st, (const f32x2s*)d_src, (float*)d_dst, n_bytes / 8);
        else if (width == 16) hipLaunchKernelGGL(stream_read_kernel<float4>, dim3(blocks), dim3(256), 0, st, (const float4*)d_src, (float*)d_dst, n_bytes / 16);
        else return AFFNET_ERR_INVALID;
    } else if (mode == 1) {
        if (width == 4) hipLaunchKernelGGL(stream_write_kernel<float>, dim3(blocks), dim3(256), 0, st, (float*)d_dst, n_bytes / 4);
        else if (width == 8) hipLaunchKernelGGL(stream_write_kernel<f32x2s>, dim3(blocks), dim3(256), 0, st, (f32x2s*)d_dst, n_bytes / 8);
        else if (width == 16) hipLaunchKernelGGL(stream_write_kernel<float4>, dim3(blocks), dim3(256), 0, st, (float4*)d_dst, n_bytes / 16);
        else return AFFNET_ERR_INVALID;
    } else if (mode == 2) {
        if (!d_src || halo < 0 || halo > 16) return AFFNET_ERR_INVALID;
        const int w = 4096, h = (int)(n_bytes / 4 / w);
        hipLaunchKernelGGL(tile_read_kernel, dim3(w / 64, (h + 63) / 64), dim3(256), 0, st, (const float*)d_src, (float*)d_dst, h, w, halo);
    } else {
        return AFFNET_ERR_INVALID;
    }
    return hipGetLastError() == hipSuccess ? AFFNET_OK : AFFNET_ERR_HIP;
}

extern "C" int affnet_probe_shape_offsets(const affnet_ctx* ctx, int64_t out[3]) {
    if (!ctx || !ctx->ws || !out) return AFFNET_ERR_INVALID;
    out[0] = (int64_t)(reinterpret_cast<const char*>(ctx->st_A) - ctx->ws) / 4;
    out[1] = (int64_t)(reinterpret_cast<const char*>(ctx->st_hard_scratch) - ctx->ws) / 4 + (int64_t)ctx->B * ctx->cap_pre * HEAD_PART_AFF;
    out[2] = (int64_t)(reinterpret_cast<const char*>(ctx->st_det_lafs) - ctx->ws) / 4;
    return AFFNET_OK;
}

static int probe_affnet_wino(affnet_ctx* ctx, const float* d_packed, const float* d_patches, int n, float* d_out, int layer, hipStream_t st) {
    if (ctx->arith != AFFNET_ARITH_FP32_MFMA) return aff_fail(ctx, AFFNET_ERR_INVALID, "probe_affnet_wino: AFFNET_ARITH_FP32_MFMA only");
    const NetLayout L = net_layout(AFFNET_NET_AFFNET);
    CnnArgs a;
    memset(&a, 0, sizeof(a));
    a.packed = d_packed; a.off = to_offsets(L, ctx->arith);
    const int rc = aff_wino_derive_u(ctx, AFFNET_NET_AFFNET, d_packed, L, st, &a.wino_u);
    if (rc) return rc;
    a.patches = d_patches; a.n_max = n; a.out = d_out; a.dbg_layer = layer; a.dbg_out = d_out; a.dbg_time = ctx->dbg_time;
    PyrSrc ps;
    memset(&ps, 0, sizeof(ps));
    hipLaunchKernelGGL(aff_trunk_affnet_wino(layer >= 0 || a.dbg_time), dim3(n, 1), dim3(512), 0, st, a, ps);
    AFF_LAUNCH_CHECK(ctx);
    return AFFNET_OK;
}

extern "C" int affnet_probe_affnet_wino_layer(affnet_ctx* ctx, int net_kind, const float* d_packed, const float* d_patch, int layer, float* d_out, void* stream) {
    AFF_DEVICE(ctx);
    if (!ctx || !d_packed || !d_patch || !d_out || net_kind != AFFNET_NET_AFFNET || layer < 0 || layer > 5)
        return aff_fail(ctx, AFFNET_ERR_INVALID, "probe_affnet_wino_layer: AffNet, layer 0 .. 5");
    return probe_affnet_wino(ctx, d_packed, d_patch, 1, d_out, layer, (hipStream_t)stream);
}

extern "C" int affnet_probe_affnet_wino_partials(affnet_ctx* ctx, const float* d_packed, const float* d_patches, int n, float* d_partials, void* stream) {
    AFF_DEVICE(ctx);
    if (!ctx || !d_packed || !d_patches || !d_partials || n < 1 || n > 65535) return aff_fail(ctx, AFFNET_ERR_INVALID, "probe_affnet_wino_partials: bad argument");
    return probe_affnet_wino(ctx, d_packed, d_patches, n, d_partials, -1, (hipStream_t)stream);
}

extern "C" int affnet_probe_hardnet_poly_layer(affnet_ctx* ctx, const float* d_packed, const float* d_patch, int layer, float* d_out, void* stream) {
    AFF_DEVICE(ctx);
    if (!ctx || !d_packed || !d_patch || !d_out || layer < 0 || layer > 5) return aff_fail(ctx, AFFNET_ERR_INVALID, "probe_hardnet_poly_layer: layer 0 .. 5");
    return aff_hardnet_poly_patches(ctx, d_packed, d_patch, 1, d_out, nullptr, layer, (hipStream_t)stream);
}

extern "C" int affnet_probe_hardnet_poly_forward(affnet_ctx* ctx, const float* d_packed, const float* d_patches, int n, float* d_out, float* d_scratch, void* stream) {
    AFF_DEVICE(ctx);
    if (!ctx || !d_packed || !d_patches || !d_out || !d_scratch || n < 1 || n > 65535) return aff_fail(ctx, AFFNET_ERR_INVALID, "probe_hardnet_poly_forward: bad argument");
    return aff_hardnet_poly_patches(ctx, d_packed, d_patches, n, d_out, d_scratch, -1, (hipStream_t)stream);
}

extern "C" int affnet_probe_hardnet_poly_u(affnet_ctx* ctx, const float* d_packed, int layer, float* d_out, void* stream) {
    AFF_DEVICE(ctx);
    if (!ctx || !d_packed || !d_out || (layer != 2 && layer != 4)) return aff_fail(ctx, AFFNET_ERR_INVALID, "probe_hardnet_poly_u: layer 2 or 4");
    const float* u;
    const int rc = aff_poly_derive_u(ctx, d_packed, net_layout(AFFNET_NET_HARDNET), (hipStream_t)stream, &u);
    if (rc) return rc;
    return aff_copy_async(ctx, d_out, u + Poly32::offset(layer), (size_t)Poly32::floats(layer) * sizeof(float), (hipStream_t)stream);
}
```

affnet_amd/engine.py:

```python
import ctypes as C

import numpy as np
import torch

from . import _lib
from ._lib import lib, check, ptr
from .host_plan import PyramidPlan

_UTILITY = {}


def require_cuda(t, what="tensor"):
    if not (isinstance(t, torch.Tensor) and t.is_cuda):
        raise RuntimeError("affnet_amd: %s must live on the MI355X (tensor.cuda()); this implementation has no CPU path" % what)


def utility_ctx(device, arith=0):
    idx = device.index if device.index is not None else torch.cuda.current_device()
    key = (idx, _lib.arith_code(arith))
    if key not in _UTILITY:
        h = C.c_void_p()
        check(lib.affnet_ctx_create(C.byref(h), idx, None), None, "affnet_ctx_create(utility)")
        check(lib.affnet_set_arith(h, key[1]), h, "affnet_set_arith")
        _UTILITY[key] = h
    h = _UTILITY[key]
    if lib.affnet_get_arith(h) != key[1]:
        check(lib.affnet_set_arith(h, key[1]), h, "affnet_set_arith")
    return h


def stream_of(device):
    return C.c_void_p(torch.cuda.current_stream(device).cuda_stream)


class Context(object):

    def __init__(self, height, width, device, n_levels, init_sigma, border, mr_size, threshold,
                 num_features, num_prefilter, max_keep=16384, batch=1, baum_iters=0, raw_div=4, onepass=False, lazy_shape_rows=-1, arith=0):
        self.plan = PyramidPlan(height, width, n_levels, init_sigma, border)
        self.batch = int(batch)
        self.onepass = bool(onepass)
        self.cfg = self.plan.fill_config(mr_size, threshold, num_features, num_prefilter, max_keep, raw_div=raw_div, batch=self.batch, baum_iters=baum_iters,
                                         onepass=onepass, lazy_shape_rows=lazy_shape_rows, arith=arith)
        self.arith = _lib.arith_code(arith)
        self.shape_form = _lib.SHAPE_FORM_WINOGRAD
        self.desc_form = _lib.DESC_FORM_POLYPHASE
        self.device = device
        self.handle = C.c_void_p()
        idx = device.index if device.index is not None else torch.cuda.current_device()
        rc = lib.affnet_ctx_create(C.byref(self.handle), idx, C.byref(self.cfg))
        check(rc, self.handle, "affnet_ctx_create")
        nbytes = lib.affnet_workspace_bytes(self.handle)
        self.workspace = torch.empty(nbytes, dtype=torch.uint8, device=device)
        check(lib.affnet_bind_workspace(self.handle, ptr(self.workspace), nbytes), self.handle, "affnet_bind_workspace")
        self.cap_pre = lib.affnet_capacity_prefilter(self.handle)
        self.cap_final = lib.affnet_capacity_final(self.handle)
        self._ws_f32 = self.workspace.view(torch.float32)

    def set_arith(self, arith):
        self.arith = _lib.arith_code(arith)
        check(lib.affnet_set_arith(self.handle, self.arith), self.handle, "affnet_set_arith")

    def set_shape_form(self, form):
        check(lib.affnet_set_shape_form(self.handle, int(form)), self.handle, "affnet_set_shape_form")
        self.shape_form = int(form)

    def set_desc_form(self, form):
        check(lib.affnet_set_desc_form(self.handle, int(form)), self.handle, "affnet_set_desc_form")
        self.desc_form = int(form)

    def pyramid_views(self, image=0):
        pyr = []
        base = image * lib.affnet_pyramid_image_stride(self.handle)
        for o, (h, w) in enumerate(self.plan.sizes):
            levels = []
            for l in range(self.plan.levels_per_octave):
                off = base + lib.affnet_pyramid_level_offset(self.handle, o, l)
                levels.append(self._ws_f32[off:off + h * w].view(1, 1, h, w))
            pyr.append(levels)
        return pyr

    def affmap_views(self, image=0):
        base = image * lib.affnet_affmap_image_stride(self.handle)
        out = []
        for o, (h, w) in enumerate(self.plan.sizes):
            off = base + lib.affnet_affmap_offset(self.handle, o)
            out.append(self._ws_f32[off:off + 4 * h * w].view(1, 4, h, w))
        return out

    def counter_view(self, which=0):
        off, stride = lib.affnet_counter_offset(self.handle, which), lib.affnet_counter_stride(self.handle)
        return self.workspace.view(torch.int32)[off:off + stride * self.batch:stride]

    def read_counts(self, allow_empty=False):
        out = (C.c_int32 * 4)()
        rc = lib.affnet_read_counts(self.handle, C.byref(out), stream_of(self.device))
        if not (allow_empty and rc == _lib.ERR_EMPTY):
            check(rc, self.handle, "affnet_read_counts")
        return list(out)

    def __del__(self):
        try:
            if self.handle:
                lib.affnet_ctx_destroy(self.handle)
                self.handle = None
        except Exception:
            pass


def pack_state_dict(kind, sd, winograd=False):
    conv_idx, bn_idx = (0, 3, 6, 9, 12, 15), (1, 4, 7, 10, 13, 16)

    def f32(name):
        return sd[name].detach().to("cpu", torch.float32).contiguous()

    keep = []
    convs = [f32("features.%d.weight" % i) for i in conv_idx]
    means = [f32("features.%d.running_mean" % i) for i in bn_idx]
    vars_ = [f32("features.%d.running_var" % i) for i in bn_idx]
    head_w = f32("features.19.weight")
    head_b = f32("features.19.bias") if "features.19.bias" in sd else None
    if kind == _lib.NET_AFFNET_FULLCONV and head_b is None:
        raise ValueError("AffNetFastFullConv: features.19.bias missing from the state dict")
    hbm = f32("features.20.running_mean") if kind == _lib.NET_HARDNET else None
    hbv = f32("features.20.running_var") if kind == _lib.NET_HARDNET else None
    keep += convs + means + vars_ + [head_w, head_b, hbm, hbv]
    arr = lambda ts: (C.c_void_p * 6)(*[t.data_ptr() for t in ts])
    n = lib.affnet_cnn32_packed_floats(kind)
    out = torch.empty(n, dtype=torch.float32)
    rc = lib.affnet_cnn32_pack_weights(kind, arr(convs), arr(means), arr(vars_), ptr(head_w), ptr(head_b), ptr(hbm), ptr(hbv), ptr(out))
    check(rc, None, "affnet_cnn32_pack_weights")
    del keep
    if not winograd:
        offs = [lib.affnet_cnn32_winograd_offset(kind, i) for i in range(6)]
        offs = [o for o in offs if o >= 0]
        if offs:
            out = out[:min(offs)].clone()
    return out


def save_flat_weights(kind, sd, path):
    conv_idx, bn_idx = (0, 3, 6, 9, 12, 15), (1, 4, 7, 10, 13, 16)
    names = ["features.%d.weight" % i for i in conv_idx] + ["features.%d.running_mean" % i for i in bn_idx] + \
            ["features.%d.running_var" % i for i in bn_idx] + ["features.19.weight"]
    names += ["features.20.running_mean", "features.20.running_var"] if kind == _lib.NET_HARDNET else ["features.19.bias"]
    flat = np.concatenate([sd[n].detach().to("cpu", torch.float32).contiguous().numpy().reshape(-1) for n in names])
    with open(path, "wb") as f:
        f.write(b"AFNW0001")
        f.write(np.array([kind, flat.size], dtype=np.int32).tobytes())
        f.write(flat.astype(np.float32).tobytes())
    return flat.size


def cnn_forward(kind, packed, patches, scratch=None, arith=0):
    require_cuda(patches, "patches")
    if patches.dim() == 4:
        if patches.size(1) != 1:
            raise ValueError("expected single-channel patches")
        patches = patches[:, 0]
    if tuple(patches.shape[1:]) != (32, 32):
        raise ValueError("the HIP CNN kernels are specialised for 32x32 patches, got %s" % (tuple(patches.shape),))
    patches = patches.contiguous().float()
    if packed.numel() != lib.affnet_cnn32_packed_floats(kind):
        raise ValueError("packed blob of %d floats, the kernels of net kind %d read %d (pack_state_dict(..., winograd=True))"
                         % (packed.numel(), kind, lib.affnet_cnn32_packed_floats(kind)))
    n = patches.size(0)
    dev = patches.device
    out = torch.empty((n, 128) if kind == _lib.NET_HARDNET else (n, 2, 2), dtype=torch.float32, device=dev)
    if n == 0:
        return out
    if scratch is None:
        scratch = torch.empty(n * ((8192 + 512) if kind == _lib.NET_HARDNET else 144), dtype=torch.float32, device=dev)
    ctx = utility_ctx(dev, arith)
    rc = lib.affnet_cnn32_forward(ctx, kind, ptr(packed), ptr(patches), None, n, ptr(out), ptr(scratch), stream_of(dev))
    check(rc, ctx, "affnet_cnn32_forward")
    return out


def fullconv_forward(packed, img, arith=0):
    img = img.contiguous().float()
    h, w = img.size(2), img.size(3)
    nbytes = lib.affnet_fullconv_scratch_bytes(h, w)
    if nbytes == 0:
        raise ValueError("image %dx%d too small for AffNetFastFullConv (this library requires H, W >= 34; the reference's LocalNorm2d(33) needs 17)" % (w, h))
    dev = img.device
    scratch = torch.empty(nbytes // 4, dtype=torch.float32, device=dev)
    out = torch.empty(1, 4, h, w, dtype=torch.float32, device=dev)
    ctx = utility_ctx(dev, arith)
    check(lib.affnet_fullconv_forward(ctx, ptr(packed), ptr(img), h, w, ptr(out), ptr(scratch), stream_of(dev)), ctx, "affnet_fullconv_forward")
    return out


def local_norm(img):
    require_cuda(img, "image")
    img = img.contiguous().float()
    out = torch.empty_like(img)
    ctx = utility_ctx(img.device)
    check(lib.affnet_local_norm(ctx, ptr(img), ptr(out), img.size(2), img.size(3), stream_of(img.device)), ctx, "affnet_local_norm")
    return out


def base_grid(ps):
    buf = (C.c_float * ps)()
    check(lib.affnet_host_base_grid(ps, buf), None, "affnet_host_base_grid")
    return np.array(buf, dtype=np.float32)
```

include/affnet_hip.h:

```cpp
#ifndef AFFNET_HIP_H
#define AFFNET_HIP_H

#include <stddef.h>
#include <stdint.h>

#ifdef __cplusplus
extern "C" {
#endif

#define AFFNET_OK 0
#define AFFNET_ERR_INVALID (-1)
#define AFFNET_ERR_HIP (-2)
#define AFFNET_ERR_CAPACITY (-3)
#define AFFNET_ERR_EMPTY (-4)

#define AFFNET_MAX_OCTAVES 16
#define AFFNET_MAX_LEVELS 8
#define AFFNET_MAX_TAPS 37

#define AFFNET_NET_AFFNET 0
#define AFFNET_NET_ORINET 1
#define AFFNET_NET_HARDNET 2
#define AFFNET_NET_AFFNET_FULLCONV 3

#define AFFNET_ARITH_FP32_MFMA 0
#define AFFNET_ARITH_FP32_SPLIT3 1
#define AFFNET_ARITH_FP32_SPLIT2H 2

typedef struct affnet_ctx affnet_ctx;

typedef struct affnet_config {
    int32_t height, width;
    int32_t n_octaves;
    int32_t levels_per_octave;
    int32_t oct_h[AFFNET_MAX_OCTAVES];
    int32_t oct_w[AFFNET_MAX_OCTAVES];
    float level_sigma[AFFNET_MAX_OCTAVES][AFFNET_MAX_LEVELS];
    float level_sigma4[AFFNET_MAX_OCTAVES][AFFNET_MAX_LEVELS];
    double level_sigma_px[AFFNET_MAX_OCTAVES][AFFNET_MAX_LEVELS];
    int32_t first_blur_taps;
    float first_blur[AFFNET_MAX_TAPS * AFFNET_MAX_TAPS];
    int32_t level_blur_taps[AFFNET_MAX_LEVELS];
    float level_blur[AFFNET_MAX_LEVELS][AFFNET_MAX_TAPS * AFFNET_MAX_TAPS];
    int32_t level_blur0_taps[AFFNET_MAX_LEVELS];
    float level_blur0[AFFNET_MAX_LEVELS][AFFNET_MAX_TAPS * AFFNET_MAX_TAPS];
    int32_t lazy_shape_rows;
    int32_t onepass;
    float mr_size;
    float threshold;
    int32_t num_features;
    int32_t num_prefilter;
    int32_t max_raw_per_octave_div;
    int32_t max_keep;
    int32_t batch;
    int32_t baum_iters;
    int32_t arith;
} affnet_config;

int affnet_config_fill(affnet_config* cfg, int height, int width, int n_levels, double init_sigma, int border, double mr_size,
                       double threshold, int num_features, int num_prefilter, int batch, int baum_iters);


int affnet_ctx_create(affnet_ctx** out, int device, const affnet_config* cfg);
void affnet_ctx_destroy(affnet_ctx* ctx);
const char* affnet_last_error(const affnet_ctx* ctx);
const char* affnet_version(void);
int affnet_set_arith(affnet_ctx* ctx, int arith);
int affnet_get_arith(const affnet_ctx* ctx);

#define AFFNET_SHAPE_FORM_DIRECT 0
#define AFFNET_SHAPE_FORM_WINOGRAD 1
int affnet_set_shape_form(affnet_ctx* ctx, int form);
int affnet_get_shape_form(const affnet_ctx* ctx);

#define AFFNET_DESC_FORM_DIRECT 0
#define AFFNET_DESC_FORM_POLYPHASE 1
int affnet_set_desc_form(affnet_ctx* ctx, int form);
int affnet_get_desc_form(const affnet_ctx* ctx);

size_t affnet_workspace_bytes(const affnet_ctx* ctx);
int affnet_bind_workspace(affnet_ctx* ctx, void* d_workspace, size_t bytes);
int64_t affnet_pyramid_level_offset(const affnet_ctx* ctx, int octave, int level);
int64_t affnet_pyramid_image_stride(const affnet_ctx* ctx);
int affnet_batch(const affnet_ctx* ctx);
int affnet_capacity_prefilter(const affnet_ctx* ctx);
int affnet_capacity_final(const affnet_ctx* ctx);


int affnet_gauss_blur(affnet_ctx* ctx, const float* d_in, float* d_out, int h, int w,
                      const float* h_taps, int k, void* stream);

int affnet_pyramid_build(affnet_ctx* ctx, const float* d_img, void* stream);

int affnet_hessian_response(affnet_ctx* ctx, const float* d_in, float* d_out, int h, int w,
                            float sigma4, void* stream);

int affnet_detect(affnet_ctx* ctx, float* d_resp, float* d_lafs, int32_t* d_ids,
                  int32_t* d_count, void* stream);

int affnet_detect_responses(affnet_ctx* ctx, const float* d_responses, float* d_resp, float* d_lafs, int32_t* d_ids,
                            int32_t* d_count, void* stream);

int affnet_laf_grid_sample(affnet_ctx* ctx, const float* d_img, int h, int w,
                           const float* d_lafs, int n, int ps, float* d_out, void* stream);

int affnet_pyr_grid_sample(affnet_ctx* ctx, const float* d_lafs, const int32_t* d_ids,
                           const int32_t* d_count, int n_max, int ps, float* d_out, void* stream);


size_t affnet_cnn32_packed_floats(int net_kind);
int64_t affnet_cnn32_winograd_offset(int net_kind, int layer);
int affnet_cnn32_pack_weights(int net_kind, const float* const* conv_w, const float* const* bn_mean,
                              const float* const* bn_var, const float* head_w, const float* head_b,
                              const float* head_bn_mean, const float* head_bn_var, float* h_out);

int affnet_cnn32_forward(affnet_ctx* ctx, int net_kind, const float* d_packed, const float* d_patches,
                         const int32_t* d_count, int n_max, float* d_out, float* d_scratch, void* stream);

int affnet_cnn32_forward_pyr(affnet_ctx* ctx, int net_kind, const float* d_packed, const float* d_lafs,
                             const int32_t* d_ids, const int32_t* d_count, int n_max, float* d_out,
                             float* d_scratch, void* stream);


int affnet_local_norm(affnet_ctx* ctx, const float* d_in, float* d_out, int h, int w, void* stream);

size_t affnet_fullconv_scratch_bytes(int h, int w);

int affnet_fullconv_forward(affnet_ctx* ctx, const float* d_packed, const float* d_img, int h, int w, float* d_out, float* d_scratch,
                            void* stream);

int affnet_nms2d(affnet_ctx* ctx, const float* d_in, float* d_out, int h, int w, float threshold, void* stream);


#define AFFNET_HC_ORIENTATION 0
#define AFFNET_HC_BAUMBERG 1

int affnet_handcrafted_forward(affnet_ctx* ctx, int kind, const float* d_patches, int n, const float* h_weights, float* d_out,
                               float* d_angles, void* stream);
int affnet_handcrafted_forward_pyr(affnet_ctx* ctx, int kind, const float* d_lafs, const int32_t* d_ids, const int32_t* d_count,
                                   int n_max, const float* h_weights, float* d_out, void* stream);


int affnet_sift_host_window(int patch_size, float* h_out);
int affnet_sift_forward(affnet_ctx* ctx, const float* d_patches, int n, const float* d_window, float clipval, float* d_desc, void* stream);
int affnet_sift_forward_pyr(affnet_ctx* ctx, const float* d_lafs_norm, const int32_t* d_ids, const int32_t* d_count, int n_max,
                            const float* d_window, float clipval, float* d_desc, void* stream);


size_t affnet_tfeat_packed_floats(void);
int affnet_tfeat_pack_weights(const float* conv1_w, const float* conv1_b, const float* conv2_w, const float* conv2_b, const float* cls_w,
                              const float* cls_b, float* h_out);
size_t affnet_tfeat_scratch_floats(int rows);
int affnet_tfeat_forward(affnet_ctx* ctx, const float* d_packed, const float* d_patches, const int32_t* d_count, int n_max, float* d_desc,
                         float* d_scratch, void* stream);
int affnet_tfeat_forward_pyr(affnet_ctx* ctx, const float* d_packed, const float* d_lafs_norm, const int32_t* d_ids, const int32_t* d_count,
                             int n_max, float* d_desc, float* d_scratch, void* stream);


int affnet_shape_filter_select(affnet_ctx* ctx, const float* d_resp_in, const float* d_lafs_in,
                               const int32_t* d_ids_in, const float* d_A, const int32_t* d_count_in,
                               float* d_resp_out, float* d_lafs_out, int32_t* d_ids_out,
                               int32_t* d_count_out, void* stream);

int affnet_shape_iterate(affnet_ctx* ctx, const float* d_A, float* d_base, const float* d_lafs, const int32_t* d_count, int mode,
                         float* d_lafs_out, void* stream);

int affnet_apply_rotation(affnet_ctx* ctx, float* d_lafs, const float* d_R, const int32_t* d_count,
                          int n_max, void* stream);

int affnet_scale_lafs(affnet_ctx* ctx, const float* d_in, float* d_out, const int32_t* d_count, int n_max,
                      int w, int h, int inverse, void* stream);

int affnet_lafs_to_ellipses(affnet_ctx* ctx, const float* d_lafs, const int32_t* d_count, int n_max, float* d_out, void* stream);

int affnet_ellipses_to_lafs(affnet_ctx* ctx, const float* d_ell, const int32_t* d_count, int n_max, float* d_lafs, void* stream);

int affnet_level_select(affnet_ctx* ctx, const float* d_lafs_px, const int32_t* d_count, int n_max,
                        int ps, int32_t* d_ids, float* d_lafs_norm, void* stream);


size_t affnet_match_scratch_bytes(int n1, int n2);

int affnet_distance_matrix(affnet_ctx* ctx, const float* d_desc1, int n1, const float* d_desc2, int n2, int dim, float* d_out,
                           void* d_scratch, void* stream);

int affnet_match_snn(affnet_ctx* ctx, const float* d_desc1, int n1, const float* d_desc2, int n2, int dim, float snn_threshold,
                     float* d_min_dist, int32_t* d_idx, float* d_min2_dist, int32_t* d_tent, int32_t* d_count, void* d_scratch,
                     void* stream);

int affnet_reproject_lafs(affnet_ctx* ctx, const float* d_lafs, int n, const float* h_H, float* d_out, void* stream);

int affnet_centre_nn(affnet_ctx* ctx, const float* d_query_lafs, int nq, const float* d_ref_lafs, int nr, float* d_min_dist,
                     int32_t* d_idx, void* stream);


typedef struct affnet_nets {
    const float* d_affnet;
    const float* d_orinet;
    const float* d_hardnet;
    const float* h_orientation_window;
    const float* h_baumberg_window;
} affnet_nets;

int affnet_extract_features(affnet_ctx* ctx, const affnet_nets* nets, const float* d_img, int do_ori,
                            float* d_lafs_px, float* d_resp, int32_t* d_ids, float* d_desc,
                            int32_t* d_count, void* stream);

int affnet_detect_image(affnet_ctx* ctx, const float* d_img, void* stream);
int affnet_detect_image_responses(affnet_ctx* ctx, const float* d_responses, void* stream);
int affnet_describe_detected(affnet_ctx* ctx, const affnet_nets* nets, int do_ori, float* d_lafs_px, float* d_resp,
                             int32_t* d_ids, float* d_desc, int32_t* d_count, void* stream);

int affnet_detect_image_onepass(affnet_ctx* ctx, const float* d_packed_fullconv, const float* d_img, void* stream);
int affnet_detect_image_onepass_responses(affnet_ctx* ctx, const float* d_packed_fullconv, const float* d_responses, void* stream);

int affnet_detected_list(affnet_ctx* ctx, float* d_resp, float* d_lafs, int32_t* d_ids, int32_t* d_count, void* stream);
int affnet_load_frames(affnet_ctx* ctx, const float* d_lafs, int normalised, const float* d_resp, const int32_t* d_ids,
                       const int32_t* d_count, int n_max, int ps, void* stream);

int affnet_describe_frames(affnet_ctx* ctx, const affnet_nets* nets, const float* d_img, const float* d_lafs_px, const float* d_resp_in,
                           const int32_t* d_count_in, int n_max, int do_ori, float* d_lafs_px_out, float* d_resp, int32_t* d_ids,
                           float* d_desc, int32_t* d_count, void* stream);

int64_t affnet_affmap_offset(const affnet_ctx* ctx, int octave);
int64_t affnet_affmap_image_stride(const affnet_ctx* ctx);

int affnet_graph_capture_extract(affnet_ctx* ctx, const affnet_nets* nets, const float* d_img, int do_ori, float* d_lafs_px, float* d_resp,
                                 int32_t* d_ids, float* d_desc, int32_t* d_count, void* stream);
int affnet_graph_launch(affnet_ctx* ctx, void* stream);

#define AFFNET_PROFILE_STAGES 8
int affnet_profile_enable(affnet_ctx* ctx, int on);
int affnet_profile_read(affnet_ctx* ctx, double sum_ms[AFFNET_PROFILE_STAGES], int32_t* n_calls);

int affnet_read_counts(affnet_ctx* ctx, int32_t out[4], void* stream);

int64_t affnet_counter_offset(const affnet_ctx* ctx, int which);
int64_t affnet_counter_stride(const affnet_ctx* ctx);

int affnet_host_base_grid(int ps, float* out);

#ifdef __cplusplus
}
#endif
#endif
```

include/affnet_hip_probes.h:

```cpp
#ifndef AFFNET_HIP_PROBES_H
#define AFFNET_HIP_PROBES_H

#include "affnet_hip.h"

#ifdef __cplusplus
extern "C" {
#endif

int affnet_cnn32_probe(const float* d_packed, int layer, int probe, int reps, int n_blocks, float* d_out, void* stream);

int affnet_debug_stream(const void* d_src, void* d_dst, size_t n_bytes, int width, int mode, int halo, void* stream);

int affnet_split3_gemm(const float* d_A, const float* d_Bt, int M, int N, int K, int mode, float* d_C, void* stream);
int affnet_split3_rate(int reps, int terms, int n_blocks, float* d_out, void* stream);

int affnet_probe_shape_offsets(const affnet_ctx* ctx, int64_t out[3]);

int affnet_probe_affnet_wino_layer(affnet_ctx* ctx, int net_kind, const float* d_packed, const float* d_patch, int layer, float* d_out, void* stream);

int affnet_probe_affnet_wino_partials(affnet_ctx* ctx, const float* d_packed, const float* d_patches, int n, float* d_partials, void* stream);

int affnet_probe_hardnet_poly_layer(affnet_ctx* ctx, const float* d_packed, const float* d_patch, int layer, float* d_out, void* stream);
int affnet_probe_hardnet_poly_forward(affnet_ctx* ctx, const float* d_packed, const float* d_patches, int n, float* d_out, float* d_scratch, void* stream);
int affnet_probe_hardnet_poly_u(affnet_ctx* ctx, const float* d_packed, int layer, float* d_out, void* stream);

#ifdef __cplusplus
}
#endif
#endif
```

Before: 1.614 million.

## Add polyphase conv2 to AffNet Winograd trunk and make it the default shape form

Adds a new shape form in which the AffNet trunk computes its strided conv2 with a polyphase decomposition, reusing the HardNet polyphase machinery with pre-derived transformed weights. This replaces the direct MFMA conv2 in the Winograd AffNet kernel (the same path the OriNet trunk already takes). The change extends the Winograd weight buffer and generalises the weight-derivation kernel to 16 channels, and makes the new form the default. It adds an extra small weight-derivation launch per call and changes register usage in the trunk kernel.

```diff
diff --git a/affnet_amd/SparseImgRepresenter.py b/affnet_amd/SparseImgRepresenter.py
--- a/affnet_amd/SparseImgRepresenter.py
+++ b/affnet_amd/SparseImgRepresenter.py
@@ -40,7 +40,7 @@
         self.max_keep = 16384
         self.raw_div = 4
         self.lazy_shape_rows = -1
-        self.shape_form = 1
+        self.shape_form = 2
 
         self.desc_form = 1
 
diff --git a/affnet_amd/_lib.py b/affnet_amd/_lib.py
--- a/affnet_amd/_lib.py
+++ b/affnet_amd/_lib.py
@@ -22,7 +22,7 @@
     if int(arith) not in (ARITH_FP32_MFMA, ARITH_FP32_SPLIT3, ARITH_FP32_SPLIT2H):
         raise ValueError("arith must be AFFNET_ARITH_FP32_MFMA (0), AFFNET_ARITH_FP32_SPLIT3 (1) or AFFNET_ARITH_FP32_SPLIT2H (2)")
     return int(arith)
-SHAPE_FORM_DIRECT, SHAPE_FORM_WINOGRAD = 0, 1
+SHAPE_FORM_DIRECT, SHAPE_FORM_WINOGRAD, SHAPE_FORM_POLYPHASE = 0, 1, 2
 DESC_FORM_DIRECT, DESC_FORM_POLYPHASE = 0, 1
 OK, ERR_INVALID, ERR_HIP, ERR_CAPACITY, ERR_EMPTY = 0, -1, -2, -3, -4
 
@@ -148,6 +148,8 @@
     "affnet_probe_shape_offsets": (_I, [_P, C.POINTER(C.c_int64 * 3)]),
     "affnet_probe_affnet_wino_layer": (_I, [_P, _I, _P, _P, _I, _P, _P]),
     "affnet_probe_affnet_wino_partials": (_I, [_P, _P, _P, _I, _P, _P]),
+    "affnet_probe_affnet_poly_layer": (_I, [_P, _I, _P, _P, _I, _P, _P]),
+    "affnet_probe_affnet_poly_partials": (_I, [_P, _P, _P, _I, _P, _P]),
     "affnet_probe_hardnet_poly_layer": (_I, [_P, _P, _P, _I, _P, _P]),
     "affnet_probe_hardnet_poly_forward": (_I, [_P, _P, _P, _I, _P, _P, _P]),
     "affnet_probe_hardnet_poly_u": (_I, [_P, _P, _I, _P, _P]),
diff --git a/affnet_amd/csrc/cnn32.hip b/affnet_amd/csrc/cnn32.hip
--- a/affnet_amd/csrc/cnn32.hip
+++ b/affnet_amd/csrc/cnn32.hip
@@ -28,13 +28,17 @@
     return ctx->arith == AFFNET_ARITH_FP32_SPLIT2H ? 2 : (ctx->arith == AFFNET_ARITH_FP32_SPLIT3 ? 1 : 0);
 }
 
-static int trunk_launch(affnet_ctx* ctx, const CnnCall& c, const NetLayout& L, dim3 grid, bool wino, const int32_t* reeval, int shape_op) {
+static int trunk_launch(affnet_ctx* ctx, const CnnCall& c, const NetLayout& L, dim3 grid, int wino, const int32_t* reeval, int shape_op) {
     CnnArgs a;
     a.packed = c.packed; a.off = to_offsets(L, ctx->arith);
     a.wino_u = nullptr; a.reeval = reeval;
     if ((c.kind == AFFNET_NET_ORINET || wino) && ctx->arith == AFFNET_ARITH_FP32_MFMA) {
         const int rc = aff_wino_derive_u(ctx, c.kind, c.packed, L, c.st, &a.wino_u);
         if (rc) return rc;
+        if (c.kind == AFFNET_NET_ORINET || wino == 2) {
+            const int rcp = aff_poly16_derive_u(ctx, c.kind, c.packed, L, c.st);
+            if (rcp) return rcp;
+        }
     }
     const bool poly = c.poly && c.kind == AFFNET_NET_HARDNET && ctx->arith == AFFNET_ARITH_FP32_MFMA;
     if (poly) {
@@ -52,7 +56,7 @@
     static_assert(AFFNET_NET_AFFNET == 0 && AFFNET_NET_ORINET == 1 && AFFNET_NET_HARDNET == 2, "trunk getter order");
     static TrunkKernel (*const trunk_of[3])(int, bool) = {aff_trunk_affnet, aff_trunk_orinet, aff_trunk_hardnet};
     const bool stamps = a.dbg_time || c.dbg_layer >= 0;
-    hipLaunchKernelGGL(wino ? aff_trunk_affnet_wino(stamps) : (poly ? aff_trunk_hardnet_poly(stamps) : trunk_of[c.kind](aff_arith_index(ctx), stamps)), grid, dim3(512), 0, c.st, a, ps);
+    hipLaunchKernelGGL(wino ? (wino == 2 ? aff_trunk_affnet_poly(stamps) : aff_trunk_affnet_wino(stamps)) : (poly ? aff_trunk_hardnet_poly(stamps) : trunk_of[c.kind](aff_arith_index(ctx), stamps)), grid, dim3(512), 0, c.st, a, ps);
     AFF_LAUNCH_CHECK(ctx);
     return AFFNET_OK;
 }
@@ -64,13 +68,13 @@
     const NetLayout L = net_layout(c.kind);
     const int B = c.patches ? 1 : ctx->B;
     const bool form1 = c.wino_reeval && c.kind == AFFNET_NET_AFFNET && c.fuse && c.dbg_layer < 0 && ctx->arith == AFFNET_ARITH_FP32_MFMA;
-    rc = trunk_launch(ctx, c, L, dim3(rows, B), form1, nullptr, c.shape_op);
+    rc = trunk_launch(ctx, c, L, dim3(rows, B), form1 ? (c.wino_poly ? 2 : 1) : 0, nullptr, c.shape_op);
     if (rc) return rc;
     if (form1) {
         int32_t* flags = reinterpret_cast<int32_t*>(c.scratch + (size_t)B * c.n_max * HEAD_PART_AFF);
         rc = aff_margin_affnet(ctx, c, L, rows, B, flags);
         if (rc) return rc;
-        rc = trunk_launch(ctx, c, L, dim3(rows, B), false, flags, 0);
+        rc = trunk_launch(ctx, c, L, dim3(rows, B), 0, flags, 0);
         if (rc) return rc;
     }
     if (c.dbg_layer < 0 && c.kind != AFFNET_NET_HARDNET) {
@@ -109,7 +113,8 @@
     c.row_begin = row_begin; c.row_count = row_count;
     c.skip_cnt = lazy ? ctx->cnt : nullptr; c.skip_n = ctx->cfg.num_features;
     c.fuse = &sf; c.shape_op = shape_op;
-    c.wino_reeval = ctx->shape_form == AFFNET_SHAPE_FORM_WINOGRAD;
+    c.wino_reeval = ctx->shape_form != AFFNET_SHAPE_FORM_DIRECT;
+    c.wino_poly = ctx->shape_form == AFFNET_SHAPE_FORM_POLYPHASE;
     return cnn_launch(ctx, c);
 }
 
@@ -163,10 +168,13 @@
 
 extern "C" int affnet_cnn32_debug_winograd_u(affnet_ctx* ctx, int net_kind, const float* d_packed, int layer, float* d_out, void* stream) {
     AFF_DEVICE(ctx);
-    if (!ctx || !d_packed || !d_out || (net_kind != AFFNET_NET_AFFNET && net_kind != AFFNET_NET_ORINET) || (layer != 1 && layer != 3 && layer != 5))
-        return aff_fail(ctx, AFFNET_ERR_INVALID, "cnn32_debug_winograd_u: AffNet / OriNet, layer 1, 3 or 5");
+    if (!ctx || !d_packed || !d_out || (net_kind != AFFNET_NET_AFFNET && net_kind != AFFNET_NET_ORINET) || (layer != 1 && layer != 2 && layer != 3 && layer != 5))
+        return aff_fail(ctx, AFFNET_ERR_INVALID, "cnn32_debug_winograd_u: AffNet / OriNet, layer 1, 3 or 5 (Winograd) or 2 (polyphase)");
     const float* u;
-    const int rc = aff_wino_derive_u(ctx, net_kind, d_packed, net_layout(net_kind), (hipStream_t)stream, &u);
+    int rc = aff_wino_derive_u(ctx, net_kind, d_packed, net_layout(net_kind), (hipStream_t)stream, &u);
     if (rc) return rc;
-    return aff_copy_async(ctx, d_out, u + Wino16::offset(layer), (size_t)Wino16::floats(layer) * sizeof(float), (hipStream_t)stream);
+    if (layer == 2) rc = aff_poly16_derive_u(ctx, net_kind, d_packed, net_layout(net_kind), (hipStream_t)stream);
+    if (rc) return rc;
+    return aff_copy_async(ctx, d_out, u + (layer == 2 ? Wino16::POLY_OFFSET : Wino16::offset(layer)), (size_t)(layer == 2 ? Wino16::U2 : Wino16::floats(layer)) * sizeof(float),
+                          (hipStream_t)stream);
 }
diff --git a/affnet_amd/csrc/cnn_trunk.h b/affnet_amd/csrc/cnn_trunk.h
--- a/affnet_amd/csrc/cnn_trunk.h
+++ b/affnet_amd/csrc/cnn_trunk.h
@@ -211,10 +211,11 @@
 
 template <int KIND, int NW, bool STAMPS, int S3 = 0>
 __global__ __launch_bounds__(NW * 64, (KIND == AFFNET_NET_HARDNET) ? NW / 4 : 4) void cnn32_trunk_kernel(CnnArgs a, PyrSrc ps) {
-    static_assert(S3 == 0 || S3 == 2 || S3 == 3 || (S3 == 1 && KIND != AFFNET_NET_ORINET),
-                  "S3 = number of terms of the split arithmetic; 1 = exact AffNet with Winograd conv1 / conv3 / conv5, exact HardNet with polyphase conv2 / conv4");
-    constexpr bool EXACT = S3 <= 1;
-    constexpr bool WINO13 = (S3 == 0 && KIND == AFFNET_NET_ORINET) || (S3 == 1 && KIND == AFFNET_NET_AFFNET);
+    static_assert(S3 == 0 || S3 == 2 || S3 == 3 || (S3 == 1 && KIND != AFFNET_NET_ORINET) || (S3 == 4 && KIND == AFFNET_NET_AFFNET),
+                  "S3 = number of terms of the split arithmetic; 1 = exact AffNet with Winograd conv1 / conv3 / conv5, exact HardNet with polyphase conv2 / conv4; 4 = exact AffNet with Winograd conv1 / conv3 / conv5 and polyphase conv2");
+    constexpr bool EXACT = S3 <= 1 || S3 == 4;
+    constexpr bool POLY16 = (S3 == 0 && KIND == AFFNET_NET_ORINET) || (S3 == 4 && KIND == AFFNET_NET_AFFNET);
+    constexpr bool WINO13 = POLY16 || (S3 == 1 && KIND == AFFNET_NET_AFFNET);
     constexpr bool WINO5 = WINO13;
     constexpr bool POLY = S3 == 1 && KIND == AFFNET_NET_HARDNET;
     using S = TrunkShape<KIND, NW>;
@@ -509,6 +510,7 @@
         static_assert(NW == 8 && CB == 16, "Wino16 describes the 16-channel trunks on 8 waves");
         f32x4 b4[S::G4][T4N];
         f32x4 bias4[T4N];
+        f32x4 Pa[1][3], Pb[1][3];
         if constexpr (WINO13) {
             constexpr int NB1 = Wino16::NB1, NB3 = Wino16::NB3;
             {
@@ -528,8 +530,12 @@
                 f32x4 y[NB1][4], bw[NB1];
                 conv3x3_wino_mfma_rows<NW, CB, CB, LayC0, NB1>(act, a.wino_u, Ur, y, wave, lane);
                 CNN_STAMP(3);
-                prefetch_b0<NW, 2 * CB, 16, T2M, T2N, S::G2>(a.packed + a.off.w[2], b2, wave, lane);
-                prefetch_bias<NW, 16, T2M, T2N>(a.packed + a.off.b[2], bias2, wave, lane);
+                if constexpr (POLY16) {
+                    poly_prefetch_u<NW, CB, 2 * CB, 16, 1, 1>(a.wino_u + Wino16::POLY_OFFSET, Pa, Pb, wave, lane);
+                } else {
+                    prefetch_b0<NW, 2 * CB, 16, T2M, T2N, S::G2>(a.packed + a.off.w[2], b2, wave, lane);
+                    prefetch_bias<NW, 16, T2M, T2N>(a.packed + a.off.b[2], bias2, wave, lane);
+                }
                 wino_bias<NW, 32, CB, NB1>(a.packed + a.off.b[1], bw, wave, lane);
                 __syncthreads();
                 CNN_STAMP(21);
@@ -541,7 +547,20 @@
             }
             if (STAMPS && a.dbg_layer == 1) { dump_planes<CB, LayC1, NTHR>(act, a.dbg_out); return; }
 
-            {
+            if constexpr (POLY16) {
+                f32x4 y[1][4], bw[1];
+                __builtin_amdgcn_s_setprio(1);
+                conv3x3_poly_mfma_rows<NW, CB, 2 * CB, LayC1, 1, 1>(act, a.wino_u + Wino16::POLY_OFFSET, Pa, Pb, y, wave, lane);
+                __builtin_amdgcn_s_setprio(0);
+                CNN_STAMP(5);
+                wino_prefetch_u_row<NW, 2 * CB, 2 * CB, 16, NB3>(a.wino_u + Wino16::offset(3), Ur, wave, lane);
+                wino_bias<NW, 16, 2 * CB, 1>(a.packed + a.off.b[2], bw, wave, lane);
+                __syncthreads();
+                zero_halo<LayC2, NTHR>(act, 2 * CB);
+                wino_store_lds<2 * CB, LayC2, 1>(act, bw, y, wave, lane);
+                __syncthreads();
+                CNN_STAMP(6);
+            } else {
                 f32x4 acc[T2M][T2N];
                 conv3x3_mfma<NW, CB, 2 * CB, LayC1, 2, T2M, T2N, S::G2>(act, a.packed + a.off.w[2], b2, acc, wave, lane);
                 CNN_STAMP(5);
diff --git a/affnet_amd/csrc/cnn_trunk_affnet_poly.hip b/affnet_amd/csrc/cnn_trunk_affnet_poly.hip
--- /dev/null
+++ b/affnet_amd/csrc/cnn_trunk_affnet_poly.hip
@@ -0,0 +1,5 @@
+#include "cnn_trunk.h"
+
+TrunkKernel aff_trunk_affnet_poly(bool stamps) {
+    return stamps ? cnn32_trunk_kernel<AFFNET_NET_AFFNET, 8, true, 4> : cnn32_trunk_kernel<AFFNET_NET_AFFNET, 8, false, 4>;
+}
diff --git a/affnet_amd/csrc/cnn_trunk_hardnet_poly.hip b/affnet_amd/csrc/cnn_trunk_hardnet_poly.hip
--- a/affnet_amd/csrc/cnn_trunk_hardnet_poly.hip
+++ b/affnet_amd/csrc/cnn_trunk_hardnet_poly.hip
@@ -1,13 +1,14 @@
 #include "cnn_trunk.h"
 
-__global__ __launch_bounds__(256) void poly_derive_u_kernel(const float* __restrict__ packed, int w2, int w4, float* __restrict__ U) {
+__global__ __launch_bounds__(256) void poly_derive_u_kernel(const float* __restrict__ packed, int w2, int w4, int cb, int pairs, float* __restrict__ U) {
     int e = blockIdx.x * 256 + threadIdx.x;
-    if (e >= Poly32::PAIRS) return;
-    const int l = e >= 32 * 64 ? 4 : 2;
-    const int cin = 16 * l, cout = 32 * l;
+    const int pairs2 = 2 * cb * cb;
+    if (e >= pairs) return;
+    const int l = e >= pairs2 ? 4 : 2;
+    const int cin = (cb / 2) * l, cout = cb * l;
     const float* src = packed + (l == 4 ? w4 : w2);
-    float* dst = U + Poly32::offset(l);
-    e -= l == 4 ? 32 * 64 : 0;
+    float* dst = U + (l == 4 ? POLY_XI * pairs2 : 0);
+    e -= l == 4 ? pairs2 : 0;
     const int n = (e >> 2) % cout, c = (e >> 2) / cout * 4 + (e & 3);
     float g[9], u[POLY_XI];
 #pragma unroll
@@ -26,9 +27,20 @@
 int aff_poly_derive_u(affnet_ctx* ctx, const float* packed, const NetLayout& L, hipStream_t st, const float** u) {
     const int rc = aff_poly_u_ensure(ctx);
     if (rc) return rc;
-    hipLaunchKernelGGL(poly_derive_u_kernel, dim3((Poly32::PAIRS + 255) / 256), dim3(256), 0, st, packed, (int)L.w_off[2], (int)L.w_off[4], ctx->poly_u);
+    static_assert(Poly32::PAIRS == 10 * 32 * 32 && Poly32::offset(4) == POLY_XI * 2 * 32 * 32, "poly_derive_u_kernel's sections");
+    hipLaunchKernelGGL(poly_derive_u_kernel, dim3((Poly32::PAIRS + 255) / 256), dim3(256), 0, st, packed, (int)L.w_off[2], (int)L.w_off[4], 32, Poly32::PAIRS, ctx->poly_u);
     AFF_LAUNCH_CHECK(ctx);
     *u = ctx->poly_u;
+    return AFFNET_OK;
+}
+
+int aff_poly16_derive_u(affnet_ctx* ctx, int kind, const float* packed, const NetLayout& L, hipStream_t st) {
+    const int rc = aff_wino_u_ensure(ctx);
+    if (rc) return rc;
+    static_assert(Wino16::U2 == POLY_XI * 2 * 16 * 16 && Wino16::POLY_OFFSET + Wino16::U2 == Wino16::FLOATS, "poly_derive_u_kernel's conv2 section");
+    float* dst = ctx->wino_u + (size_t)kind * Wino16::FLOATS + Wino16::POLY_OFFSET;
+    hipLaunchKernelGGL(poly_derive_u_kernel, dim3((2 * 16 * 16 + 255) / 256), dim3(256), 0, st, packed, (int)L.w_off[2], (int)L.w_off[4], 16, 2 * 16 * 16, dst);
+    AFF_LAUNCH_CHECK(ctx);
     return AFFNET_OK;
 }
 
diff --git a/affnet_amd/csrc/common.h b/affnet_amd/csrc/common.h
--- a/affnet_amd/csrc/common.h
+++ b/affnet_amd/csrc/common.h
@@ -97,7 +97,7 @@
     std::vector<hipEvent_t> prof_ev;
     int prof_calls = 0;
     unsigned long long* dbg_time = nullptr;
-    int shape_form = AFFNET_SHAPE_FORM_WINOGRAD;
+    int shape_form = AFFNET_SHAPE_FORM_POLYPHASE;
     int arith = AFFNET_ARITH_FP32_MFMA;
     int split3_variant = 0;
     hipGraph_t graph = nullptr;
@@ -219,11 +219,13 @@
 }
 
 struct Wino16 {
-    static constexpr int U1 = 16 * 16 * 16, U3 = 16 * 32 * 32, U5 = 16 * 64 * 64, FLOATS = U1 + U3 + U5;
+    static constexpr int U1 = 16 * 16 * 16, U3 = 16 * 32 * 32, U5 = 16 * 64 * 64;
+    static constexpr int U2 = POLY_XI * 16 * 32, FLOATS = U1 + U3 + U5 + U2;
     static constexpr int PAIRS = 16 * 16 + 32 * 32 + 64 * 64;
     static constexpr int NB1 = 2, NB3 = 1;
     static constexpr int offset(int layer) { return layer == 1 ? 0 : (layer == 3 ? U1 : U1 + U3); }
     static constexpr int floats(int layer) { return layer == 1 ? U1 : (layer == 3 ? U3 : U5); }
+    static constexpr int POLY_OFFSET = U1 + U3 + U5;
 };
 
 struct ShapeFuse {
@@ -245,6 +247,7 @@
     const ShapeFuse* fuse = nullptr; int shape_op = 0;
     bool poly = false;
     bool wino_reeval = false;
+    bool wino_poly = false;
     float* rot_lafs = nullptr; const DenormSel* denorm = nullptr;
 };
 
@@ -289,11 +292,13 @@
 
 TrunkKernel aff_trunk_affnet(int arith_index, bool stamps);
 TrunkKernel aff_trunk_affnet_wino(bool stamps);
+TrunkKernel aff_trunk_affnet_poly(bool stamps);
 TrunkKernel aff_trunk_orinet(int arith_index, bool stamps);
 TrunkKernel aff_trunk_hardnet(int arith_index, bool stamps);
 TrunkKernel aff_trunk_hardnet_poly(bool stamps);
 int aff_poly_u_ensure(affnet_ctx* ctx);
 int aff_poly_derive_u(affnet_ctx* ctx, const float* packed, const NetLayout& L, hipStream_t st, const float** u);
+int aff_poly16_derive_u(affnet_ctx* ctx, int kind, const float* packed, const NetLayout& L, hipStream_t st);
 int aff_wino_u_ensure(affnet_ctx* ctx);
 int aff_wino_derive_u(affnet_ctx* ctx, int kind, const float* packed, const NetLayout& L, hipStream_t st, const float** u);
 
diff --git a/affnet_amd/csrc/context.hip b/affnet_amd/csrc/context.hip
--- a/affnet_amd/csrc/context.hip
+++ b/affnet_amd/csrc/context.hip
@@ -218,7 +218,7 @@
 
 extern "C" int affnet_set_shape_form(affnet_ctx* ctx, int form) {
     if (!ctx) return AFFNET_ERR_INVALID;
-    if (form != AFFNET_SHAPE_FORM_DIRECT && form != AFFNET_SHAPE_FORM_WINOGRAD) return aff_fail(ctx, AFFNET_ERR_INVALID, "shape form=%d (AFFNET_SHAPE_FORM_*)", form);
+    if (form != AFFNET_SHAPE_FORM_DIRECT && form != AFFNET_SHAPE_FORM_WINOGRAD && form != AFFNET_SHAPE_FORM_POLYPHASE) return aff_fail(ctx, AFFNET_ERR_INVALID, "shape form=%d (AFFNET_SHAPE_FORM_*)", form);
     ctx->shape_form = form;
     return AFFNET_OK;
 }
diff --git a/affnet_amd/csrc/debug.hip b/affnet_amd/csrc/debug.hip
--- a/affnet_amd/csrc/debug.hip
+++ b/affnet_amd/csrc/debug.hip
@@ -73,18 +73,20 @@
     return AFFNET_OK;
 }
 
-static int probe_affnet_wino(affnet_ctx* ctx, const float* d_packed, const float* d_patches, int n, float* d_out, int layer, hipStream_t st) {
+static int probe_affnet_wino(affnet_ctx* ctx, const float* d_packed, const float* d_patches, int n, float* d_out, int layer, hipStream_t st, bool poly = false) {
     if (ctx->arith != AFFNET_ARITH_FP32_MFMA) return aff_fail(ctx, AFFNET_ERR_INVALID, "probe_affnet_wino: AFFNET_ARITH_FP32_MFMA only");
     const NetLayout L = net_layout(AFFNET_NET_AFFNET);
     CnnArgs a;
     memset(&a, 0, sizeof(a));
     a.packed = d_packed; a.off = to_offsets(L, ctx->arith);
-    const int rc = aff_wino_derive_u(ctx, AFFNET_NET_AFFNET, d_packed, L, st, &a.wino_u);
+    int rc = aff_wino_derive_u(ctx, AFFNET_NET_AFFNET, d_packed, L, st, &a.wino_u);
+    if (rc) return rc;
+    if (poly) rc = aff_poly16_derive_u(ctx, AFFNET_NET_AFFNET, d_packed, L, st);
     if (rc) return rc;
     a.patches = d_patches; a.n_max = n; a.out = d_out; a.dbg_layer = layer; a.dbg_out = d_out; a.dbg_time = ctx->dbg_time;
     PyrSrc ps;
     memset(&ps, 0, sizeof(ps));
-    hipLaunchKernelGGL(aff_trunk_affnet_wino(layer >= 0 || a.dbg_time), dim3(n, 1), dim3(512), 0, st, a, ps);
+    hipLaunchKernelGGL(poly ? aff_trunk_affnet_poly(layer >= 0 || a.dbg_time) : aff_trunk_affnet_wino(layer >= 0 || a.dbg_time), dim3(n, 1), dim3(512), 0, st, a, ps);
     AFF_LAUNCH_CHECK(ctx);
     return AFFNET_OK;
 }
@@ -100,6 +102,19 @@
     AFF_DEVICE(ctx);
     if (!ctx || !d_packed || !d_patches || !d_partials || n < 1 || n > 65535) return aff_fail(ctx, AFFNET_ERR_INVALID, "probe_affnet_wino_partials: bad argument");
     return probe_affnet_wino(ctx, d_packed, d_patches, n, d_partials, -1, (hipStream_t)stream);
+}
+
+extern "C" int affnet_probe_affnet_poly_layer(affnet_ctx* ctx, int net_kind, const float* d_packed, const float* d_patch, int layer, float* d_out, void* stream) {
+    AFF_DEVICE(ctx);
+    if (!ctx || !d_packed || !d_patch || !d_out || net_kind != AFFNET_NET_AFFNET || layer < 0 || layer > 5)
+        return aff_fail(ctx, AFFNET_ERR_INVALID, "probe_affnet_poly_layer: AffNet, layer 0 .. 5");
+    return probe_affnet_wino(ctx, d_packed, d_patch, 1, d_out, layer, (hipStream_t)stream, true);
+}
+
+extern "C" int affnet_probe_affnet_poly_partials(affnet_ctx* ctx, const float* d_packed, const float* d_patches, int n, float* d_partials, void* stream) {
+    AFF_DEVICE(ctx);
+    if (!ctx || !d_packed || !d_patches || !d_partials || n < 1 || n > 65535) return aff_fail(ctx, AFFNET_ERR_INVALID, "probe_affnet_poly_partials: bad argument");
+    return probe_affnet_wino(ctx, d_packed, d_patches, n, d_partials, -1, (hipStream_t)stream, true);
 }
 
 extern "C" int affnet_probe_hardnet_poly_layer(affnet_ctx* ctx, const float* d_packed, const float* d_patch, int layer, float* d_out, void* stream) {
diff --git a/affnet_amd/engine.py b/affnet_amd/engine.py
--- a/affnet_amd/engine.py
+++ b/affnet_amd/engine.py
@@ -43,7 +43,7 @@
         self.cfg = self.plan.fill_config(mr_size, threshold, num_features, num_prefilter, max_keep, raw_div=raw_div, batch=self.batch, baum_iters=baum_iters,
                                          onepass=onepass, lazy_shape_rows=lazy_shape_rows, arith=arith)
         self.arith = _lib.arith_code(arith)
-        self.shape_form = _lib.SHAPE_FORM_WINOGRAD
+        self.shape_form = _lib.SHAPE_FORM_POLYPHASE
         self.desc_form = _lib.DESC_FORM_POLYPHASE
         self.device = device
         self.handle = C.c_void_p()
diff --git a/include/affnet_hip.h b/include/affnet_hip.h
--- a/include/affnet_hip.h
+++ b/include/affnet_hip.h
@@ -70,6 +70,7 @@
 
 #define AFFNET_SHAPE_FORM_DIRECT 0
 #define AFFNET_SHAPE_FORM_WINOGRAD 1
+#define AFFNET_SHAPE_FORM_POLYPHASE 2
 int affnet_set_shape_form(affnet_ctx* ctx, int form);
 int affnet_get_shape_form(const affnet_ctx* ctx);
 
diff --git a/include/affnet_hip_probes.h b/include/affnet_hip_probes.h
--- a/include/affnet_hip_probes.h
+++ b/include/affnet_hip_probes.h
@@ -20,6 +20,9 @@
 
 int affnet_probe_affnet_wino_partials(affnet_ctx* ctx, const float* d_packed, const float* d_patches, int n, float* d_partials, void* stream);
 
+int affnet_probe_affnet_poly_layer(affnet_ctx* ctx, int net_kind, const float* d_packed, const float* d_patch, int layer, float* d_out, void* stream);
+int affnet_probe_affnet_poly_partials(affnet_ctx* ctx, const float* d_packed, const float* d_patches, int n, float* d_partials, void* stream);
+
 int affnet_probe_hardnet_poly_layer(affnet_ctx* ctx, const float* d_packed, const float* d_patch, int layer, float* d_out, void* stream);
 int affnet_probe_hardnet_poly_forward(affnet_ctx* ctx, const float* d_packed, const float* d_patches, int n, float* d_out, float* d_scratch, void* stream);
 int affnet_probe_hardnet_poly_u(affnet_ctx* ctx, const float* d_packed, int layer, float* d_out, void* stream);
```

Result: no change. 1.627 million (median of 6 runs) (+0.9%).
